# AlibabaResearch/efficientteacher

Hardware: AMD Instinct MI355X
Metric: SSOD images/sec (teacher+student step) YOLOv5l 640px (higher is better)
Workload: dtype bf16

## Files before the change

### efficientteacher_amd/_lib.py

```python
import ctypes
import os
from ctypes import c_char_p, c_double, c_float, c_int, c_int64, c_size_t, c_void_p

import torch

_HERE = os.path.dirname(os.path.abspath(__file__))
LIB_PATH = os.environ.get("ET_HIP_LIB") or os.path.join(_HERE, "libet_hip.so")

ET_F32, ET_BF16, ET_F16 = 0, 1, 2

P = c_void_p
SIGNATURES = {
    "et_build_arch": (c_char_p, []),
    "et_abi_version": (c_int, []),
    "et_nms_ssod_workspace_bytes": (c_int, [c_int, c_int, ctypes.POINTER(c_size_t)]),
    "et_nms_workspace_bytes": (c_int, [c_int, c_int, c_int, c_int, c_int, ctypes.POINTER(c_size_t)]),
    "et_nms": (c_int, [P, c_int, c_int, c_int, c_float, c_float, c_int, c_int, ctypes.c_uint64, ctypes.c_uint64, c_int,
                       c_float, c_int, P, P, P, P, P, c_size_t, P]),
    "et_nms_ssod": (c_int, [P, c_int, c_int, c_int, c_float, c_float, c_int, c_int, P, P, P, P, P, c_size_t, P]),
    "et_val_match": (c_int, [P, c_int, P, c_int, c_int, P, c_int, P, c_int, c_int, P, c_int, c_int, c_int, c_int64, c_int64,
                             P, P, P, P, P, P]),
    "et_val_ap_workspace_bytes": (c_int, [c_int, ctypes.POINTER(c_size_t)]),
    "et_val_ap": (c_int, [P, P, P, c_int64, P, c_int, c_int, P, P, P, P, P, c_size_t, P]),
    "et_detect_decode": (c_int, [P, c_int, c_int, c_int, c_int, c_int, c_int, c_int64, c_int64, c_int64, c_int64,
                                 P, c_float, P, c_int64, c_int64, P]),
    "et_ema_update": (c_int, [P, P, c_int64, c_float, c_float, P]),
    "et_adamw": (c_int, [P, P, P, P, P, c_int, c_int64, c_float, c_float, c_float, c_float, c_float, c_int, c_float, P, P]),
    "et_adamw_tick": (c_int, [P, c_float, c_float, P, P]),
    "et_adamw_dev": (c_int, [P, P, P, P, P, c_int, c_int64, c_float, c_float, c_float, c_float, c_float, P, c_float, P, P]),
    "et_sgd_nesterov": (c_int, [P, P, P, P, c_int, c_int64, c_float, c_float, c_float, c_int, c_float, P, P]),
    "et_cast_f32_to_lp": (c_int, [P, P, c_int, c_int64, P]),
    "et_scaler_check": (c_int, [P, c_int64, P, P]),
    "et_scaler_update": (c_int, [P, c_float, c_float, c_int, P]),
    "et_ema_update_dev": (c_int, [P, P, c_int64, P, P]),
    "et_sgd_nesterov_dev": (c_int, [P, P, P, P, c_int, c_int64, P, c_int, P, P]),
    "et_conv2d_stats_rows": (c_int, [c_int, c_int, c_int]),
    "et_conv2d_stats_rows_for": (c_int, [c_int] * 12),
    "et_conv2d_stats_adds_for": (c_int, [c_int] * 12),
    "et_conv2d_fwd": (c_int, [P, P, P, c_int] + [c_int] * 11 + [P, P, c_int, P, c_int, P, c_int, P, P]),
    "et_conv2d_dgrad": (c_int, [P, P, P, c_int] + [c_int] * 11 + [c_int, P, c_int, P, P]),
    "et_conv2d_dgrad_bn": (c_int, [P, P, P, c_int] + [c_int] * 10 + [P, c_int, P, c_int, P, P, c_int, P, c_int, P, P]),
    "et_conv2d_wgrad": (c_int, [P, P, P, c_int] + [c_int] * 11 + [P, P]),
    "et_conv2d_wgrad_grouped": (c_int, [P, c_int, c_int] + [c_int] * 9 + [P, P]),
    "et_weight_transpose_all": (c_int, [P, P, c_int, P, c_int, ctypes.c_longlong, P]),
    "et_weight_transpose": (c_int, [P, P, c_int, c_int, c_int, c_int, P]),
    "et_conv2d_kernel_name": (c_int, [c_int] * 13 + [c_char_p, c_int]),
    "et_env_knobs": (c_int, [c_char_p, c_int]),
    "et_conv2d_stem_u8_fwd": (c_int, [P, P, c_int, c_float, P, P, c_int, c_int, c_int, c_int, c_int, P, P, c_int, P, c_int, P, P]),
    "et_conv2d_stem_u8_wgrad": (c_int, [P, P, c_int, c_float, P, P, c_int, c_int, c_int, c_int, c_int, P, P]),
    "et_conv2d_stem_kernel_name": (c_int, [c_int] * 12 + [c_char_p, c_int]),
    "et_colsum": (c_int, [P, c_int, c_int, c_int, c_int, P, P]),
    "et_bn_reduce_rows": (c_int, [c_int, c_int, c_int]),
    "et_bn_finalize": (c_int, [P, c_int, c_int, c_double, P, P, c_float, c_float, P, P, P, P, P, P, P, P]),
    "et_bn_eval_affine": (c_int, [c_int, P, P, P, P, c_float, P, P, P]),
    "et_bn_act_fwd": (c_int, [P, c_int, P, c_int, P, c_int, c_int, c_int, c_int, P, P, c_int, P]),
    "et_bn_act_fwd_sharded": (c_int, [P, c_int, P, c_int, P, c_int, c_int, c_int, c_int, P, c_int, c_double, P, P, c_float, c_float,
                                      P, P, P, P, P, P, c_int, P]),
    "et_bn_act_bwd_sharded": (c_int, [P, c_int, P, c_int, P, c_int, c_int, c_int, c_int, P, P, P, P, P, c_int, P, P, P, c_int, c_int, P]),
    "et_bn_act_bwd": (c_int, [P, c_int, P, c_int, P, c_int, c_int, c_int, c_int, P, P, P, P, P, c_int, P, P, P, P,
                              c_size_t, P]),
    "et_bn_act_bwd_from_partials": (c_int, [P, c_int, P, c_int, P, c_int, c_int, c_int, c_int, P, P, P, P, P, c_int, P, P, P,
                                            P, c_int, P, P]),
    "et_act_bwd": (c_int, [P, c_int, P, c_int, P, c_int, c_int, c_int, c_int, c_int, P]),
    "et_pack_input": (c_int, [P, P, c_int, c_int, c_int, c_int, c_int, P]),
    "et_pack_input_u8": (c_int, [P, P, c_int, c_int, c_int, c_int, c_int, c_float, P]),
    "et_maxpool5_fwd": (c_int, [P, c_int, P, c_int, P, c_int, c_int, c_int, c_int, c_int, P]),
    "et_maxpool5_bwd": (c_int, [P, c_int, P, P, c_int, P, c_int, c_int, c_int, c_int, c_int, c_int, P]),
    "et_upsample2x_fwd": (c_int, [P, c_int, P, c_int, c_int, c_int, c_int, c_int, c_int, P]),
    "et_upsample2x_bwd": (c_int, [P, c_int, P, c_int, c_int, c_int, c_int, c_int, c_int, c_int, P]),
    "et_strong_view_u8": (c_int, [P, P, c_int, c_int, c_int, P, P, P, P, c_int, P]),
    "et_mosaic4_u8": (c_int, [P, P, c_int, c_int, c_int, P]),
    "et_pseudo_label_transform": (c_int, [P, P, P, c_int, c_int, c_int, c_int, c_int, P, P, P]),
    "et_score_log_append": (c_int, [P, P, c_int, c_int, P, P, P, c_int64, P]),
    "et_yolo_loss": (c_int, [P, P]),
    "et_ota_workspace_bytes": (c_int, [c_int, c_int, c_int, c_int, ctypes.POINTER(c_size_t)]),
    "et_ota_assign": (c_int, [P, P, c_float, c_int, P, P, P]),
    "et_select_targets": (c_int, [P, P, c_int, P, P, c_int, c_int, P, P]),
    "et_scale_cast": (c_int, [P, P, c_int, c_int64, c_float, P, P]),
    "et_domain_focal": (c_int, [P, c_int, c_int, c_int64, c_int, c_float, P, c_int, P, P]),
    "et_scale_inplace": (c_int, [P, c_int, c_int64, c_float, P, P]),
    "et_v8_decode": (c_int, [P, c_int, P, c_int, c_int, c_int, c_int, c_int, c_int, c_int, c_float, c_float, P, c_int64, c_int64, P]),
    "et_tal_loss": (c_int, [P, P, P, P, P, P, P, c_int, c_int, c_int, c_int, c_int, c_float, c_float, c_float, P, P, P, P, P]),
    "et_tal_assign_workspace_bytes": (c_int, [c_int, c_int, c_int, ctypes.POINTER(c_size_t)]),
    "et_tal_assign": (c_int, [P, P, P, P, P, P, c_int, c_int, c_int, c_int, c_int, c_float, c_float, c_float, P, P, P, P, P, c_size_t, P]),
    "et_tal_targets_pad": (c_int, [P, c_int, c_int, c_int, c_float, c_float, P, P, P]),
    "et_tal_pseudo_split": (c_int, [P, P, P, P, c_int, c_int, c_int, c_int, c_int, c_int, c_float, c_float, P, P, P, P, P, P, P, P, P]),
    "et_tal_assigned_gt": (c_int, [P, c_int, c_int, c_int, P, P]),
    "et_tal_merge_pseudo": (c_int, [P, P, P, P, P, P, P, P, P, c_int, c_int, c_int, c_int, P, P, P, P]),
}



class WgradItem(ctypes.Structure):
    _fields_ = [("x", ctypes.c_void_p), ("dy", ctypes.c_void_p), ("dw", ctypes.c_void_p), ("ldx", ctypes.c_int),
                ("ldy", ctypes.c_int)]


class LossLevel(ctypes.Structure):
    _fields_ = [("p", P), ("dp", P), ("tobj_ws", P), ("sb", c_int64), ("sa", c_int64), ("sy", c_int64),
                ("sx", c_int64), ("ny", c_int), ("nx", c_int), ("anchors", c_float * 6), ("balance", c_float)]


class LossDesc(ctypes.Structure):
    _fields_ = [("dtype", c_int), ("B", c_int), ("na", c_int), ("nc", c_int), ("NT", c_int), ("nl", c_int),
                ("anchor_t", c_float), ("gr", c_float), ("cp", c_float), ("cn", c_float), ("cls_pw", c_float),
                ("obj_pw", c_float), ("box_w", c_float), ("obj_w", c_float), ("cls_w", c_float),
                ("pass_mask", c_int), ("ignore_obj", c_int), ("targets", P), ("acc_ws", P), ("out", P),
                ("ota_match", P), ("obj_channel", c_int), ("balance_dev", P), ("autobalance_ssi", c_int), ("fl_gamma", c_float), ("level", LossLevel * 4)]


_dll = None
_emulated = False
CALL_TIMER = None
_NO_LAUNCH = frozenset(n for n in (
    "et_build_arch", "et_abi_version", "et_nms_ssod_workspace_bytes", "et_nms_workspace_bytes", "et_conv2d_stats_rows", "et_conv2d_stats_rows_for",
    "et_conv2d_kernel_name", "et_conv2d_stem_kernel_name", "et_env_knobs", "et_bn_reduce_rows", "et_ota_workspace_bytes", "et_tal_assign_workspace_bytes", "et_val_ap_workspace_bytes"))


class _TimedDll:

    def __init__(self, dll, timer):
        self._dll, self._timer, self._cache = dll, timer, {}

    def __getattr__(self, name):
        fn = self._cache.get(name)
        if fn is None:
            raw = getattr(self._dll, name)
            if name in _NO_LAUNCH or not name.startswith("et_"):
                fn = raw
            else:
                timer = self._timer

                def fn(*a, _raw=raw, _name=name):
                    tok = timer.begin(_name)
                    rc = _raw(*a)
                    timer.end(tok)
                    return rc
            self._cache[name] = fn
        return fn


class EtHipError(RuntimeError):
    pass


def _header_abi_version():
    import re
    with open(os.path.join(os.path.dirname(_HERE), "include", "et_hip.h")) as f:
        m = re.search(r"^#define\s+ET_ABI_VERSION\s+(\d+)", f.read(), re.M)
    if m is None:
        raise EtHipError("include/et_hip.h does not define ET_ABI_VERSION")
    return int(m.group(1))


ABI_VERSION = _header_abi_version()


def _declare(dll):
    for name, (res, args) in SIGNATURES.items():
        fn = getattr(dll, name)
        fn.restype = res
        fn.argtypes = args
    got = dll.et_abi_version()
    if got != ABI_VERSION:
        raise EtHipError(f"{getattr(dll, '_name', 'libet_hip.so')} has ABI version {got}, this binding needs {ABI_VERSION}: "
                         f"rebuild it (python -m efficientteacher_amd.csrc.build)")
    return dll


def load(path=None):
    global _dll
    if _dll is None:
        path = path or LIB_PATH
        if not os.path.exists(path):
            raise EtHipError(
                f"{path} not found: build the gfx950 kernels first "
                f"(python -m efficientteacher_amd.csrc.build).  There is no CPU fallback.")
        _dll = _declare(ctypes.CDLL(path))
    if CALL_TIMER is not None:
        w = getattr(CALL_TIMER, "_wrapped", None)
        if w is None or w._dll is not _dll:
            w = CALL_TIMER._wrapped = _TimedDll(_dll, CALL_TIMER)
        return w
    return _dll


def _use_library_for_tests(path, emulated):
    global _dll, _emulated
    _dll = _declare(ctypes.CDLL(path)) if path else None
    _emulated = bool(emulated) if path else False


def is_emulated():
    return _emulated
# ... 27 lines not shown
```

### efficientteacher_amd/autograd.py

```python
import torch
from torch.autograd import Function

from . import ops

ACT_CODE = {"silu": ops.ACT_SILU, "relu": ops.ACT_RELU, "none": ops.ACT_NONE}

FUSE_BN_BWD = True
FUSE_BN_BWD_K = 1
_RS_DGRAD = {}


def _dgrad_on_rs_tile(cs, x):
    key = (tuple(x.shape), x.dtype, cs.cinp, cs.coutp, cs.k, cs.stride, cs.pad)
    r = _RS_DGRAD.get(key)
    if r is None:
        N, H, W, _ = x.shape
        r = _RS_DGRAD[key] = cs.stride == 1 and ops.kernel_name("dgrad_full", x.dtype, N, H, W, cs.cinp, cs.coutp, cs.k, cs.stride,
                                                               cs.pad).startswith("conv_gemm_rs_kernel")
    return r


def _fuse_into(cs, bn, x=None):
    if bn is None:
        return None
    if FUSE_BN_BWD_K & (1 if cs.k == 1 else 2):
        return bn
    if cs.k > 1 and (FUSE_BN_BWD_K & 4) and x is not None and _dgrad_on_rs_tile(cs, x):
        return bn
    return None
SHARDED_BN = True


def _bn_train_fwd(x, w_lp, cs_stride, cs_pad, bs, act, residual=None, out=None):
    N, IH, IW, Cin = x.shape
    sh = None
    if SHARDED_BN and bs.sh_ld and ops.few_rows("fwd", x.dtype, N, IH, IW, Cin, w_lp.shape[0], w_lp.shape[1], cs_stride, cs_pad):
        sh = bs.acquire_fwd()
    if sh is not None:
        y = ops.conv2d_fwd(x, w_lp, cs_stride, cs_pad, shards=sh)
        N, OH, OW, _ = y.shape
        z, scale, shift, mean, invstd = ops.bn_act_fwd_sharded(y, sh, N * OH * OW, bs.gamma, bs.beta, bs.eps, bs.momentum, bs.rmean,
                                                               bs.rvar, act, residual=residual, out=out)
        return y, z, scale, shift, mean, invstd
    y, stats = ops.conv2d_fwd(x, w_lp, cs_stride, cs_pad, want_stats=True)
    N, OH, OW, _ = y.shape
    scale, shift, mean, invstd = ops.bn_finalize(stats, N * OH * OW, bs.gamma, bs.beta, bs.eps, bs.momentum, bs.rmean, bs.rvar)
    z = ops.bn_act_fwd(y, scale, shift, act, residual=residual, out=out)
    return y, z, scale, shift, mean, invstd


def _bn_sums(y, scale, shift, act, bs):
    return ops.BnBwdSums(y, scale, shift, act, slot=bs if (SHARDED_BN and bs.sh_ld) else None)


def _bn_train_bwd(dz, y, bs, scale, shift, mean, invstd, act, sums=None, out=None):
    part = sums.take(dz) if sums is not None else None
    if SHARDED_BN and bs.sh_ld and (isinstance(part, tuple) or (part is None and ops.few_reduce_rows(y))):
        sh = part if part is not None else bs.acquire_bwd()
        return ops.bn_act_bwd(dz, y, bs.gamma, scale, shift, mean, invstd, act, bs.ggamma, bs.gbeta, out=out, partial=part, shards=sh)
    return ops.bn_act_bwd(dz, y, bs.gamma, scale, shift, mean, invstd, act, bs.ggamma, bs.gbeta, out=out, partial=part)


GRAD_FORK = True

GRAD_READY_HOOK = None


class GradFork:

    def __init__(self):
        self.gb = None
        self.merged = False

    @staticmethod
    def split(x):
        if not (GRAD_FORK and torch.is_grad_enabled() and x.requires_grad):
            return x, x, None
        h = GradFork()
        a, b = _ForkFn.apply(x, h)
        return a, b, h

    @staticmethod
    def tap(b, fork):
        return b if fork is None else _TapFn.apply(b, fork)

    def take(self, shape, dtype):
        g = self.gb
        if g is None or tuple(g.shape) != tuple(shape) or g.dtype != dtype or g.dim() != 4 or g.stride(3) != 1:
            return None
        ld = g.stride(2)
        if not (ld >= g.shape[3] and g.stride(1) == ld * g.shape[2] and g.stride(0) == ld * g.shape[2] * g.shape[1]):
            return None
        return g


class _ForkFn(Function):
    @staticmethod
    def forward(ctx, x, holder):
        ctx.holder = holder
        return (x.as_strided(x.size(), x.stride(), x.storage_offset()), x.as_strided(x.size(), x.stride(), x.storage_offset()))

    @staticmethod
    def backward(ctx, ga, gb):
        h = ctx.holder
        merged = h.merged
        h.gb, h.merged = None, False
        if ga is None or gb is None:
            return (gb if ga is None else ga), None
        if merged:
            return ga, None
        return ga + gb, None


class _TapFn(Function):
    @staticmethod
    def forward(ctx, x, holder):
        ctx.holder = holder
        return x.as_strided(x.size(), x.stride(), x.storage_offset())

    @staticmethod
    def backward(ctx, g):
        ctx.holder.gb = g
        ctx.holder.merged = False
        return g, None


def _wgrad(x, dy, cs, *more_slots):
    hook = GRAD_READY_HOOK
    slots = (cs,) + more_slots

    def done():
        if hook is not None:
            for s in slots:
                hook(s)
    ops.WGRAD_QUEUE.submit(x, dy, cs.gw if not more_slots else _fused_gw(cs), cs.k, cs.stride, cs.pad,
                           on_done=done if hook is not None else None)


def _fused_gw(cs1):
    return cs1.gw.as_strided((2 * cs1.cout, 1, 1, cs1.cinp), (cs1.cinp, cs1.cinp, cs1.cinp, 1), cs1.gw.storage_offset())


class ConvBnActFn(Function):

    @staticmethod
    def forward(ctx, x, residual, wparam, cs, bs, act, nbt, dst=None, bn_in=None, bn_out=None, acc=None, u8=None):
        ctx.u8 = u8
        ctx.x_u8 = x if isinstance(x, ops.U8Images) else None
        ctx.w_needs_grad = wparam.requires_grad
        ctx.bn_in = bn_in if (bn_in is not None and cs.stride == 1 and residual is None) else None
        ctx.acc = acc
        if nbt is not None:
            nbt.add_(1)
        out = None if dst is None else dst[0][..., dst[1]:dst[1] + cs.coutp]
        y, z, scale, shift, mean, invstd = _bn_train_fwd(x, cs.w_lp, cs.stride, cs.pad, bs, act, residual=residual, out=out)
        ctx.cs, ctx.bs, ctx.act = cs, bs, act
        ctx.has_res = residual is not None
        ctx.x_needs_grad = x.requires_grad
        ctx.bn_mine = None
        if bn_out is not None and residual is None:
            ctx.bn_mine = _bn_sums(y, scale, shift, act, bs)
            bn_out.append(ctx.bn_mine)
        ctx.save_for_backward(None if ctx.x_u8 is not None else x, y, scale, shift, mean, invstd)
        return z

    @staticmethod
    def backward(ctx, dz):
        x, y, scale, shift, mean, invstd = ctx.saved_tensors
        cs, bs = ctx.cs, ctx.bs
        dz = _dense_or_slice(dz)
        dy = _bn_train_bwd(dz, y, bs, scale, shift, mean, invstd, ctx.act, sums=ctx.bn_mine)
        if ctx.w_needs_grad and ctx.u8 is not None:
            hook = GRAD_READY_HOOK
            ops.WGRAD_QUEUE.submit_stem_u8(ctx.u8, dy, cs.gw, on_done=(lambda: hook(cs)) if hook is not None else None)
        elif ctx.w_needs_grad:
            _wgrad(x if ctx.x_u8 is None else ctx.x_u8.packed(), dy, cs)
        dx = None
        if ctx.x_needs_grad:
            wT = cs.transposed()
            into = ctx.acc.take(x.shape, dy.dtype) if (ctx.acc is not None and ctx.bn_in is None) else None
            if into is not None:
                dx = ops.conv2d_dgrad(dy, wT, (x.shape[1], x.shape[2]), cs.stride, cs.pad, out=into, accumulate=True)
                ctx.acc.merged = True
            else:
                dx = ops.conv2d_dgrad(dy, wT, (x.shape[1], x.shape[2]), cs.stride, cs.pad, bn=_fuse_into(cs, ctx.bn_in, x))
        return dx, (dz if ctx.has_res else None), None, None, None, None, None, None, None, None, None, None


class BottleneckFn(Function):

    @staticmethod
    def forward(ctx, x, w1, w2, cs1, bs1, cs2, bs2, act1, act2, nbt1, nbt2, dst=None, bn_in=None, bn_out=None):
        ctx.w_needs_grad = w1.requires_grad or w2.requires_grad
        ctx.bn_in = bn_in
        y1, h, *a1 = _bn_train_fwd(x, cs1.w_lp, cs1.stride, cs1.pad, bs1, act1)
        for nbt in (nbt1, nbt2):
            if nbt is not None:
                nbt.add_(1)
        out = None if dst is None else dst[0][..., dst[1]:dst[1] + cs2.coutp]
        y2, z, *a2 = _bn_train_fwd(h, cs2.w_lp, cs2.stride, cs2.pad, bs2, act2, residual=x, out=out)
        ctx.meta = (cs1, bs1, cs2, bs2, act1, act2)
        ctx.x_needs_grad = x.requires_grad
        ctx.bn_mine = None
        if bn_out is not None:
            ctx.bn_mine = _bn_sums(y2, a2[0], a2[1], act2, bs2)
            bn_out.append(ctx.bn_mine)
        ctx.save_for_backward(x, y1, h, y2, *a1, *a2)
        return z

    @staticmethod
    def backward(ctx, dz):
        x, y1, h, y2, s1, b1, m1, i1, s2, b2, m2, i2 = ctx.saved_tensors
        cs1, bs1, cs2, bs2, act1, act2 = ctx.meta
        dz = _dense_or_slice(dz)
        dy2 = _bn_train_bwd(dz, y2, bs2, s2, b2, m2, i2, act2, sums=ctx.bn_mine)
        if ctx.w_needs_grad:
            _wgrad(h, dy2, cs2)
        inner = _fuse_into(cs2, _bn_sums(y1, s1, b1, act1, bs1), h) if FUSE_BN_BWD else None
        dh = ops.conv2d_dgrad(dy2, cs2.transposed(), (h.shape[1], h.shape[2]), cs2.stride, cs2.pad, bn=inner)
        dy1 = _bn_train_bwd(dh, y1, bs1, s1, b1, m1, i1, act1, sums=inner)
        if ctx.w_needs_grad:
            _wgrad(x, dy1, cs1)
        dx = None
        if ctx.x_needs_grad:
            dx = ops.conv2d_dgrad(dy1, cs1.transposed(), (x.shape[1], x.shape[2]), cs1.stride, cs1.pad,
                                  residual=dz, bn=_fuse_into(cs1, ctx.bn_in, x))
        return (dx,) + (None,) * 13


def c3_stem_fusable(cs1, bs1, cs2, bs2):
    es = cs1.w_lp.element_size()
    return (cs1.k == 1 and cs2.k == 1 and cs1.stride == 1 and cs2.stride == 1 and cs1.cinp == cs2.cinp
            and cs1.coutp == cs1.cout and cs2.coutp == cs2.cout and cs1.cout == cs2.cout
            and cs2.w_lp.data_ptr() == cs1.w_lp.data_ptr() + cs1.w_lp.numel() * es
            and cs2.gw.data_ptr() == cs1.gw.data_ptr() + cs1.gw.numel() * 4
            and bs2.aff_off == bs1.aff_off + bs1.c and bs1.c == cs1.cout and bs2.c == cs2.cout
            and bs1.eps == bs2.eps and bs1.momentum == bs2.momentum)


def _fused_vec(a, b):
    return a.as_strided((a.numel() + b.numel(),), (1,), a.storage_offset())


class C3StemFn(Function):

    @staticmethod
    def forward(ctx, x, w1, w2, cs1, bs1, cs2, bs2, act, nbt1, nbt2, buf, bn_out=None):
        ctx.w_needs_grad = w1.requires_grad or w2.requires_grad
        c = cs1.cout
        wf = cs1.w_lp.as_strided((2 * c, 1, 1, cs1.cinp), (cs1.cinp, cs1.cinp, cs1.cinp, 1), cs1.w_lp.storage_offset())
        sh1 = sh2 = None
        if SHARDED_BN and bs1.sh_ld and bs2.sh_ld and ops.few_rows("fwd", x.dtype, x.shape[0], x.shape[1], x.shape[2], cs1.cinp, 2 * c, 1, 1, 0):
            sh1, sh2 = bs1.acquire_fwd(), bs2.acquire_fwd()
        for nbt in (nbt1, nbt2):
            if nbt is not None:
                nbt.add_(1)
        if sh1 is not None and sh2 is not None:
            y = ops.conv2d_fwd(x, wf, 1, 0, shards=sh1)
            N, H, W, _ = y.shape
            af = torch.empty((4, 2 * c), dtype=torch.float32, device=y.device)
            t = ops.bn_act_fwd_sharded(y[..., :c], sh1, N * H * W, bs1.gamma, bs1.beta, bs1.eps, bs1.momentum, bs1.rmean, bs1.rvar,
                                       act, out=buf[..., :c], aff=af[:, :c])[0]
            y2 = ops.bn_act_fwd_sharded(y[..., c:], sh2, N * H * W, bs2.gamma, bs2.beta, bs2.eps, bs2.momentum, bs2.rmean, bs2.rvar,
                                        act, out=buf[..., 2 * c:], aff=af[:, c:])[0]
            aff = (af[0], af[1], af[2], af[3])
        else:
            y, st = ops.conv2d_fwd(x, wf, 1, 0, want_stats=True)
            N, H, W, _ = y.shape
            aff = ops.bn_finalize(st, N * H * W, _fused_vec(bs1.gamma, bs2.gamma), _fused_vec(bs1.beta, bs2.beta), bs1.eps,
                                  bs1.momentum, _fused_vec(bs1.rmean, bs2.rmean), _fused_vec(bs1.rvar, bs2.rvar))
            t = ops.bn_act_fwd(y[..., :c], aff[0][:c], aff[1][:c], act, out=buf[..., :c])
            y2 = ops.bn_act_fwd(y[..., c:], aff[0][c:], aff[1][c:], act, out=buf[..., 2 * c:])
        ctx.meta = (cs1, bs1, cs2, bs2, act)
        ctx.x_needs_grad = x.requires_grad
        ctx.bn_mine = None
        if bn_out is not None:
            ctx.bn_mine = _bn_sums(y[..., :c], aff[0][:c], aff[1][:c], act, bs1)
            bn_out.append(ctx.bn_mine)
        ctx.save_for_backward(x, y, *aff)
        return t, y2

    @staticmethod
    def backward(ctx, dt, dy2):
        x, y, scale, shift, mean, invstd = ctx.saved_tensors
        cs1, bs1, cs2, bs2, act = ctx.meta
        c = cs1.cout
        N, H, W, _ = y.shape
        dy = torch.empty_like(y)
        halves = ((dt, slice(0, c), bs1), (dy2, slice(c, 2 * c), bs2))
        for g, sl, bs in halves:
            if g is None:
                dy[..., sl].zero_()
                continue
            g = _dense_or_slice(g)
            _bn_train_bwd(g, y[..., sl], bs, scale[sl], shift[sl], mean[sl], invstd[sl], act,
                          sums=ctx.bn_mine if sl.start == 0 else None, out=dy[..., sl])
        if ctx.w_needs_grad:
            _wgrad(x, dy, cs1, cs2)
        dx = None
        if ctx.x_needs_grad:
            wf = cs1.w_lp.as_strided((2 * c, 1, 1, cs1.cinp), (cs1.cinp, cs1.cinp, cs1.cinp, 1), cs1.w_lp.storage_offset())
            dx = ops.conv2d_dgrad(dy, ops.weight_transpose(wf), (x.shape[1], x.shape[2]), 1, 0)
        return (dx,) + (None,) * 11


class _GradDst:

    def __init__(self, p):
        self.shape, self.stride, self.dtype, self.device = tuple(p.shape), tuple(p.stride()), p.dtype, p.device
        self.span = ops._flat_span(p)
        self.buf = None
        self.written = [False, False]

    def flat(self, half, n):
        if self.buf is None:
            self.buf = torch.empty(self.span, dtype=self.dtype, device=self.device)
        cut = n * self.stride[0]
        self.written[half] = True
        return self.buf[:cut] if half == 0 else self.buf[cut:]


class BatchSplitFn(Function):
    @staticmethod
    def forward(ctx, p, n, holder):
        ctx.n, ctx.holder = n, holder
        return p[:n], p[n:]

    @staticmethod
    def backward(ctx, ga, gb):
        h, n = ctx.holder, ctx.n
        cut = n * h.stride[0]

        def is_slot(g, half):
            return (g is not None and h.buf is not None and h.written[half] and tuple(g.stride()) == h.stride
                    and g.data_ptr() == h.buf.data_ptr() + (cut * h.buf.element_size() if half else 0))
        if h.buf is None:
            h.buf = torch.empty(h.span, dtype=h.dtype, device=h.device)
        full = h.buf.as_strided(h.shape, h.stride)
        for half, g in ((0, ga), (1, gb)):
            if is_slot(g, half):
                continue
            dst = full[:n] if half == 0 else full[n:]
            if g is None:
                (h.buf[:cut] if half == 0 else h.buf[cut:]).zero_()
            else:
                (h.buf[:cut] if half == 0 else h.buf[cut:]).zero_()
                dst.copy_(g)
        return full, None, None


def split_batch(p, n):
    if not (torch.is_grad_enabled() and p.requires_grad) or n <= 0 or n >= p.shape[0]:
        return p[:n], p[n:]
    h = _GradDst(p)
    a, b = BatchSplitFn.apply(p, n, h)
    a._et_grad_dst = (h, 0, n)
    b._et_grad_dst = (h, 1, n)
    return a, b


class ConvBiasFn(Function):

    @staticmethod
    def forward(ctx, x, wparam, cs, act, head):
        ctx.w_needs_grad = wparam.requires_grad
        y = ops.conv2d_fwd(x, cs.w_lp, cs.stride, cs.pad, bias=cs.bias, act=act)
        ctx.cs, ctx.act, ctx.head = cs, act, head
        ctx.x_needs_grad = x.requires_grad
        ctx.save_for_backward(x, y)
        if head is None:
            return y
        return head_view(y, *head)

    @staticmethod
    def backward(ctx, dy):
        x, y = ctx.saved_tensors
        cs = ctx.cs
        if ctx.head is not None:
            dy = head_grad_to_nhwc(dy, y.shape, *ctx.head)
        dy = _dense_or_slice(dy)
        if ctx.act != ops.ACT_NONE:
            dy = ops.act_bwd(dy, y, ctx.act)
        if ctx.w_needs_grad:
            ops.conv2d_wgrad(x, dy, cs.gw, cs.k, cs.stride, cs.pad)
            if cs.gbias is not None:
                ops.colsum(dy, cs.gbias)
            if GRAD_READY_HOOK is not None:
                GRAD_READY_HOOK(cs)
        dx = None
        if ctx.x_needs_grad:
            wT = cs.transposed()
            dx = ops.conv2d_dgrad(dy, wT, (x.shape[1], x.shape[2]), cs.stride, cs.pad)
        return dx, None, None, None, None


def head_view(y, na, no):
    B, ny, nx, CP = y.shape
    return y.as_strided((B, na, ny, nx, no), (ny * nx * CP, no, nx * CP, CP, 1), y.storage_offset())


def head_grad_to_nhwc(g, yshape, na, no):
    B, ny, nx, CP = yshape
    want = (ny * nx * CP, no, nx * CP, CP, 1)
    need = (g.storage_offset() + B * ny * nx * CP) * g.element_size()
    if tuple(g.stride()) == want and g.untyped_storage().nbytes() >= need:
        return g.as_strided((B, ny, nx, CP), (ny * nx * CP, nx * CP, CP, 1), g.storage_offset())
    buf = torch.zeros((B, ny, nx, CP), dtype=g.dtype, device=g.device)
    buf.as_strided((B, na, ny, nx, no), want).copy_(g)
    return buf


class JoinSlicesFn(Function):

    @staticmethod
    def forward(ctx, holder, *parts):
        buf = holder[0]
        off = 0
        for p in parts:
            assert p.data_ptr() == buf.data_ptr() + off * buf.element_size() and p.stride() == buf[..., :1].stride()
            off += p.shape[3]
        assert off == buf.shape[3]
        ctx.splits = [p.shape[3] for p in parts]
        return buf

    @staticmethod
    def backward(ctx, dcat):
        dcat = _dense_or_slice(dcat)
        return (None, *torch.split(dcat, ctx.splits, dim=3))


class SppfPoolFn(Function):

    @staticmethod
    def forward(ctx, x, holder=None):
        N, H, W, C = x.shape
        if holder is not None:
            cat = holder[0]
            assert cat.shape == (N, H, W, 4 * C) and x.data_ptr() == cat.data_ptr() and x.stride() == cat[..., :C].stride()
        else:
            cat = torch.empty((N, H, W, 4 * C), dtype=x.dtype, device=x.device)
            cat[..., :C].copy_(x)
        idx = []
        for i in range(3):
            _, ix = ops.maxpool5_fwd(cat[..., i * C:(i + 1) * C], out=cat[..., (i + 1) * C:(i + 2) * C])
            idx.append(ix)
        ctx.save_for_backward(*idx)
        ctx.C = C
        return cat

    @staticmethod
    def backward(ctx, dcat):
        i1, i2, i3 = ctx.saved_tensors
        C = ctx.C
        dcat = _dense_or_slice(dcat)
        d2 = ops.maxpool5_bwd(dcat[..., 3 * C:], i3, base=dcat[..., 2 * C:3 * C])
        d1 = ops.maxpool5_bwd(d2, i2, base=dcat[..., C:2 * C])
        return ops.maxpool5_bwd(d1, i1, base=dcat[..., :C]), None


class UpsampleCatFn(Function):

    @staticmethod
    def forward(ctx, a, b, acc=None, buf=None):
        N, H, W, Ca = a.shape
        Cb = b.shape[3]
        cat = in_place_concat_buffer(b, Ca, buf)
        if cat is None or cat.shape != (N, 2 * H, 2 * W, Ca + Cb):
            cat = torch.empty((N, 2 * H, 2 * W, Ca + Cb), dtype=a.dtype, device=a.device)
            cat[..., Ca:].copy_(b)
        ops.upsample2x_fwd(a, out=cat[..., :Ca])
        ctx.Ca = Ca
        ctx.acc = acc
        ctx.a_shape = tuple(a.shape)
        return cat

    @staticmethod
    def backward(ctx, dcat):
        dcat = _dense_or_slice(dcat)
        da_src = dcat[..., :ctx.Ca]
        into = ctx.acc.take(ctx.a_shape, dcat.dtype) if ctx.acc is not None else None
        if into is not None:
            da = ops.upsample2x_bwd(da_src, out=into, accumulate=True)
            ctx.acc.merged = True
        else:
            da = ops.upsample2x_bwd(da_src)
        return da, dcat[..., ctx.Ca:], None, None


def in_place_concat_buffer(b, Ca, buf):
    if buf is None:
        return None
    es = buf.element_size()
    if (b.data_ptr() == buf.data_ptr() + Ca * es and b.stride() == buf[..., Ca:].stride() and b.shape[:3] == buf.shape[:3]
            and Ca + b.shape[3] == buf.shape[3]):
        return buf
    return None


class GradReverseFn(Function):
    @staticmethod
    def forward(ctx, x):
        return x.view_as(x)

    @staticmethod
    def backward(ctx, g):
        return ops.scale_inplace(g.contiguous().clone(), -1.0)


class DomainFocalFn(Function):

    @staticmethod
    def forward(ctx, label, *feats):
        total = sum(f.shape[0] * f.shape[1] * f.shape[2] for f in feats)
        acc = torch.zeros(1, dtype=torch.float32, device=feats[0].device)
        grads = [ops.domain_focal(f, label, 0.5 / total, acc, want_grad=True) for f in feats]
        ctx.save_for_backward(*grads)
        return ops.scale_cast(acc, torch.float32, scale=0.5 / total)

    @staticmethod
    def backward(ctx, gout):
        g = gout.reshape(1).float().contiguous()
        return (None, *[ops.scale_inplace(gr.clone(), 1.0, dev_scale=g) for gr in ctx.saved_tensors])


def _dense_or_slice(g):
    if g.dim() == 4 and g.stride(3) == 1:
        ld = g.stride(2)
        if ld >= g.shape[3] and g.stride(1) == ld * g.shape[2] and g.stride(0) == ld * g.shape[2] * g.shape[1]:
            return g
    return g.contiguous()
```

### efficientteacher_amd/csrc/conv.hip

```cpp
#include "et_device.h"
#include "../../include/et_hip.h"
#include <stdlib.h>
#include <stdio.h>
#include <string.h>
#include <type_traits>

typedef __attribute__((ext_vector_type(16))) float f32x16;
typedef __attribute__((ext_vector_type(8))) __bf16 bf16x8;
typedef __attribute__((ext_vector_type(8))) _Float16 f16x8;
typedef __attribute__((ext_vector_type(4))) unsigned int u32x4;
__device__ __forceinline__ u32x4 mk4(unsigned a, unsigned b, unsigned c, unsigned d) { u32x4 v = {a, b, c, d}; return v; }
__device__ __forceinline__ void et_pin_loaded(u32x4& v) {
#if defined(__HIP_DEVICE_COMPILE__)
    asm volatile("" : "+v"(v));
#endif
}

template <typename T, typename V> __device__ __forceinline__ f32x16 et_mfma32(const V a, const V b, const f32x16 c) {
    static_assert(sizeof(V) == 16, "8 x 16-bit operands");
    if constexpr (std::is_same<T, et_f16>::value)
        return __builtin_amdgcn_mfma_f32_32x32x16_f16(__builtin_bit_cast(f16x8, a), __builtin_bit_cast(f16x8, b), c, 0, 0, 0);
    else
        return __builtin_amdgcn_mfma_f32_32x32x16_bf16(__builtin_bit_cast(bf16x8, a), __builtin_bit_cast(bf16x8, b), c, 0, 0, 0);
}

#define CONV_MAX_TAPS 36
#ifndef ET_S1_NT
#define ET_S1_NT 1
#endif
#ifndef ET_GLDS_SHORTK_WGS
#define ET_GLDS_SHORTK_WGS 4
#endif
#define RS_A_ROWS(BM) ((BM) + 16)

struct FastDiv {
    uint32_t magic, shift, d;
};
static FastDiv make_fastdiv(uint32_t d) {
    FastDiv f;
    if (d == 0) d = 1;
    f.d = d;
    uint32_t s = 0;
    while ((1ull << s) < d) ++s;
    f.shift = s;
    f.magic = (uint32_t)((((1ull << 32) * ((1ull << s) - d)) / d) + 1);
    return f;
}
__device__ __forceinline__ uint32_t fdiv(uint32_t n, const FastDiv& f) {
    return (__umulhi(n, f.magic) + n) >> f.shift;
}

struct GatherGeom {
    int N, IH, IW, Cin, ldx;
    int QH, QW, M;
    int OH, OW, Cout, ldy;
    int isy, isx;
    int osy, osx, ooy, oox;
    int T, TT;
    int CV, KV;
    int tap_inner;
    int xcd_swz;
    int ntm, ntn, nfast;
    FastDiv dQW, dQH, dCV, dW1;
    signed char dy[CONV_MAX_TAPS], dx[CONV_MAX_TAPS];
    unsigned char wt[CONV_MAX_TAPS];
    int tapinfo[CONV_MAX_TAPS];
};

__device__ __forceinline__ void tap_lookup_uniform(const GatherGeom& g, int tap, int& dy, int& dx, int& wt) {
    const int ti = g.tapinfo[__builtin_amdgcn_readfirstlane(tap)];
    dy = (int)(signed char)(ti & 0xff);
    dx = (int)(signed char)((ti >> 8) & 0xff);
    wt = (ti >> 16) & 0xff;
}

enum { ACT_NONE = 0, ACT_SILU = 1, ACT_RELU = 2 };

struct Epilogue {
    const float* scale;
    const float* bias;
    int act;
    const void* res;
    int ldr;
    float* stats;
    int accumulate;
    const void* bn_y;
    int ld_bn;
    const float* bn_scale;
    const float* bn_shift;
    int bn_act;
    int stats_ld;
};

__device__ __forceinline__ void tile_of_block(const GatherGeom& g, int& bx, int& by) {
    int id = blockIdx.x;
    if (g.nfast) {
        if (g.xcd_swz) {
            const int nb = gridDim.x, q = nb >> 3, r = nb & 7, xcd = id & 7, k = id >> 3;
            id = (xcd < r ? xcd * (q + 1) : r * (q + 1) + (xcd - r) * q) + k;
        }
        bx = id / g.ntn;
        by = id - bx * g.ntn;
    } else {
        by = id / g.ntm;
        bx = id - by * g.ntm;
        if (g.xcd_swz) {
            const int nb = g.ntm, q = nb >> 3, r = nb & 7, xcd = bx & 7, k = bx >> 3;
            bx = (xcd < r ? xcd * (q + 1) : r * (q + 1) + (xcd - r) * q) + k;
        }
    }
}

template <int BKV> __device__ __forceinline__ int lds_swz(int r) {
    if constexpr (BKV == 8) return ((r >> 1) & 7) ^ ((r >> 4) & 3);
    else return (r >> 2) & 3;
}


struct NoBetween { __device__ __forceinline__ void operator()(int) const {} };
template <typename T, int BM, int BN, int WM, int WN, int BKV, typename BETWEEN = NoBetween>
__device__ __forceinline__ void mma_chunk(const u32x4* __restrict__ sm, f32x16 (&acc)[BM / WM / 32][BN / WN / 32],
                                          int wm, int wn, int lane, BETWEEN between = BETWEEN()) {
    constexpr int TM = BM / WM / 32, TN = BN / WN / 32;
    const int l31 = lane & 31, g = lane >> 5;
    u32x4 af[2][TM], bf[2][TN];
    auto fetch = [&](int kk, int set) {
#pragma unroll
        for (int tm = 0; tm < TM; ++tm) {
            const int r = wm * (BM / WM) + tm * 32 + l31;
            af[set][tm] = sm[r * BKV + ((kk * 2 + g) ^ lds_swz<BKV>(r))];
        }
#pragma unroll
        for (int tn = 0; tn < TN; ++tn) {
            const int r = wn * (BN / WN) + tn * 32 + l31;
            bf[set][tn] = sm[(BM + r) * BKV + ((kk * 2 + g) ^ lds_swz<BKV>(r))];
        }
    };
    fetch(0, 0);
#pragma unroll
    for (int kk = 0; kk < BKV / 2; ++kk) {
        const int cur = kk & 1;
        if (kk + 1 < BKV / 2) {
            fetch(kk + 1, cur ^ 1);
            __builtin_amdgcn_sched_barrier(0);
        }
#pragma unroll
        for (int tm = 0; tm < TM; ++tm)
#pragma unroll
            for (int tn = 0; tn < TN; ++tn) {
                if constexpr (sizeof(T) == 2) {
                    acc[tm][tn] = et_mfma32<T>(af[cur][tm], bf[cur][tn], acc[tm][tn]);
                } else {
                    acc[tm][tn] = __builtin_amdgcn_mfma_f32_32x32x2f32(__uint_as_float(af[cur][tm].x), __uint_as_float(bf[cur][tn].x), acc[tm][tn], 0, 0, 0);
                    acc[tm][tn] = __builtin_amdgcn_mfma_f32_32x32x2f32(__uint_as_float(af[cur][tm].y), __uint_as_float(bf[cur][tn].y), acc[tm][tn], 0, 0, 0);
                    acc[tm][tn] = __builtin_amdgcn_mfma_f32_32x32x2f32(__uint_as_float(af[cur][tm].z), __uint_as_float(bf[cur][tn].z), acc[tm][tn], 0, 0, 0);
                    acc[tm][tn] = __builtin_amdgcn_mfma_f32_32x32x2f32(__uint_as_float(af[cur][tm].w), __uint_as_float(bf[cur][tn].w), acc[tm][tn], 0, 0, 0);
                }
            }
        between(kk);
    }
}

template <int BM, int BN, int WM, int WN, int SROWS = 32> struct EpiLds {
    static constexpr int WCOLS = BN / WN, SLD = WCOLS + 4, SLAB = SROWS * SLD;
    static constexpr int FLOATS = WM * WN * SLAB;
    static constexpr int VEC16 = (FLOATS * 4 + 15) / 16;
};

template <int TN> struct EpiSums {
    float ssum[TN], ssq[TN];
    float bs1[8], bs2[8];
    const float* cst = nullptr;
    int cstride = 0;
    __device__ __forceinline__ void clear() {
#pragma unroll
        for (int tn = 0; tn < TN; ++tn) { ssum[tn] = 0.f; ssq[tn] = 0.f; }
#pragma unroll
        for (int e = 0; e < 8; ++e) { bs1[e] = 0.f; bs2[e] = 0.f; }
    }
};

template <int BN, int WN, int MODE>
__device__ __forceinline__ void conv_epilogue_write_stats(EpiSums<BN / WN / 32>& st, const GatherGeom& g, const Epilogue& ep, int n0, int lane,
                                                          int wn, int row, int zero_rows, int nrows) {
    constexpr int TN = BN / WN / 32, WCOLS = BN / WN, CVN = WCOLS / 8;
    const int l31 = lane & 31, hi = lane >> 5;
    const int scv = lane % CVN;
    const int co = n0 + wn * WCOLS + scv * 8;
    const bool bnb = MODE == 1 ? false : ep.bn_y != nullptr;
    if (bnb) {
#pragma unroll
        for (int e = 0; e < 8; ++e)
            for (int m = CVN; m < 64; m <<= 1) { st.bs1[e] += __shfl_xor(st.bs1[e], m); st.bs2[e] += __shfl_xor(st.bs2[e], m); }
        if (ep.stats_ld) {
            if (lane < CVN && co + 8 <= g.Cout) {
                float* d0 = ep.stats + ((size_t)(blockIdx.x % ET_BN_SHARDS) * 2) * ep.stats_ld + co;
#pragma unroll
                for (int e = 0; e < 8; ++e) { unsafeAtomicAdd(d0 + e, st.bs1[e]); unsafeAtomicAdd(d0 + ep.stats_ld + e, st.bs2[e]); }
            }
        } else if (lane < CVN && co + 8 <= g.Cout) {
            for (int r = 0; r <= zero_rows; ++r) {
                if (row + r >= nrows) break;
                float* d0 = ep.stats + ((size_t)(row + r) * 2 + 0) * g.Cout + co;
                float* d1 = ep.stats + ((size_t)(row + r) * 2 + 1) * g.Cout + co;
                if (r == 0) {
                    *(float4*)d0 = make_float4(st.bs1[0], st.bs1[1], st.bs1[2], st.bs1[3]); *(float4*)(d0 + 4) = make_float4(st.bs1[4], st.bs1[5], st.bs1[6], st.bs1[7]);
                    *(float4*)d1 = make_float4(st.bs2[0], st.bs2[1], st.bs2[2], st.bs2[3]); *(float4*)(d1 + 4) = make_float4(st.bs2[4], st.bs2[5], st.bs2[6], st.bs2[7]);
                } else {
                    const float4 z = make_float4(0.f, 0.f, 0.f, 0.f);
                    *(float4*)d0 = z; *(float4*)(d0 + 4) = z; *(float4*)d1 = z; *(float4*)(d1 + 4) = z;
                }
            }
        }
    } else {
#pragma unroll
        for (int tn = 0; tn < TN; ++tn) {
            const float sv = st.ssum[tn] + __shfl_xor(st.ssum[tn], 32);
            const float qv = st.ssq[tn] + __shfl_xor(st.ssq[tn], 32);
            const int cc = n0 + wn * WCOLS + tn * 32 + l31;
            if (ep.stats_ld) {
                if (hi == 0 && cc < g.Cout) {
                    float* d0 = ep.stats + ((size_t)(blockIdx.x % ET_BN_SHARDS) * 2) * ep.stats_ld + cc;
                    unsafeAtomicAdd(d0, sv); unsafeAtomicAdd(d0 + ep.stats_ld, qv);
                }
            } else if (hi == 0 && cc < g.Cout) {
                for (int r = 0; r <= zero_rows; ++r) {
                    if (row + r >= nrows) break;
                    ep.stats[((size_t)(row + r) * 2 + 0) * g.Cout + cc] = r == 0 ? sv : 0.f;
                    ep.stats[((size_t)(row + r) * 2 + 1) * g.Cout + cc] = r == 0 ? qv : 0.f;
                }
            }
        }
    }
}

template <int BN, int WN, int WM, int MODE>
__device__ __forceinline__ void conv_stats_add_sharded_wg(EpiSums<BN / WN / 32>& st, const GatherGeom& g, const Epilogue& ep, int tid, int lane,
                                                          int wm, int wn, float* red, int n0 = 0) {
    constexpr int TN = BN / WN / 32, WCOLS = BN / WN, CVN = WCOLS / 8;
    const int l31 = lane & 31, hi = lane >> 5;
    const bool bnb = MODE == 1 ? false : ep.bn_y != nullptr;
    __syncthreads();
    float* const r0 = red + (wm * 2) * BN + wn * WCOLS;
    if (bnb) {
        const int scv = lane % CVN;
#pragma unroll
        for (int e = 0; e < 8; ++e)
            for (int m = CVN; m < 64; m <<= 1) { st.bs1[e] += __shfl_xor(st.bs1[e], m); st.bs2[e] += __shfl_xor(st.bs2[e], m); }
        if (lane < CVN) {
#pragma unroll
            for (int e = 0; e < 8; ++e) { r0[scv * 8 + e] = st.bs1[e]; r0[BN + scv * 8 + e] = st.bs2[e]; }
        }
    } else {
#pragma unroll
        for (int tn = 0; tn < TN; ++tn) {
            const float sv = st.ssum[tn] + __shfl_xor(st.ssum[tn], 32);
            const float qv = st.ssq[tn] + __shfl_xor(st.ssq[tn], 32);
            if (hi == 0) { r0[tn * 32 + l31] = sv; r0[BN + tn * 32 + l31] = qv; }
        }
    }
    __syncthreads();
    float* const dst = ep.stats + ((size_t)(blockIdx.x % ET_BN_SHARDS) * 2) * ep.stats_ld + n0;
    for (int i = tid; i < 2 * BN; i += 64 * WM * WN) {
        const int t = i / BN, c = i % BN;
        float v = 0.f;
#pragma unroll
        for (int w = 0; w < WM; ++w) v += red[(w * 2 + t) * BN + c];
        if (n0 + c < g.Cout) unsafeAtomicAdd(dst + (size_t)t * ep.stats_ld + c, v);
    }
}

template <typename T, int BM, int BN, int WM, int WN, int ACT, int SROWS = 32, int MODE = 0, bool DEFER = false, bool EPF = true>
__device__ __forceinline__ void conv_epilogue_act(f32x16 (&acc)[BM / WM / 32][BN / WN / 32], u32x4* lds_raw, T* __restrict__ Y,
                                                  const GatherGeom& g, const Epilogue& ep, int bx, int m0, int n0, int tid,
                                                  int lane, int wm, int wn, EpiSums<BN / WN / 32>& st) {
    constexpr int TM = BM / WM / 32, TN = BN / WN / 32;
    static_assert(SROWS == 32 || SROWS == 16, "slab rows");
    constexpr int NH = 32 / SROWS;
    using L = EpiLds<BM, BN, WM, WN, SROWS>;
    constexpr int WCOLS = L::WCOLS, SLD = L::SLD;
    constexpr int CVN = WCOLS / 8;
    constexpr int RPI = 64 / CVN;
    static_assert(RPI <= SROWS, "a store iteration covers at most one slab");
    const int l31 = lane & 31, hi = lane >> 5;
    const int wave = wm * WN + wn;
    float* const stg = (float*)lds_raw + wave * L::SLAB;
    float (&ssum)[TN] = st.ssum;
    float (&ssq)[TN] = st.ssq;
    float (&bs1)[8] = st.bs1;
    float (&bs2)[8] = st.bs2;
    const bool ident = (g.osy == 1 && g.osx == 1 && g.ooy == 0 && g.oox == 0 && g.QH == g.OH && g.QW == g.OW);
    float csc[TN], cbi[TN];
#pragma unroll
    for (int tn = 0; tn < TN; ++tn) {
        const int co = n0 + wn * WCOLS + tn * 32 + l31;
        const bool cok = co < g.Cout;
        if constexpr (DEFER) {
            csc[tn] = st.cst[co - n0];
            cbi[tn] = st.cst[st.cstride + co - n0];
        } else {
            csc[tn] = (ep.scale && cok) ? ep.scale[co] : 1.0f;
            cbi[tn] = (ep.bias && cok) ? ep.bias[co] : 0.0f;
        }
    }
    const int srow = lane / CVN, scv = lane % CVN;
    const int co = n0 + wn * WCOLS + scv * 8;
    const bool bnb = MODE == 1 ? false : ep.bn_y != nullptr;
    const void* const ep_res = MODE == 1 ? nullptr : ep.res;
    const bool ep_accumulate = MODE == 1 ? false : (bool)ep.accumulate;
    const bool lean = ident && !bnb && ep_res == nullptr && !ep_accumulate && m0 + (wm + 1) * (BM / WM) <= g.M && n0 + BN <= g.Cout;
    float bsc[8], bsh[8];
#pragma unroll
    for (int e = 0; e < 8; ++e) { bsc[e] = 1.f; bsh[e] = 0.f; }
    if (bnb && co + 8 <= g.Cout) {
#pragma unroll
        for (int e = 0; e < 8; ++e) {
            if constexpr (DEFER) { bsc[e] = st.cst[2 * st.cstride + co - n0 + e]; bsh[e] = st.cst[3 * st.cstride + co - n0 + e]; }
            else { bsc[e] = ep.bn_scale[co + e]; bsh[e] = ep.bn_shift[co + e]; }
        }
    }
    auto bn_bwd_sums = [&](const float (&dz8)[8], const float (&y8)[8]) {
        auto body = [&](auto act_tag) {
            constexpr int BACT = decltype(act_tag)::value;
#pragma unroll
            for (int e = 0; e < 8; ++e) {
                const float u = y8[e] * bsc[e] + bsh[e];
                float gact = 1.f;
                if constexpr (BACT == ACT_SILU) { const float sg = __builtin_amdgcn_rcpf(1.0f + __expf(-u)); gact = sg * (1.0f + u * (1.0f - sg)); }
                else if constexpr (BACT == ACT_RELU) gact = u > 0.f ? 1.f : 0.f;
                const float du = dz8[e] * gact;
                bs1[e] += du;
                bs2[e] += du * y8[e];
            }
        };
        if (ep.bn_act == ACT_SILU) body(std::integral_constant<int, ACT_SILU>{});
        else if (ep.bn_act == ACT_RELU) body(std::integral_constant<int, ACT_RELU>{});
        else body(std::integral_constant<int, ACT_NONE>{});
    };
    constexpr int NIT = SROWS / RPI;
    constexpr bool PF = EPF && sizeof(T) == 2 && MODE == 0;
    const bool pf_on = PF && !lean && (ep_res != nullptr || ep_accumulate || bnb);
    const bool pf_a_is_res = ep_res != nullptr;
    u32x4 pf_a[NIT], pf_b[NIT];
    auto pix_of = [&](int p) -> long long {
        if (ident) return p;
        const uint32_t t1 = fdiv((uint32_t)p, g.dQW), qx = p - t1 * g.QW;
        const uint32_t n = fdiv(t1, g.dQH), qy = t1 - n * g.QH;
        return ((long long)n * g.OH + (qy * g.osy + g.ooy)) * g.OW + (qx * g.osx + g.oox);
    };
#pragma unroll
    for (int tmh = 0; tmh < TM * NH; ++tmh) {
        const int tm = tmh / NH, hoff = (tmh % NH) * SROWS;
        if constexpr (PF) {
            if (pf_on) {
#pragma unroll
                for (int it = 0; it < NIT; ++it) {
                    const int p = m0 + wm * (BM / WM) + tm * 32 + hoff + it * RPI + srow;
                    if (p < g.M && co + 8 <= g.Cout) {
                        const long long pix = pix_of(p);
                        if (pf_a_is_res) pf_a[it] = *(const u32x4*)((const T*)ep_res + pix * ep.ldr + co);
                        else if (ep_accumulate) pf_a[it] = *(const u32x4*)(Y + pix * g.ldy + co);
                        if (bnb) pf_b[it] = *(const u32x4*)((const T*)ep.bn_y + pix * ep.ld_bn + co);
                    }
                }
            }
        }
#pragma unroll
        for (int rr = 0; rr < 16 / NH; ++rr) {
            const int r = (tmh % NH) * (16 / NH) + rr;
            const int row = (rr & 3) + 8 * (rr >> 2) + 4 * hi;
#pragma unroll
            for (int tn = 0; tn < TN; ++tn) {
                float v = acc[tm][tn][r];
                ssum[tn] += v;
                ssq[tn] += v * v;
                v = v * csc[tn] + cbi[tn];
                if constexpr (ACT == ACT_SILU) v = v * __builtin_amdgcn_rcpf(1.0f + __expf(-v));
                else if constexpr (ACT == ACT_RELU) v = fmaxf(v, 0.f);
                stg[row * SLD + tn * 32 + l31] = v;
            }
        }
        __builtin_amdgcn_s_waitcnt(0xC07F);
        __builtin_amdgcn_wave_barrier();
        if constexpr (sizeof(T) == 2) {
            if (lean) {
#pragma unroll
                for (int it = 0; it < SROWS / RPI; ++it) {
                    const int row = it * RPI + srow;
                    const long long p = m0 + wm * (BM / WM) + tm * 32 + hoff + row;
                    const float4 a = *(const float4*)(stg + row * SLD + scv * 8);
                    const float4 b = *(const float4*)(stg + row * SLD + scv * 8 + 4);
                    *(u32x4*)(Y + p * g.ldy + co) = mk4(et_lp<T>::pack(a.x, a.y), et_lp<T>::pack(a.z, a.w), et_lp<T>::pack(b.x, b.y), et_lp<T>::pack(b.z, b.w));
                }
                __builtin_amdgcn_s_waitcnt(0xC07F);
                __builtin_amdgcn_wave_barrier();
                continue;
            }
        }
#pragma unroll
        for (int it = 0; it < SROWS / RPI; ++it) {
            const int row = it * RPI + srow;
            const int p = m0 + wm * (BM / WM) + tm * 32 + hoff + row;
            if (p < g.M && co < g.Cout) {
                const long long pix = pix_of(p);
                float v[8];
                const float4 a = *(const float4*)(stg + row * SLD + scv * 8);
                const float4 b = *(const float4*)(stg + row * SLD + scv * 8 + 4);
                v[0] = a.x; v[1] = a.y; v[2] = a.z; v[3] = a.w; v[4] = b.x; v[5] = b.y; v[6] = b.z; v[7] = b.w;
                T* yp = Y + pix * g.ldy + co;
                if (co + 8 <= g.Cout) {
                    if constexpr (sizeof(T) == 2) {
                        if (ep_res) {
                            u32x4 rr;
                            if constexpr (PF) rr = pf_a[it];
                            else rr = *(const u32x4*)((const T*)ep_res + pix * ep.ldr + co);
                            v[0] += et_lp<T>::lo(rr.x); v[1] += et_lp<T>::hi(rr.x);
                            v[2] += et_lp<T>::lo(rr.y); v[3] += et_lp<T>::hi(rr.y);
                            v[4] += et_lp<T>::lo(rr.z); v[5] += et_lp<T>::hi(rr.z);
                            v[6] += et_lp<T>::lo(rr.w); v[7] += et_lp<T>::hi(rr.w);
                        }
                        if (ep_accumulate) {
                            u32x4 rr;
                            if (PF && !pf_a_is_res) rr = pf_a[it];
                            else rr = *(const u32x4*)yp;
                            v[0] += et_lp<T>::lo(rr.x); v[1] += et_lp<T>::hi(rr.x);
                            v[2] += et_lp<T>::lo(rr.y); v[3] += et_lp<T>::hi(rr.y);
                            v[4] += et_lp<T>::lo(rr.z); v[5] += et_lp<T>::hi(rr.z);
                            v[6] += et_lp<T>::lo(rr.w); v[7] += et_lp<T>::hi(rr.w);
                        }
                        const u32x4 packed = mk4(et_lp<T>::pack(v[0], v[1]), et_lp<T>::pack(v[2], v[3]), et_lp<T>::pack(v[4], v[5]),
                                                 et_lp<T>::pack(v[6], v[7]));
                        *(u32x4*)yp = packed;
                        if (bnb) {
                            u32x4 yy;
                            if constexpr (PF) yy = pf_b[it];
                            else yy = *(const u32x4*)((const T*)ep.bn_y + pix * ep.ld_bn + co);
                            const unsigned pw[4] = {packed.x, packed.y, packed.z, packed.w}, yw[4] = {yy.x, yy.y, yy.z, yy.w};
                            float dz8[8], y8[8];
#pragma unroll
                            for (int e = 0; e < 8; ++e) {
                                dz8[e] = (e & 1) ? et_lp<T>::hi(pw[e >> 1]) : et_lp<T>::lo(pw[e >> 1]);
                                y8[e] = (e & 1) ? et_lp<T>::hi(yw[e >> 1]) : et_lp<T>::lo(yw[e >> 1]);
                            }
                            bn_bwd_sums(dz8, y8);
                        }
                    } else {
                        if (ep_res) {
                            const float* rp = (const float*)ep_res + pix * ep.ldr + co;
                            const float4 r0 = *(const float4*)rp, r1 = *(const float4*)(rp + 4);
                            v[0] += r0.x; v[1] += r0.y; v[2] += r0.z; v[3] += r0.w; v[4] += r1.x; v[5] += r1.y; v[6] += r1.z; v[7] += r1.w;
                        }
                        if (ep_accumulate) {
                            const float4 r0 = *(const float4*)yp, r1 = *(const float4*)((const float*)yp + 4);
                            v[0] += r0.x; v[1] += r0.y; v[2] += r0.z; v[3] += r0.w; v[4] += r1.x; v[5] += r1.y; v[6] += r1.z; v[7] += r1.w;
                        }
                        *(float4*)yp = make_float4(v[0], v[1], v[2], v[3]);
                        *(float4*)((float*)yp + 4) = make_float4(v[4], v[5], v[6], v[7]);
                        if (bnb) {
                            const float* bp = (const float*)ep.bn_y + pix * ep.ld_bn + co;
                            const float4 y0 = *(const float4*)bp, y1 = *(const float4*)(bp + 4);
                            const float yv8[8] = {y0.x, y0.y, y0.z, y0.w, y1.x, y1.y, y1.z, y1.w};
                            bn_bwd_sums(v, yv8);
                        }
                    }
                } else {
                    for (int e = 0; e < 8 && co + e < g.Cout; ++e) {
                        float x = v[e];
                        if (ep_res) x += et_elem<T>::ld(((const T*)ep_res)[pix * ep.ldr + co + e]);
                        if (ep_accumulate) x += et_elem<T>::ld(yp[e]);
                        yp[e] = et_elem<T>::st(x);
                    }
                }
            }
        }
        __builtin_amdgcn_s_waitcnt(0xC07F);
        __builtin_amdgcn_wave_barrier();
    }
    if constexpr (!DEFER) {
        if (ep.stats) {
            constexpr int RPW = (BM / WM) / 64;
            static_assert((BM / WM) % 64 == 0, "wave tiles are whole 64-row blocks");
            if (ep.stats_ld) conv_stats_add_sharded_wg<BN, WN, WM, MODE>(st, g, ep, tid, lane, wm, wn, (float*)lds_raw, n0);
            else conv_epilogue_write_stats<BN, WN, MODE>(st, g, ep, n0, lane, wn, (m0 + wm * (BM / WM)) / 64, RPW - 1, (g.M + 63) / 64);
        }
    }
}

template <typename T, int BM, int BN, int WM, int WN, int SROWS = 32, int MODE = 0, bool DEFER = false, bool EPF = true>
__device__ __forceinline__ void conv_epilogue(f32x16 (&acc)[BM / WM / 32][BN / WN / 32], u32x4* lds_raw, T* __restrict__ Y,
                                              const GatherGeom& g, const Epilogue& ep, int bx, int m0, int n0, int tid,
                                              int lane, int wm, int wn, EpiSums<BN / WN / 32>& st) {
    if (ep.act == ACT_SILU) conv_epilogue_act<T, BM, BN, WM, WN, ACT_SILU, SROWS, MODE, DEFER, EPF>(acc, lds_raw, Y, g, ep, bx, m0, n0, tid, lane, wm, wn, st);
    else if (ep.act == ACT_RELU) conv_epilogue_act<T, BM, BN, WM, WN, ACT_RELU, SROWS, MODE, DEFER, EPF>(acc, lds_raw, Y, g, ep, bx, m0, n0, tid, lane, wm, wn, st);
    else conv_epilogue_act<T, BM, BN, WM, WN, ACT_NONE, SROWS, MODE, DEFER, EPF>(acc, lds_raw, Y, g, ep, bx, m0, n0, tid, lane, wm, wn, st);
}
template <typename T, int BM, int BN, int WM, int WN, bool EPF = true>
__device__ __forceinline__ void conv_epilogue(f32x16 (&acc)[BM / WM / 32][BN / WN / 32], u32x4* lds_raw, T* __restrict__ Y,
                                              const GatherGeom& g, const Epilogue& ep, int bx, int m0, int n0, int tid,
                                              int lane, int wm, int wn) {
    EpiSums<BN / WN / 32> st;
    st.clear();
    conv_epilogue<T, BM, BN, WM, WN, 32, 0, false, EPF>(acc, lds_raw, Y, g, ep, bx, m0, n0, tid, lane, wm, wn, st);
}

template <typename T, int BM, int BN, int WM, int WN, int BKV, bool UTAP>
__global__ __launch_bounds__(256) void conv_gemm_kernel(const T* __restrict__ X, const T* __restrict__ W,
                                                        T* __restrict__ Y, GatherGeom g, Epilogue ep) {
    constexpr int VEC = et_elem<T>::VEC;
    constexpr int TM = BM / WM / 32, TN = BN / WN / 32;
    constexpr int RPT = 256 / BKV;
    constexpr int RA = BM / RPT, RB = BN / RPT;
    constexpr int STAGE_VEC = (BM + BN) * BKV;
    constexpr int EPI_VEC = EpiLds<BM, BN, WM, WN>::VEC16;
    constexpr int LDS_VEC = 2 * STAGE_VEC > EPI_VEC ? 2 * STAGE_VEC : EPI_VEC;
    __shared__ __attribute__((aligned(16))) u32x4 lds_raw[LDS_VEC];
    u32x4* const lds0 = lds_raw;
    u32x4* const lds1 = lds_raw + STAGE_VEC;

    const int tid = threadIdx.x, lane = tid & 63, wave = tid >> 6;
    const int wm = wave / WN, wn = wave % WN;
    int bx, by;
    tile_of_block(g, bx, by);
    const int m0 = bx * BM, n0 = by * BN;
    const int lvec = tid % BKV, lrow = tid / BKV;

    int a_off[RA], a_iy[RA], a_ix[RA];
    bool a_ok[RA];
#pragma unroll
    for (int j = 0; j < RA; ++j) {
        const int p = m0 + lrow + j * RPT;
        a_ok[j] = p < g.M;
        const uint32_t pp = a_ok[j] ? p : 0;
        const uint32_t t1 = fdiv(pp, g.dQW), qx = pp - t1 * g.QW;
        const uint32_t n = fdiv(t1, g.dQH), qy = t1 - n * g.QH;
        a_iy[j] = qy * g.isy;
        a_ix[j] = qx * g.isx;
        a_off[j] = ((n * g.IH + a_iy[j]) * g.IW + a_ix[j]) * g.ldx;
    }
    int b_off[RB];
    bool b_ok[RB];
#pragma unroll
    for (int j = 0; j < RB; ++j) {
        const int co = n0 + lrow + j * RPT;
        b_ok[j] = co < g.Cout;
        b_off[j] = (b_ok[j] ? co : 0) * g.TT * g.Cin;
    }

    f32x16 acc[TM][TN];
#pragma unroll
    for (int tm = 0; tm < TM; ++tm)
#pragma unroll
        for (int tn = 0; tn < TN; ++tn)
#pragma unroll
            for (int r = 0; r < 16; ++r) acc[tm][tn][r] = 0.f;

    const int nchunks = (g.KV + BKV - 1) / BKV;
    u32x4 raA[RA], rbA[RB], raB[RA], rbB[RB];
    unsigned okA = 0u, okB = 0u;
    int tap_u = 0, cv_u = 0;

    auto gload = [&](int chunk, int tap_c, int cv_c, u32x4 (&ra)[RA], u32x4 (&rb)[RB]) -> unsigned {
        int tap, cv;
        bool kok = true;
        if constexpr (UTAP) {
            tap = tap_c; cv = cv_c + lvec;
        } else {
            const uint32_t kv = chunk * BKV + lvec;
            kok = kv < (uint32_t)g.KV;
            const uint32_t kk = kok ? kv : 0;
            tap = fdiv(kk, g.dCV); cv = kk - tap * g.CV;
        }
        int dy, dx, wt;
        if constexpr (UTAP) tap_lookup_uniform(g, tap, dy, dx, wt);
        else { dy = g.dy[tap]; dx = g.dx[tap]; wt = g.wt[tap]; }
        const int doff = (dy * g.IW + dx) * g.ldx + cv * VEC;
        const int woff = wt * g.Cin + cv * VEC;
        unsigned okmask = 0u;
#pragma unroll
        for (int j = 0; j < RA; ++j) {
            const bool ok = kok && a_ok[j] && (unsigned)(a_iy[j] + dy) < (unsigned)g.IH &&
                            (unsigned)(a_ix[j] + dx) < (unsigned)g.IW;
            ra[j] = *(const u32x4*)(X + (ok ? a_off[j] + doff : 0));
            okmask |= ok ? (1u << j) : 0u;
        }
#pragma unroll
        for (int j = 0; j < RB; ++j) {
            const bool ok = kok && b_ok[j];
            rb[j] = *(const u32x4*)(W + (ok ? b_off[j] + woff : 0));
            okmask |= ok ? (1u << (16 + j)) : 0u;
        }
        return okmask;
    };
#define ET_ADVANCE_CURSOR()                                              \
    if constexpr (UTAP) {                                                \
        if (g.tap_inner) {                                               \
            if (++tap_u >= g.T) { tap_u = 0; cv_u += BKV; }              \
        } else {                                                         \
            cv_u += BKV;                                                 \
            if (cv_u >= g.CV) { cv_u = 0; ++tap_u; }                     \
        }                                                                \
    }
    auto lstore = [&](u32x4* __restrict__ dst, const u32x4 (&ra)[RA], const u32x4 (&rb)[RB], unsigned okmask) {
        const u32x4 zero = mk4(0, 0, 0, 0);
#pragma unroll
        for (int j = 0; j < RA; ++j) {
            const int r = lrow + j * RPT;
            dst[r * BKV + (lvec ^ lds_swz<BKV>(r))] = ((okmask >> j) & 1u) ? ra[j] : zero;
        }
#pragma unroll
        for (int j = 0; j < RB; ++j) {
            const int r = lrow + j * RPT;
            dst[(BM + r) * BKV + (lvec ^ lds_swz<BKV>(r))] = ((okmask >> (16 + j)) & 1u) ? rb[j] : zero;
// ... 623 lines not shown
    auto stage_a_piece = [&](int q, int ub, int j, int cv) {
        u32x4* const wbase = slotA + ub * A_VEC + q * 512 + wave * 64;
        const int dy = sgn * (j - 1);
        if constexpr (BUF) {
            const unsigned bad = (a_nokm >> (3 * q + 1 + dy)) & 1u;
            et_bufdma16(rsX, (bad << 31) | (unsigned)a_off[q], (unsigned)(((dy + 1) * rowstep + cv * VEC) * (int)sizeof(T)), wbase);
        } else {
            const bool ok = (a_okm >> (3 * q + 1 + dy)) & 1u;
            et_glds16(ok ? X + (a_off[q] + dy * g.IW * g.ldx + (cv + lv) * VEC) : ZERO, wbase);
        }
    };
    auto stage_b_piece = [&](int j, int b, int jj, int tap, int cv) {
        u32x4* const wbase = slotB + (2 * j + b) * HALF_VEC + wave * 64;
        if constexpr (BUF) {
            et_bufdma16(rsW, voffB, (unsigned)(((jj * 128 + j * 32) * wrow + tap * g.Cin + cv * VEC) * (int)sizeof(T)), wbase + jj * 512);
        } else {
            const bool ok = (b_okm >> (j * 2 + jj)) & 1u;
            et_glds16(ok ? W + (b_off0 + (jj * 128 + j * 32) * wrow + tap * g.Cin + (cv + lv) * VEC) : ZERO, wbase + jj * 512);
        }
    };

    u32x4 af[2][4], bf[4];
    auto load_a = [&](int i, int ub, auto shift_tag) {
        constexpr int SFT = decltype(shift_tag)::value;
        const char* sm = (const char*)(slotA + ub * A_VEC);
#pragma unroll
        for (int t = 0; t < 2; ++t)
#pragma unroll
            for (int kk = 0; kk < 4; ++kk) af[t][kk] = *(const u32x4*)(sm + (abase[i][t][SFT] ^ (kk * 32)));
    };
    auto load_b = [&](int j, int b) {
        const u32x4* sm = slotB + (2 * j + b) * HALF_VEC;
        const int r = wn * 32 + l31;
#pragma unroll
        for (int kk = 0; kk < 4; ++kk) bf[kk] = sm[r * BKV + ((kk * 2 + gk) ^ lds_swz<BKV>(r))];
    };
    auto mfma8 = [&](int i, int j, auto&& piece0, auto&& piece1) {
        __builtin_amdgcn_s_setprio(1);
        __builtin_amdgcn_sched_barrier(0);
#pragma unroll
        for (int kk = 0; kk < 4; ++kk)
#pragma unroll
            for (int t = 0; t < 2; ++t) {
                acc[2 * i + t][j] = et_mfma32<T>(af[t][kk], bf[kk], acc[2 * i + t][j]);
                const int n = kk * 2 + t;
                if (n == 1) { __builtin_amdgcn_sched_barrier(0); piece0(); __builtin_amdgcn_sched_barrier(0); }
                if (n == 4) { __builtin_amdgcn_sched_barrier(0); piece1(); __builtin_amdgcn_sched_barrier(0); }
            }
        __builtin_amdgcn_sched_barrier(0);
        __builtin_amdgcn_s_setprio(0);
    };
    auto nothing = [] {};

    const int nunits = 3 * (g.CV / BKV);
#pragma unroll
    for (int q = 0; q < NPIECE; ++q) stage_a_piece(q, 0, 0, 0);
#pragma unroll
    for (int j = 0; j < 2; ++j) { stage_b_piece(j, 0, 0, sgn > 0 ? 0 : 2, 0); stage_b_piece(j, 0, 1, sgn > 0 ? 0 : 2, 0); }
    et_wait_vmem();
    __builtin_amdgcn_s_barrier();
#define ET_PP_BAR() __builtin_amdgcn_s_barrier()
#define ET_PP_WAIT(n) et_wait_vmem_le_pp<n>()
    if (wm == 1) __builtin_amdgcn_s_barrier();

    int jrow = 0, cv_u = 0, bbuf = 0;
#pragma unroll 1
    for (int u = 0; u < nunits; ++u) {
        const bool more = u + 1 < nunits;
        int nj = jrow + 1, ncv = cv_u;
        if (nj == 3) { nj = 0; ncv += BKV; }
        const int ub = u & 1, nub = ub ^ 1;
        auto chunk = [&](auto ktag) {
            constexpr int k = decltype(ktag)::value;
            const bool stage_b = k < 2 || more;
            const int kn = k < 2 ? k + 1 : 0;
            const int ntap = (k < 2 ? jrow : nj) * 3 + (sgn > 0 ? kn : 2 - kn), nbcv = k < 2 ? cv_u : ncv;
            const int nb = bbuf ^ 1;
            const std::integral_constant<int, k> shift{};
            load_a(0, ub, shift); load_b(0, bbuf);
            if (k > 0 && more) ET_PP_WAIT(1); else ET_PP_WAIT(0);
            ET_PP_BAR();
            mfma8(0, 0, [&] { if (more) stage_a_piece(2 * k, nub, nj, ncv); }, nothing);
            ET_PP_BAR();
            load_b(1, bbuf);
            ET_PP_BAR();
            mfma8(0, 1, [&] { if (stage_b) stage_b_piece(0, nb, 0, ntap, nbcv); }, [&] { if (stage_b) stage_b_piece(0, nb, 1, ntap, nbcv); });
            ET_PP_BAR();
            load_a(1, ub, shift);
            ET_PP_BAR();
            mfma8(1, 1, [&] { if (stage_b) stage_b_piece(1, nb, 0, ntap, nbcv); }, [&] { if (stage_b) stage_b_piece(1, nb, 1, ntap, nbcv); });
            ET_PP_BAR();
            load_b(0, bbuf);
            if (stage_b) ET_PP_WAIT(2); else ET_PP_WAIT(0);
            ET_PP_BAR();
            mfma8(1, 0, [&] { if (k < 2 && more) stage_a_piece(2 * k + 1, nub, nj, ncv); }, nothing);
            ET_PP_BAR();
            bbuf = nb;
        };
        chunk(std::integral_constant<int, 0>{});
        chunk(std::integral_constant<int, 1>{});
        chunk(std::integral_constant<int, 2>{});
        jrow = nj; cv_u = ncv;
    }
    if (wm == 0) __builtin_amdgcn_s_barrier();
    __syncthreads();
    conv_epilogue<T, BM, BN, WM, WN, false>(acc, lds_raw, Y, g, ep, bx, m0, n0, tid, lane, wm, wn);
#undef ET_PP_BAR
#undef ET_PP_WAIT
}
template <typename T>
__global__ __launch_bounds__(512, 2) void conv_gemm_pprs_kernel(const T* __restrict__ X, const T* __restrict__ W,
                                                                T* __restrict__ Y, const T* __restrict__ ZERO,
                                                                GatherGeom g, Epilogue ep) {
    conv_gemm_pprs_body<T, true>(X, W, Y, ZERO, g, ep);
}
template <typename T>
__global__ __launch_bounds__(512, 2) void conv_gemm_pprs_flat_kernel(const T* __restrict__ X, const T* __restrict__ W,
                                                                     T* __restrict__ Y, const T* __restrict__ ZERO,
                                                                     GatherGeom g, Epilogue ep) {
    conv_gemm_pprs_body<T, false>(X, W, Y, ZERO, g, ep);
}

template <typename T, int KC, int WN, int TN, int WM, int TMW, int NS, int WGS, bool FULL, bool BUF>
__device__ __forceinline__ void conv1x1_stream_body(const T* __restrict__ X, const T* __restrict__ W,
                                                    T* __restrict__ Y, const T* __restrict__ ZERO,
                                                    const GatherGeom& g, const Epilogue& ep) {
    constexpr int BN = 32 * TN * WN, BM = 32 * TMW * WM, BKV = 8, VEC = 8;
    constexpr int TM = TMW;
    constexpr int NT = 64 * WM * WN;
    constexpr int CH_VEC = BM * BKV;
    constexpr int DT = CH_VEC < NT ? CH_VEC : NT;
    constexpr int PER = CH_VEC / DT;
    constexpr int MODE = FULL ? 0 : 1;
    using L = EpiLds<BM, BN, WM, WN, 16>;
    static_assert(KC == 1 || KC == 2 || KC == 4, "K = 64 * KC");
    static_assert(CH_VEC % DT == 0 && DT % 64 == 0 && PER >= 1 && (NS - 1) * PER < 64 && NS >= 2 && NS <= 16, "ring");
    __shared__ __attribute__((aligned(16))) u32x4 lds_raw[NS * CH_VEC + L::VEC16 + BN];
    u32x4* const ring = lds_raw;
    u32x4* const slabs = lds_raw + NS * CH_VEC;
    float* const cst = (float*)(lds_raw + NS * CH_VEC + L::VEC16);

    const int tid = threadIdx.x, lane = tid & 63;
    const int wave = __builtin_amdgcn_readfirstlane(tid >> 6);
    const int wm = wave / WN, wn = wave % WN;
    const int l31 = lane & 31, gk = lane >> 5;
    const int lvec = tid % BKV, lrow = tid / BKV;
    constexpr int RPT = DT / BKV;
    const bool stager = wave * 64 < DT;

    for (int c = tid; c < BN; c += NT) {
        const bool cok = c < g.Cout;
        cst[c] = (ep.scale && cok) ? ep.scale[c] : 1.0f;
        cst[BN + c] = (ep.bias && cok) ? ep.bias[c] : 0.0f;
        cst[2 * BN + c] = (FULL && ep.bn_y && cok) ? ep.bn_scale[c] : 1.0f;
        cst[3 * BN + c] = (FULL && ep.bn_y && cok) ? ep.bn_shift[c] : 0.0f;
    }

    int a_row[PER], a_lv[PER];
#pragma unroll
    for (int j = 0; j < PER; ++j) {
        a_row[j] = lrow + j * RPT;
        a_lv[j] = (lvec ^ lds_swz<BKV>(a_row[j])) * VEC;
    }
    et_rsrc rsX;
    if constexpr (BUF) {
        rsX = et_make_rsrc(X, (unsigned)(((size_t)(g.M - 1) * g.ldx + KC * 64) * sizeof(T)));
#pragma unroll
        for (int j = 0; j < PER; ++j) a_row[j] = (a_row[j] * g.ldx + a_lv[j]) * (int)sizeof(T);
    }
    const int ntiles = g.ntm;
    const int my_tiles = ((int)blockIdx.x < ntiles) ? (ntiles - 1 - (int)blockIdx.x) / (int)gridDim.x + 1 : 0;
    const int total = my_tiles * KC;
    int is_tile = blockIdx.x, is_kc = 0, is_slot = 0, issued = 0;
    auto issue = [&]() {
        if (stager) {
            u32x4* const wbase = ring + is_slot * CH_VEC + wave * 64;
            const int m0i = is_tile * BM;
            const unsigned soff = (unsigned)(((size_t)m0i * g.ldx + is_kc * 64) * sizeof(T));
#pragma unroll
            for (int j = 0; j < PER; ++j) {
                if constexpr (BUF) {
#if ET_S1_NT
                    et_bufdma16_nt(rsX, (unsigned)a_row[j], soff, wbase + j * DT);
#else
                    et_bufdma16(rsX, (unsigned)a_row[j], soff, wbase + j * DT);
#endif
                } else {
                    const int p = m0i + a_row[j];
                    const T* src = p < g.M ? X + ((size_t)p * g.ldx + is_kc * 64 + a_lv[j]) : ZERO;
#if ET_S1_NT
                    et_glds16_nt(src, wbase + j * DT);
#else
                    et_glds16(src, wbase + j * DT);
#endif
                }
            }
        }
        ++issued;
        if (++is_kc == KC) { is_kc = 0; is_tile += gridDim.x; }
        is_slot = is_slot + 1 == NS ? 0 : is_slot + 1;
    };
#pragma unroll
    for (int s = 0; s < NS - 1; ++s)
        if (issued < total) issue();

    u32x4 bw[TN][KC * 4];
#pragma unroll
    for (int tn = 0; tn < TN; ++tn) {
        const int co = wn * (32 * TN) + tn * 32 + l31;
        const bool cok = co < g.Cout;
        const T* wr = W + (size_t)(cok ? co : 0) * g.Cin + gk * VEC;
#pragma unroll
        for (int ks = 0; ks < KC * 4; ++ks) {
            bw[tn][ks] = *(const u32x4*)(wr + ks * 16);
            if (!cok) bw[tn][ks] = mk4(0, 0, 0, 0);
        }
    }
#pragma unroll
    for (int tn = 0; tn < TN; ++tn)
#pragma unroll
        for (int ks = 0; ks < KC * 4; ++ks) et_pin_loaded(bw[tn][ks]);
    __syncthreads();

    int abase[TM];
#pragma unroll
    for (int tm = 0; tm < TM; ++tm) {
        const int r = wm * (32 * TMW) + tm * 32 + l31;
        abase[tm] = (r * BKV + (gk ^ lds_swz<BKV>(r))) * 16;
    }

    EpiSums<TN> st;
    st.clear();
    st.cst = cst;
    st.cstride = BN;
    int rd = 0, q = 0;
    for (int i = 0; i < my_tiles; ++i) {
        const int m0 = ((int)blockIdx.x + i * (int)gridDim.x) * BM;
        f32x16 acc[TM][TN];
#pragma unroll
        for (int tm = 0; tm < TM; ++tm)
#pragma unroll
            for (int tn = 0; tn < TN; ++tn)
#pragma unroll
                for (int r = 0; r < 16; ++r) acc[tm][tn][r] = 0.f;
#pragma unroll
        for (int kc = 0; kc < KC; ++kc, ++q) {
            const int ahead = min(NS - 2, total - 1 - q);
            switch (ahead) {
#define ET_S1_WAIT(A) case A: et_wait_vmem_le_lds_read_done<((A) <= NS - 2 ? (A) : 0) * PER>(); break;
                ET_S1_WAIT(1) ET_S1_WAIT(2) ET_S1_WAIT(3) ET_S1_WAIT(4) ET_S1_WAIT(5) ET_S1_WAIT(6) ET_S1_WAIT(7)
                ET_S1_WAIT(8) ET_S1_WAIT(9) ET_S1_WAIT(10) ET_S1_WAIT(11) ET_S1_WAIT(12) ET_S1_WAIT(13) ET_S1_WAIT(14)
#undef ET_S1_WAIT
                default: et_wait_vmem_lds_read_done(); break;
            }
            __builtin_amdgcn_s_barrier();
            if (issued < total) issue();
            const char* const sa = (const char*)(ring + rd * CH_VEC);
            u32x4 af[2][TM];
#pragma unroll
            for (int tm = 0; tm < TM; ++tm) af[0][tm] = *(const u32x4*)(sa + abase[tm]);
#pragma unroll
            for (int kk = 0; kk < 4; ++kk) {
                const int cur = kk & 1;
                if (kk + 1 < 4) {
#pragma unroll
                    for (int tm = 0; tm < TM; ++tm) af[cur ^ 1][tm] = *(const u32x4*)(sa + (abase[tm] ^ ((kk + 1) * 32)));
                    __builtin_amdgcn_sched_barrier(0);
                }
#pragma unroll
                for (int tm = 0; tm < TM; ++tm)
#pragma unroll
                    for (int tn = 0; tn < TN; ++tn)
                        acc[tm][tn] = et_mfma32<T>(af[cur][tm], bw[tn][kc * 4 + kk], acc[tm][tn]);
            }
            rd = rd + 1 == NS ? 0 : rd + 1;
        }
        conv_epilogue<T, BM, BN, WM, WN, 16, MODE, true>(acc, slabs, Y, g, ep, 0, m0, 0, tid, lane, wm, wn, st);
    }
    if (ep.stats) {
        if (ep.stats_ld) conv_stats_add_sharded_wg<BN, WN, WM, MODE>(st, g, ep, tid, lane, wm, wn, (float*)ring);
        else conv_epilogue_write_stats<BN, WN, MODE>(st, g, ep, 0, lane, wn, (int)blockIdx.x * WM + wm, 0, (int)gridDim.x * WM);
    }
}
template <typename T, int KC, int WN, int TN, int WM, int TMW, int NS, int WGS, bool FULL>
__global__ __launch_bounds__(64 * WM * WN, WGS) void conv1x1_stream_kernel(const T* __restrict__ X, const T* __restrict__ W,
                                                                          T* __restrict__ Y, const T* __restrict__ ZERO,
                                                                          GatherGeom g, Epilogue ep) {
    conv1x1_stream_body<T, KC, WN, TN, WM, TMW, NS, WGS, FULL, true>(X, W, Y, ZERO, g, ep);
}
template <typename T, int KC, int WN, int TN, int WM, int TMW, int NS, int WGS, bool FULL>
__global__ __launch_bounds__(64 * WM * WN, WGS) void conv1x1_stream_flat_kernel(const T* __restrict__ X, const T* __restrict__ W,
                                                                               T* __restrict__ Y, const T* __restrict__ ZERO,
                                                                               GatherGeom g, Epilogue ep) {
    conv1x1_stream_body<T, KC, WN, TN, WM, TMW, NS, WGS, FULL, false>(X, W, Y, ZERO, g, ep);
}

#define STEM_TR 4
#define STEM_TC 64
#define STEM_PH 12
#define STEM_PITCH 132
#define STEM_PSLOTS (7 * 256)
#define STEM_WPITCH 37
#define STEM_WSLOTS (10 * 256)
#define STEM_MAX_SEGS 4

struct StemArgs {
    const uint16_t* x; const uint16_t* w; uint16_t* y; const uint16_t* zero;
    int N, IH, IW, ldx, OH, OW, ldy, Cout;
// ... 1266 lines not shown
    else if (p.kind == GEMM_PP) snprintf(buf, n, "conv_gemm_pp_kernel<%s>", t);
    else if (p.kind == GEMM_PPRS) snprintf(buf, n, "conv_gemm_pprs_kernel<%s>", t);
    else if (p.kind == GEMM_RS) snprintf(buf, n, "conv_gemm_rs_kernel<%s, %d, %d, %d, %d>", t, p.BM, p.BN, p.WM, p.WN);
    else if (p.kind == GEMM_GLDS) snprintf(buf, n, "conv_gemm_glds_kernel<%s, %d, %d, %d, %d, %d, %d, %s>", t, p.BM, p.BN, p.WM, p.WN, p.BKV, p.NS, p.utap ? "true" : "false");
    else snprintf(buf, n, "conv_gemm_kernel<%s, %d, %d, %d, %d, %d, %s>", t, p.BM, p.BN, p.WM, p.WN, p.BKV, p.utap ? "true" : "false");
}

static int s1_grid(int ntm, const GemmPlan& p) {
    int n = env_int("ET_CONV_S1_WGS", p.wgs * device_cus());
    if (n < 1) n = 1;
    return n < ntm ? n : ntm;
}

template <typename T>
static int launch_gemm(const void* X, const void* W, void* Y, const void* zero16, GatherGeom g, const Epilogue& ep,
                       hipStream_t s) {
    if (g.M <= 0) return 0;
    g.nfast = 1;
    const GemmPlan* const pp = plan_gemm(g, (int)sizeof(T), zero16 != nullptr, ep.res != nullptr || ep.accumulate || ep.bn_y != nullptr);
    if (!pp) return -2;
    const GemmPlan& p = *pp;
    g.ntm = (g.M + p.BM - 1) / p.BM;
    g.ntn = (g.Cout + p.BN - 1) / p.BN;
    const T* x = (const T*)X; const T* w = (const T*)W; T* y = (T*)Y; const T* z = (const T*)zero16;
    const dim3 grid(g.ntm * g.ntn), block(64 * p.WM * p.WN);
    int i = 0;
#define ET_TWINS(BUF_, GRID_, KERN_, FLAT_) \
    { if (BUF_) hipLaunchKernelGGL(KERN_, GRID_, block, 0, s, x, w, y, z, g, ep); else hipLaunchKernelGGL(FLAT_, GRID_, block, 0, s, x, w, y, z, g, ep); return 0; }
    if (p.kind == GEMM_REG) {
#define ET_REG(BM_, BN_, WM_, WN_, BKV_, UT_) \
    if (pp == &reg_rows[i++]) { hipLaunchKernelGGL((conv_gemm_kernel<T, BM_, BN_, WM_, WN_, BKV_, UT_>), grid, block, 0, s, x, w, y, g, ep); return 0; }
        ET_REG_ROWS
#undef ET_REG
    }
    if (p.kind == GEMM_GLDS) {
#define ET_GLDS(BM_, BN_, WM_, WN_, BKV_, NS_, UT_) \
    if constexpr (NS_ == 2 || sizeof(T) == 2) if (pp == &glds_rows[i]) { hipLaunchKernelGGL((conv_gemm_glds_kernel<T, BM_, BN_, WM_, WN_, BKV_, NS_, UT_>), grid, block, 0, s, x, w, y, z, g, ep); return 0; } \
    ++i;
        ET_GLDS_ROWS
#undef ET_GLDS
    }
    if constexpr (sizeof(T) == 2) {
        if (p.kind == GEMM_S1) {
            const dim3 sgrid(s1_grid(g.ntm, p));
            const bool s1buf = env_int("ET_CONV_BUF_DMA", 1) && (size_t)g.M * g.ldx * sizeof(T) < (1ull << 31);
#define ET_S1(KC_, WN_, TN_, WM_, TMW_, NS_, WGS_, FULL_) \
    if (pp == &s1_rows[i++]) ET_TWINS(s1buf, sgrid, (conv1x1_stream_kernel<T, KC_, WN_, TN_, WM_, TMW_, NS_, WGS_, FULL_>), (conv1x1_stream_flat_kernel<T, KC_, WN_, TN_, WM_, TMW_, NS_, WGS_, FULL_>))
            ET_S1_ROWS
#undef ET_S1
        }
        if (p.kind == GEMM_PP) {
            hipLaunchKernelGGL((conv_gemm_pp_kernel<T>), grid, block, 0, s, x, w, y, z, g, ep);
            return 0;
        }
        if (p.kind == GEMM_PPRS || p.kind == GEMM_RS) {
            const size_t xb = ((size_t)g.N * g.IH * g.IW * g.ldx + (size_t)g.IW * g.ldx) * sizeof(T), wb = (size_t)g.Cout * g.TT * g.Cin * sizeof(T);
            const bool buf = env_int("ET_CONV_BUF_DMA", 1) && xb < (1ull << 31) && wb < (1ull << 31);
            if (p.kind == GEMM_PPRS) ET_TWINS(buf, grid, (conv_gemm_pprs_kernel<T>), (conv_gemm_pprs_flat_kernel<T>))
#define ET_RS(BM_, BN_, WM_, WN_) \
    if (pp == &rs_rows[i++]) ET_TWINS(buf, grid, (conv_gemm_rs_kernel<T, BM_, BN_, WM_, WN_>), (conv_gemm_rs_flat_kernel<T, BM_, BN_, WM_, WN_>))
            ET_RS_ROWS
#undef ET_RS
        }
    }
#undef ET_TWINS
    return -2;
}

extern "C" int et_conv2d_stats_rows(int N, int OH, int OW) { return (N * OH * OW + 63) / 64; }

static bool stem_eligible(int dtype, int Cin, int Cout, int KH, int KW, int stride, int pad, bool has_residual, bool has_zero_page) {
    return (dtype == ET_BF16 || dtype == ET_F16) && KH == 6 && KW == 6 && stride == 2 && pad == 2 && Cin == 8 && Cout <= 64 && Cout % 8 == 0 &&
           !has_residual && has_zero_page;
}
static int stem_grid(int ntiles) {
    int grid = env_int("ET_CONV_STEM_WGS", 2 * device_cus());
    if (grid < 1) grid = 1;
    return grid < ntiles ? grid : ntiles;
}
template <typename A>
static void stem_tiles(A& a, int N, int IH, int IW) {
    a.N = N; a.IH = IH; a.IW = IW;
    a.OH = (IH + 4 - 6) / 2 + 1; a.OW = (IW + 4 - 6) / 2 + 1;
    a.trn = (a.OH + STEM_TR - 1) / STEM_TR; a.tcn = (a.OW + STEM_TC - 1) / STEM_TC;
    a.ntiles = N * a.trn * a.tcn;
}
template <bool U8>
static void launch_stem(StemArgs& a, int dtype, const float* scale, const float* bias, int act, float* stats, int stats_ld, hipStream_t s) {
    a.scale = scale; a.bias = bias; a.act = act; a.stats = stats; a.stats_ld = stats ? stats_ld : 0;
    a.stat_rows = (a.N * a.OH * a.OW + 63) / 64;
    int grid = stem_grid(a.ntiles);
    if (stats && !stats_ld && grid > a.stat_rows) grid = a.stat_rows;
#define ET_STEM(T_, ACT_) \
    do { \
        if constexpr (U8) hipLaunchKernelGGL((conv_stem_u8_kernel<T_, ACT_>), dim3(grid), dim3(256), 0, s, a); \
        else hipLaunchKernelGGL((conv_stem_kernel<T_, ACT_>), dim3(grid), dim3(256), 0, s, a); \
    } while (0)
    if (dtype == ET_F16) { if (act == ACT_SILU) ET_STEM(et_f16, ACT_SILU); else if (act == ACT_RELU) ET_STEM(et_f16, ACT_RELU); else ET_STEM(et_f16, ACT_NONE); }
    else { if (act == ACT_SILU) ET_STEM(uint16_t, ACT_SILU); else if (act == ACT_RELU) ET_STEM(uint16_t, ACT_RELU); else ET_STEM(uint16_t, ACT_NONE); }
#undef ET_STEM
}

extern "C" int et_conv2d_fwd(const void* x, const void* w, void* y, int dtype, int N, int IH, int IW, int Cin,
                             int ldx, int Cout, int KH, int KW, int stride, int pad, int ldy, const float* scale,
                             const float* bias, int act, const void* residual, int ldr, float* stats_partial,
                             int stats_ld, const void* zero16, et_stream_t stream) {
    if (!x || !w || !y) return -1;
    if (KH * KW > CONV_MAX_TAPS || stride < 1 || N <= 0 || Cout <= 0 || stats_ld < 0 || (stats_ld && stats_ld < Cout)) return -2;
    if (stem_eligible(dtype, Cin, Cout, KH, KW, stride, pad, residual != nullptr, zero16 != nullptr)) {
        StemArgs a;
        a.x = (const uint16_t*)x; a.w = (const uint16_t*)w; a.y = (uint16_t*)y; a.zero = (const uint16_t*)zero16;
        a.ldx = ldx; a.Cout = Cout; a.ldy = ldy;
        stem_tiles(a, N, IH, IW);
        launch_stem<false>(a, dtype, scale, bias, act, stats_partial, stats_ld, (hipStream_t)stream);
        ET_CHECK_LAUNCH();
        return 0;
    }
    GatherGeom g;
    const int vec = dtype == ET_F32 ? 4 : 8;
    int rc = fwd_geom(g, N, IH, IW, Cin, ldx, Cout, KH, KW, stride, pad, ldy, vec);
    if (rc) return rc;
    if (residual && !(residual == (const void*)y && ldr == ldy)) {
        const size_t eb = dtype == ET_F32 ? 4 : 2, npix = (size_t)g.N * g.OH * g.OW;
        const uintptr_t r0 = (uintptr_t)residual, r1 = r0 + ((npix - 1) * (size_t)ldr + (size_t)Cout) * eb;
        const uintptr_t y0 = (uintptr_t)y, y1 = y0 + ((npix - 1) * (size_t)ldy + (size_t)Cout) * eb;
        if (npix > 0 && r0 < y1 && y0 < r1) {
            const bool same_rows = ldr == ldy && ((r0 > y0 ? r0 - y0 : y0 - r0) % ((size_t)ldy * eb)) >= (size_t)Cout * eb &&
                                   ((r0 > y0 ? r0 - y0 : y0 - r0) % ((size_t)ldy * eb)) + (size_t)Cout * eb <= (size_t)ldy * eb;
            if (!same_rows) return -2;
        }
    }
    Epilogue ep{scale, bias, act, residual, ldr, stats_partial, 0};
    ep.stats_ld = stats_partial ? stats_ld : 0;
    if (!with_dtype(dtype, [&](auto t) { rc = launch_gemm<typename decltype(t)::type>(x, w, y, zero16, g, ep, (hipStream_t)stream); })) return -2;
    if (rc) return rc;
    ET_CHECK_LAUNCH();
    return 0;
}

template <typename T>
__global__ __launch_bounds__(256) void zero_lattice_kernel(T* __restrict__ dx, int N, int IH, int IW, int ldx, int Cin, int QH, int QW,
                                                           int stride, int py, int px) {
    const long long i = (long long)blockIdx.x * 256 + threadIdx.x;
    const long long total = (long long)N * QH * QW * Cin;
    if (i >= total) return;
    const int c = (int)(i % Cin);
    long long q = i / Cin;
    const int qx = (int)(q % QW); q /= QW;
    const int qy = (int)(q % QH);
    const int n = (int)(q / QH);
    dx[(((long long)n * IH + qy * stride + py) * IW + qx * stride + px) * ldx + c] = T(0);
}

static int conv2d_dgrad_impl(const void* dy, const void* wT, void* dx, int dtype, int N, int IH, int IW, int Cin,
                             int ldx, int Cout, int KH, int KW, int stride, int pad, int ldy, int accumulate,
                             const void* residual, int ldr, const void* bn_y, int ld_bn, const float* bn_scale,
                             const float* bn_shift, int bn_act, float* bn_stats, int bn_stats_ld, const void* zero16, et_stream_t stream) {
    if (!dy || !wT || !dx) return -1;
    if (KH * KW > CONV_MAX_TAPS || stride < 1 || stride > 2 || N <= 0) return -2;
    if (residual && stride != 1) return -2;
    if (bn_y && (stride != 1 || !bn_scale || !bn_shift || !bn_stats || Cin % 8 || bn_stats_ld < 0 || (bn_stats_ld && bn_stats_ld < Cin))) return -2;
    const int vec = dtype == ET_F32 ? 4 : 8;
    for (int py = 0; py < stride; ++py)
        for (int px = 0; px < stride; ++px) {
            GatherGeom g;
            int rc = dgrad_geom(g, py, px, N, IH, IW, Cin, ldx, Cout, KH, KW, stride, pad, ldy, vec);
            if (rc == 1) continue;
            if (rc) return rc;
            const int t = g.T, QH = g.QH, QW = g.QW;
            Epilogue ep{nullptr, nullptr, ACT_NONE, residual, ldr, bn_y ? bn_stats : nullptr, accumulate,
                        bn_y, ld_bn, bn_scale, bn_shift, bn_act, bn_y ? bn_stats_ld : 0};
            if (t == 0) {
                const long long total = (long long)N * QH * QW * Cin;
                if (!accumulate && total > 0) {
                    if (dtype == ET_F32) hipLaunchKernelGGL((zero_lattice_kernel<float>), dim3(et_cdiv(total, 256)), dim3(256), 0, (hipStream_t)stream, (float*)dx, N, IH, IW, ldx, Cin, QH, QW, stride, py, px);
                    else hipLaunchKernelGGL((zero_lattice_kernel<uint16_t>), dim3(et_cdiv(total, 256)), dim3(256), 0, (hipStream_t)stream, (uint16_t*)dx, N, IH, IW, ldx, Cin, QH, QW, stride, py, px);
                }
                continue;
            }
            if (!with_dtype(dtype, [&](auto t) { rc = launch_gemm<typename decltype(t)::type>(dy, wT, dx, zero16, g, ep, (hipStream_t)stream); })) return -2;
            if (rc) return rc;
        }
    ET_CHECK_LAUNCH();
    return 0;
}

extern "C" int et_conv2d_dgrad(const void* dy, const void* wT, void* dx, int dtype, int N, int IH, int IW, int Cin,
                               int ldx, int Cout, int KH, int KW, int stride, int pad, int ldy, int accumulate,
                               const void* residual, int ldr,
                               const void* zero16, et_stream_t stream) {
    return conv2d_dgrad_impl(dy, wT, dx, dtype, N, IH, IW, Cin, ldx, Cout, KH, KW, stride, pad, ldy, accumulate, residual, ldr,
                             nullptr, 0, nullptr, nullptr, 0, nullptr, 0, zero16, stream);
}

extern "C" int et_conv2d_dgrad_bn(const void* dy, const void* wT, void* dx, int dtype, int N, int IH, int IW, int Cin,
                                  int ldx, int Cout, int KH, int KW, int pad, int ldy, const void* residual, int ldr,
                                  const void* bn_y, int ld_bn, const float* bn_scale, const float* bn_shift, int bn_act,
                                  float* bn_stats_partial, int bn_stats_ld, const void* zero16, et_stream_t stream) {
    if (!bn_y) return -1;
    return conv2d_dgrad_impl(dy, wT, dx, dtype, N, IH, IW, Cin, ldx, Cout, KH, KW, 1, pad, ldy, 0, residual, ldr, bn_y, ld_bn,
                             bn_scale, bn_shift, bn_act, bn_stats_partial, bn_stats_ld, zero16, stream);
}

static void wgrad_geom(WgradGeom& g, int N, int IH, int IW, int Cin, int ldx, int Cout, int KH, int KW, int stride, int pad, int ldy) {
    const int OH = (IH + 2 * pad - KH) / stride + 1, OW = (IW + 2 * pad - KW) / stride + 1;
    g.N = N; g.IH = IH; g.IW = IW; g.Cin = Cin; g.ldx = ldx;
    g.QH = OH; g.QW = OW; g.P = N * OH * OW; g.Cout = Cout; g.ldy = ldy;
    g.isy = g.isx = stride; g.T = KH * KW; g.NC = g.T * Cin;
    g.dQW = make_fastdiv(OW); g.dQH = make_fastdiv(OH); g.dCin = make_fastdiv(Cin); g.dW1 = make_fastdiv(OW + 1);
    g.PP = N * OH * (OW + 1);
    g.ident = (KH == 1 && KW == 1 && stride == 1 && pad == 0 && OH == IH && OW == IW) ? 1 : 0;
    g.buf = 0;
    for (int ky = 0; ky < KH; ++ky)
        for (int kx = 0; kx < KW; ++kx) {
            g.dy[ky * KW + kx] = (signed char)(ky - pad);
            g.dx[ky * KW + kx] = (signed char)(kx - pad);
        }
}

#define ET_WG_ROWS \
    ET_WG(256, 256, 2, 4) ET_WG(256, 128, 4, 2) ET_WG(256, 64, 4, 1) \
    ET_WG(128, 256, 2, 4) ET_WG(128, 128, 2, 2) ET_WG(128, 64, 2, 2) \
    ET_WG(64, 256, 1, 4)  ET_WG(64, 128, 2, 2)  ET_WG(64, 64, 2, 2)
#define ET_WGRS_ROWS ET_WGRS(128, 128, 2, 4, 1) ET_WGRS(64, 64, 2, 2, 1) ET_WGRS(128, 64, 2, 2, 2)
#define ET_WGREG_ROWS ET_WGREG(128, 128) ET_WGREG(128, 64) ET_WGREG(64, 128) ET_WGREG(64, 64)
enum { WGRAD_REG = 0, WGRAD_TR = 1, WGRAD_RS = 2 };
struct WgradRow { int kind, bm, bn, wm, wn, stride; };
#define ET_WG(BM_, BN_, WM_, WN_) {WGRAD_TR, BM_, BN_, WM_, WN_, 0},
#define ET_WGRS(BM_, BN_, WM_, WN_, ST_) {WGRAD_RS, BM_, BN_, WM_, WN_, ST_},
#define ET_WGREG(BM_, BN_) {WGRAD_REG, BM_, BN_, 2, 2, 0},
static const WgradRow wg_rows[] = {ET_WG_ROWS};
static const WgradRow wgrs_rows[] = {ET_WGRS_ROWS};
static const WgradRow wgreg_rows[] = {ET_WGREG_ROWS};
#undef ET_WG
#undef ET_WGRS
#undef ET_WGREG

static const WgradRow* plan_wgrad(const WgradGeom& g, int elem_bytes, bool have_zero_page) {
    const bool wideN = g.NC > 64;
    const bool tallM = g.Cout > 64;
    struct { bool tr; int bm, bn; bool rs; int rs_stride; } p{false, tallM ? 128 : 64, wideN ? 128 : 64, false, 1};
    p.tr = elem_bytes == 2 && have_zero_page;
    if (p.tr) {
        if (g.T > 1 && g.Cout >= 256 && g.NC >= 256) { p.bm = 256; p.bn = 256; }
        else if (g.T > 1 && g.isy == 1 && g.NC >= 256 && g.Cout == 128) p.bn = 256;
        else if (g.T == 1 && g.Cout >= 512 && g.NC >= 512) { p.bm = 256; p.bn = 256; }
    }
    if (p.tr && g.T == 9 && g.isy == 1 && g.isx == 1 && g.dy[0] == -1 && g.dx[0] == -1 && g.dy[8] == 1 && g.dx[8] == 1 &&
        g.QH == g.IH && g.QW == g.IW && g.QW >= 2 && 64 / (g.QW + 1) + 2 <= g.QH &&
        (long long)g.N * g.IH * g.IW * (g.ldx > g.ldy ? g.ldx : g.ldy) < (1ll << 31)) {
        if (g.Cout >= 128 && g.Cin >= 128) { p.rs = true; p.bm = 128; p.bn = 128; }
        else if (g.Cout <= 64 && g.Cin <= 64) { p.rs = true; p.bm = 64; p.bn = 64; }
    }
    if (p.tr && g.T == 9 && g.isy == 2 && g.isx == 2 && g.dy[0] == -1 && g.dx[0] == -1 && g.dy[8] == 1 && g.dx[8] == 1 &&
        g.IH == 2 * g.QH && g.IW == 2 * g.QW && g.QW >= 2 && 64 / (g.QW + 1) + 2 <= g.QH && g.Cout >= 128 && g.Cin >= 64 && g.Cin < 128 &&
        (long long)g.N * g.IH * g.IW * (g.ldx > g.ldy ? g.ldx : g.ldy) < (1ll << 31)) {
        p.rs = true; p.rs_stride = 2; p.bm = 128; p.bn = 64;
    }
    if (p.rs) return find_row(wgrs_rows, [&](const WgradRow& r) { return r.bm == p.bm && r.bn == p.bn && r.stride == p.rs_stride; });
    const auto tile = [&](const WgradRow& r) { return r.bm == p.bm && r.bn == p.bn; };
    return p.tr ? find_row(wg_rows, tile) : find_row(wgreg_rows, tile);
}
static void wgrad_plan_name(const WgradRow& p, int dtype, char* buf, int n) {
    const char* t = dtype_tname(dtype);
    if (p.kind == WGRAD_RS && p.stride == 2) snprintf(buf, n, "conv_wgrad_rs_kernel<%s, %d, %d, %d, %d, 2>", t, p.bm, p.bn, p.wm, p.wn);
    else if (p.kind == WGRAD_RS) snprintf(buf, n, "conv_wgrad_rs_kernel<%s, %d, %d, %d, %d>", t, p.bm, p.bn, p.wm, p.wn);
    else if (p.kind == WGRAD_TR) snprintf(buf, n, "conv_wgrad_tr_kernel<%s, %d, %d, %d, %d>", t, p.bm, p.bn, p.wm, p.wn);
    else snprintf(buf, n, "conv_wgrad_kernel<%s, %d, %d>", t, p.bm, p.bn);
}

struct SplitK { int per, nsk; };
static SplitK wgrad_split_k(int len, int chunk, int tiles, int cap) {
    const int max_sk = max(1, len / (chunk * 25));
    auto eff = [&](int k) { const int b = tiles * k; return (double)b / ((double)((b + cap - 1) / cap) * cap); };
    int sk = max(1, min(cap / tiles, max_sk));
    if (eff(sk) < 0.8)
        for (int k = sk + 1; k <= min(max_sk, max(4, 2 * cap / tiles)); ++k)
            if (eff(k) > eff(sk) + 0.1) sk = k;
    sk = max(1, min(sk, max_sk));
    int per = (len + sk - 1) / sk;
    per = ((per + chunk - 1) / chunk) * chunk;
    return SplitK{per, (len + per - 1) / per};
}

template <typename T>
static int launch_wgrad(const WgradGroup& grp, const void* zero16, WgradGeom& g, hipStream_t s) {
    constexpr int VEC = et_elem<T>::VEC;
    constexpr int BKP = 8 * VEC;
    const WgradRow* const wp = plan_wgrad(g, (int)sizeof(T), zero16 != nullptr);
    if (!wp) return -2;
    const bool tr = wp->kind == WGRAD_TR;
    const int bm = wp->bm, bn = wp->bn, n_cu = device_cus();
    const uint16_t* z = (const uint16_t*)zero16;
    g.xcd = 1;
    g.ntm = (g.Cout + bm - 1) / bm;
    int i = 0;
    if constexpr (sizeof(T) == 2) {
        if (wp->kind == WGRAD_RS) {
            g.ntn = 3 * ((g.Cin + bn - 1) / bn);
            const int slots = wp->stride == 2 ? 2 : (bm == 128 ? 2 : 4);
            const SplitK sk = wgrad_split_k(g.PP, 64, grp.n * g.ntn * g.ntm, slots * n_cu);
            g.Pper = sk.per; g.nsk = sk.nsk;
            const dim3 grid(grp.n * g.ntn * g.ntm * sk.nsk);
#define ET_WGRS(BM_, BN_, WM_, WN_, ST_) \
    if (wp == &wgrs_rows[i++]) { hipLaunchKernelGGL((conv_wgrad_rs_kernel<T, BM_, BN_, WM_, WN_, ST_>), grid, dim3(64 * WM_ * WN_), 0, s, grp, z, g); return 0; }
            ET_WGRS_ROWS
#undef ET_WGRS
            return -2;
        }
    }
    g.ntn = (g.NC + bn - 1) / bn;
    const int lds_kb = tr ? (bm + bn) / 4 : 64;
    const int slots = tr ? max(1, min(160 / lds_kb, bm * bn <= 64 * 64 ? 5 : (bm * bn <= 128 * 64 ? 3 : 2))) : 2;
    const SplitK sk = wgrad_split_k(g.P, BKP, grp.n * g.ntn * g.ntm, slots * n_cu);
    g.Pper = sk.per; g.nsk = sk.nsk;
    if constexpr (sizeof(T) == 2) {
        if (tr) {
            const dim3 grid(grp.n * g.ntn * g.ntm * sk.nsk);
            g.buf = g.ident && env_int("ET_CONV_BUF_DMA", 1);
            for (int k = 0; k < grp.n && g.buf; ++k)
                if ((size_t)g.P * grp.it[k].ldx * 2 >= (1ull << 31) || (size_t)g.P * grp.it[k].ldy * 2 >= (1ull << 31)) g.buf = 0;
#define ET_WG(BM_, BN_, WM_, WN_) \
    if (wp == &wg_rows[i++]) { hipLaunchKernelGGL((conv_wgrad_tr_kernel<T, BM_, BN_, WM_, WN_>), grid, dim3(64 * WM_ * WN_), 0, s, grp, z, g); return 0; }
            ET_WG_ROWS
#undef ET_WG
            return -2;
        }
    }
    const dim3 grid(g.ntn * g.ntm * sk.nsk), block(256);
    for (int k = 0; k < grp.n; ++k) {
        const T* xx = (const T*)grp.it[k].x; const T* yy = (const T*)grp.it[k].dy;
        float* dw = grp.it[k].dw;
        g.ldx = grp.it[k].ldx; g.ldy = grp.it[k].ldy;
        i = 0;
#define ET_WGREG(BM_, BN_) \
    if (wp == &wgreg_rows[i++]) hipLaunchKernelGGL((conv_wgrad_kernel<T, BM_, BN_>), grid, block, 0, s, xx, yy, dw, g);
        ET_WGREG_ROWS
#undef ET_WGREG
    }
    return wp->kind == WGRAD_REG ? 0 : -2;
}

extern "C" int et_conv2d_wgrad_grouped(const et_wgrad_item* items, int n_items, int dtype, int N, int IH, int IW, int Cin,
                                       int Cout, int KH, int KW, int stride, int pad, const void* zero16,
                                       et_stream_t stream) {
    if (!items || n_items <= 0 || n_items > WGRAD_MAX_GROUP) return -1;
    if (KH * KW > CONV_MAX_TAPS || stride < 1 || N <= 0) return -2;
    const int vec = dtype == ET_F32 ? 4 : 8;
    if (Cin % vec || Cout % vec) return -2;
    WgradGroup grp;
    grp.n = n_items;
    for (int i = 0; i < n_items; ++i) {
        if (!items[i].x || !items[i].dy || !items[i].dw) return -1;
        grp.it[i].x = (const uint16_t*)items[i].x; grp.it[i].dy = (const uint16_t*)items[i].dy; grp.it[i].dw = items[i].dw;
// ... 234 lines not shown
```

### efficientteacher_amd/models/backbone/common.py

```python
import torch
import torch.nn as nn

from ... import ops
from ... import autograd as _ag
from ...autograd import BottleneckFn, C3StemFn, ConvBnActFn, JoinSlicesFn, SppfPoolFn, c3_stem_fusable


_ACTIVATIONS = {"silu": (nn.SiLU, None), "relu": (lambda: nn.ReLU(inplace=True), "relu")}


def get_activation(act=True):
    if isinstance(act, str):
        if act not in _ACTIVATIONS:
            raise AttributeError(f"activation '{act}' has no fused kernel (supported: {sorted(_ACTIVATIONS)})")
        make, name = _ACTIVATIONS[act]
        return make(), name
    if isinstance(act, nn.Module):
        return act, None
    return (nn.SiLU() if act is True else nn.Identity()), None


def autopad(k, p=None):
    if p is not None:
        return p
    return [x // 2 for x in k] if isinstance(k, (list, tuple)) else k // 2


def _act_code(m):
    if isinstance(m, nn.SiLU):
        return ops.ACT_SILU
    if isinstance(m, nn.ReLU):
        return ops.ACT_RELU
    if isinstance(m, nn.Identity):
        return ops.ACT_NONE
    raise NotImplementedError(f"activation {type(m).__name__} has no gfx950 kernel yet (SiLU / ReLU / Identity only)")


class Conv(nn.Module):
    def __init__(self, c1, c2, k=1, s=1, p=None, g=1, act=True):
        super().__init__()
        self.conv = nn.Conv2d(c1, c2, k, s, autopad(k, p), groups=g, bias=False)
        self.bn = nn.BatchNorm2d(c2)
        self.act, self.act_name = get_activation(act=act)

    def forward(self, x, residual=None, dst=None, bn_in=None, bn_out=None, acc=None):
        cs = getattr(self.conv, "_et_slot", None)
        if cs is None:
            raise RuntimeError("model state is not on the device arenas yet: move the Model to a GPU "
                               "(model.to('cuda')) before calling it -- there is no CPU path")
        bs = self.bn._et_slot
        act = _act_code(self.act)
        u8 = None
        if isinstance(x, ops.U8Images):
            mode = ops.stem_u8_mode(x, cs.w_lp, cs.stride, cs.pad)
            u8 = x if mode & 2 else None
            if not mode & 1:
                x = x.packed()
        if self.bn.training:
            nbt = None if self._et_flat().bulk_nbt else self.bn.num_batches_tracked
            return ConvBnActFn.apply(x, residual, self.conv.weight, cs, bs, act, nbt, dst, bn_in, bn_out, acc, u8)
        flat = self._et_flat()
        o = bs.aff_off
        out = None if dst is None else dst[0][..., dst[1]:dst[1] + cs.coutp]
        return ops.conv2d_fwd(x, cs.w_lp, cs.stride, cs.pad, scale=flat.eval_scale[o:o + bs.c],
                              bias=flat.eval_shift[o:o + bs.c], act=act, residual=residual, out=out)

    def forward_fuse(self, x):
        return self.forward(x)

    def _et_flat(self):
        return self.conv._et_flat_ref()


class Bottleneck(nn.Module):
    def __init__(self, c1, c2, shortcut=True, g=1, k=(1, 3), e=0.5, act=True):
        super().__init__()
        c_ = int(c2 * e)
        self.cv1 = Conv(c1, c_, k[0], 1, act=act)
        self.cv2 = Conv(c_, c2, k[1], 1, g=g, act=act)
        self.add = shortcut and c1 == c2

    def forward(self, x, dst=None, bn_in=None, bn_out=None):
        c1, c2 = self.cv1, self.cv2
        if (self.add and c1.bn.training and c2.bn.training and torch.is_grad_enabled() and c1.conv.stride[0] == 1
                and getattr(c1.conv, "_et_slot", None) is not None):
            bulk = c1._et_flat().bulk_nbt
            return BottleneckFn.apply(x, c1.conv.weight, c2.conv.weight, c1.conv._et_slot, c1.bn._et_slot,
                                      c2.conv._et_slot, c2.bn._et_slot, _act_code(c1.act), _act_code(c2.act),
                                      None if bulk else c1.bn.num_batches_tracked,
                                      None if bulk else c2.bn.num_batches_tracked, dst, bn_in, bn_out)
        if self.add or not (c1.bn.training and torch.is_grad_enabled() and _ag.FUSE_BN_BWD):
            return self.cv2(self.cv1(x), residual=x if self.add else None, dst=dst)
        mid = []
        h = self.cv1(x, bn_in=bn_in, bn_out=mid)
        return self.cv2(h, dst=dst, bn_in=mid[0] if mid else None, bn_out=bn_out)


class C3(nn.Module):
    def __init__(self, c1, c2, n=1, shortcut=True, g=1, e=0.5, act=True):
        super().__init__()
        c_ = int(c2 * e)
        if act == 'relu_silu':
            act, last_act = 'relu', 'silu'
        elif act == 'silu':
            act, last_act = 'silu', 'silu'
        elif act == 'relu_lrelu':
            act, last_act = 'relu', 'lrelu'
        elif act == 'relu_hswish':
            act, last_act = 'relu', 'hard_swish'
        else:
            last_act = act
        self.cv1 = Conv(c1, c_, 1, 1, act=act)
        self.cv2 = Conv(c1, c_, 1, 1, act=act)
        self.cv3 = Conv(2 * c_, c2, 1, act=last_act)
        self.m = nn.Sequential(*[Bottleneck(c_, c_, shortcut, g, e=1.0, act=act) for _ in range(n)])

    def forward(self, x, dst=None):
        N, H, W, _ = x.shape
        c_ = self.cv2.conv.out_channels
        c1s, c2s = getattr(self.cv1.conv, "_et_slot", None), getattr(self.cv2.conv, "_et_slot", None)
        last = len(self.m) - 1
        if (c1s is not None and self.cv1.bn.training and self.cv2.bn.training and torch.is_grad_enabled()
                and len(self.m) > 0 and c3_stem_fusable(c1s, self.cv1.bn._et_slot, c2s, self.cv2.bn._et_slot)):
            buf = torch.empty((N, H, W, 3 * c_), dtype=x.dtype, device=x.device)
            bulk = self.cv1._et_flat().bulk_nbt
            fuse = _ag.FUSE_BN_BWD
            hand = [] if fuse else None
            t, y2 = C3StemFn.apply(x, self.cv1.conv.weight, self.cv2.conv.weight, c1s, self.cv1.bn._et_slot, c2s,
                                   self.cv2.bn._et_slot, _act_code(self.cv1.act),
                                   None if bulk else self.cv1.bn.num_batches_tracked,
                                   None if bulk else self.cv2.bn.num_batches_tracked, buf, hand)
            for i, b in enumerate(self.m):
                nxt = [] if (fuse and i != last) else None
                t = b(t, dst=(buf, c_) if i == last else None, bn_in=hand[0] if hand else None, bn_out=nxt)
                hand = nxt
            return self.cv3(JoinSlicesFn.apply((buf[..., c_:],), t, y2), dst=dst)
        if (c1s is not None and not self.cv1.bn.training and not self.cv2.bn.training and not torch.is_grad_enabled() and len(self.m) > 0
                and c3_stem_fusable(c1s, self.cv1.bn._et_slot, c2s, self.cv2.bn._et_slot)
                and _act_code(self.cv1.act) == _act_code(self.cv2.act)):
            flat = self.cv1._et_flat()
            o = self.cv1.bn._et_slot.aff_off
            buf = torch.empty((N, H, W, 2 * c_), dtype=x.dtype, device=x.device)
            wf = c1s.w_lp.as_strided((2 * c_, 1, 1, c1s.cinp), (c1s.cinp, c1s.cinp, c1s.cinp, 1), c1s.w_lp.storage_offset())
            ops.conv2d_fwd(x, wf, 1, 0, scale=flat.eval_scale[o:o + 2 * c_], bias=flat.eval_shift[o:o + 2 * c_],
                           act=_act_code(self.cv1.act), out=buf)
            t = buf[..., :c_]
            for i, b in enumerate(self.m):
                t = b(t, dst=(buf, 0) if i == last else None)
            return self.cv3(buf, dst=dst)
        buf = torch.empty((N, H, W, 2 * c_), dtype=x.dtype, device=x.device)
        y2 = self.cv2(x, dst=(buf, c_))
        train = self.cv1.bn.training and torch.is_grad_enabled() and _ag.FUSE_BN_BWD and len(self.m) > 0
        hand = [] if train else None
        t = self.cv1(x, bn_out=hand)
        for i, b in enumerate(self.m):
            nxt = [] if (train and i != last) else None
            t = b(t, dst=(buf, 0) if i == last else None, bn_in=hand[0] if hand else None, bn_out=nxt)
            hand = nxt
        if torch.is_grad_enabled() and (t.requires_grad or y2.requires_grad):
            cat = JoinSlicesFn.apply((buf,), t, y2)
        else:
            cat = buf
        return self.cv3(cat, dst=dst)


class C2f(nn.Module):
    def __init__(self, c1, c2, n=1, shortcut=False, g=1, e=0.5, act=True):
        super().__init__()
        self.c = int(c2 * e)
        if self.c % 8:
            raise NotImplementedError("C2f hidden width must be a multiple of 8 channels (16-byte NHWC vectors)")
        self.cv1 = Conv(c1, 2 * self.c, 1, 1, act=act)
        self.cv2 = Conv((2 + n) * self.c, c2, 1, act=act)
        self.m = nn.ModuleList(Bottleneck(self.c, self.c, shortcut, g, k=(3, 3), e=1.0, act=act) for _ in range(n))

    def forward(self, x):
        N, H, W, _ = x.shape
        c, n = self.c, len(self.m)
        buf = torch.empty((N, H, W, (2 + n) * c), dtype=x.dtype, device=x.device)
        y = self.cv1(x, dst=(buf, 0))
        parts = [y]
        t = y[..., c:]
        for i, m in enumerate(self.m):
            t = m(t, dst=(buf, (2 + i) * c))
            parts.append(t)
        if torch.is_grad_enabled() and any(p.requires_grad for p in parts):
            return self.cv2(JoinSlicesFn.apply((buf,), *parts))
        return self.cv2(buf)


class SPPF(nn.Module):
    def __init__(self, c1, c2, k=5, act=True):
        super().__init__()
        if k != 5:
            raise NotImplementedError("the SPPF pooling kernel is specialised for k=5 (every shipped config)")
        c_ = c1 // 2
        if act == 'relu_silu':
            act, last_act = 'relu', 'silu'
        elif act == 'relu_lrelu':
            act, last_act = 'relu', 'lrelu'
        elif act == 'relu_hswish':
            act, last_act = 'relu', 'hard_swish'
        else:
            last_act = act
        self.cv1 = Conv(c1, c_, 1, 1, act=act)
        self.cv2 = Conv(c_ * 4, c2, 1, 1, act=last_act)
        self.m = nn.MaxPool2d(kernel_size=k, stride=1, padding=k // 2)

    def forward(self, x):
        cs = getattr(self.cv1.conv, "_et_slot", None)
        if cs is None or cs.coutp != self.cv1.conv.out_channels:
            return self.cv2(SppfPoolFn.apply(self.cv1(x)))
        N, H, W, _ = x.shape
        cat = torch.empty((N, H, W, 4 * cs.coutp), dtype=x.dtype, device=x.device)
        return self.cv2(SppfPoolFn.apply(self.cv1(x, dst=(cat, 0)), (cat,)))


class Concat(nn.Module):
    def __init__(self, dimension=1):
        super().__init__()
        self.d = dimension

    def forward(self, x):
        return torch.cat(x, 3 if self.d == 1 else self.d)
```

### efficientteacher_amd/models/backbone/yolov5_backbone.py

```python
import torch.nn as nn

from ...autograd import GradFork

from ...utils.general import make_divisible
from .common import C3, SPPF, Conv


STAGE_EVENTS = None


def _mark_stage(name, t):
    if STAGE_EVENTS is not None and t.is_cuda and t.requires_grad:
        import torch
        e = torch.cuda.Event()
        e.record()
        STAGE_EVENTS[name] = e


class YoloV5BackBone(nn.Module):
    reads_u8_images = True
    supports_concat_dst = True

    def __init__(self, cfg):
        super(YoloV5BackBone, self).__init__()
        self.gd = cfg.Model.depth_multiple
        self.gw = cfg.Model.width_multiple
        self.channels_out = {'stage1': 64, 'stage2_1': 128, 'stage2_2': 128, 'stage3_1': 256, 'stage3_2': 256,
                             'stage4_1': 512, 'stage4_2': 512, 'stage5': 1024, 'spp': 1024, 'csp1': 1024,
                             'conv1': 1024}
        self.re_channels_out()
        if cfg.Model.Backbone.activation == 'SiLU':
            CONV_ACT, C_ACT = 'silu', 'silu'
        elif cfg.Model.Backbone.activation == 'ReLU':
            CONV_ACT, C_ACT = 'relu', 'relu'
        else:
            CONV_ACT, C_ACT = 'hard_swish', 'relu_hswish'
        c = self.channels_out
        self.stage1 = Conv(3, c['stage1'], 6, 2, 2, 1, CONV_ACT)
        self.stage2_1 = Conv(c['stage1'], c['stage2_1'], 3, 2, None, 1, CONV_ACT)
        self.stage2_2 = C3(c['stage2_1'], c['stage2_2'], self.get_depth(3), True, 1, 0.5, C_ACT)
        self.stage3_1 = Conv(c['stage2_2'], c['stage3_1'], 3, 2, None, 1, CONV_ACT)
        self.stage3_2 = C3(c['stage3_1'], c['stage3_2'], self.get_depth(6), True, 1, 0.5, C_ACT)
        self.stage4_1 = Conv(c['stage3_2'], c['stage4_1'], 3, 2, None, 1, CONV_ACT)
        self.stage4_2 = C3(c['stage4_1'], c['stage4_2'], self.get_depth(9), True, 1, 0.5, C_ACT)
        self.stage5_1 = Conv(c['stage4_2'], c['stage5'], 3, 2, None, 1, CONV_ACT)
        self.stage5_2 = C3(c['stage5'], c['csp1'], self.get_depth(3), True, 1, 0.5, C_ACT)
        self.sppf = SPPF(c['csp1'], c['spp'], 5, CONV_ACT)
        self.out_shape = {'C3_size': c['stage3_2'], 'C4_size': c['stage4_2'], 'C5_size': c['conv1']}

    def forward(self, x, dst_c3=None, dst_c4=None):
        x1 = self.stage1(x)
        _mark_stage("p1", x1)
        x21 = self.stage2_1(x1)
        x22 = self.stage2_2(x21)
        _mark_stage("p2", x22)
        x31 = self.stage3_1(x22)
        c3, c3n, f3 = GradFork.split(self.stage3_2(x31, dst=dst_c3))
        _mark_stage("p3", c3)
        x41 = self.stage4_1(c3, acc=f3)
        c4, c4n, f4 = GradFork.split(self.stage4_2(x41, dst=dst_c4))
        _mark_stage("p4", c4)
        x51 = self.stage5_1(c4, acc=f4)
        x5 = self.stage5_2(x51)
        return GradFork.tap(c3n, f3), GradFork.tap(c4n, f4), self.sppf(x5)

    def get_depth(self, n):
        return max(round(n * self.gd), 1) if n > 1 else n

    def get_width(self, n):
        return make_divisible(n * self.gw, 8)

    def re_channels_out(self):
        for k, v in self.channels_out.items():
            self.channels_out[k] = self.get_width(v)
```

### efficientteacher_amd/models/head/yolov5_head.py

```python
import math

import torch
import torch.nn as nn

from ... import ops
from ...autograd import ConvBiasFn, head_view


class Detect(nn.Module):
    stride = None

    def __init__(self, cfg):
        super().__init__()
        ds, mdl = cfg.Dataset, cfg.Model
        if ds.np:
            raise NotImplementedError("keypoint heads are outside the hot path")
        self.nc, self.num_keypoints = ds.nc, ds.np
        self.cur_imgsize = [ds.img_size] * 2
        anchor_table = torch.tensor(mdl.anchors, dtype=torch.float32)
        self.nl, self.na = anchor_table.shape[0], anchor_table.shape[1] // 2
        self.no = 5 + self.nc + self.num_keypoints
        self.register_buffer('anchors', anchor_table.view(self.nl, self.na, 2))
        self.grid = [torch.zeros(1) for _ in range(self.nl)]
        self.anchor_grid = [torch.zeros(1) for _ in range(self.nl)]
        widths = [int(c * mdl.width_multiple) for c in mdl.Neck.out_channels]
        self.m = nn.ModuleList([nn.Conv2d(c, self.na * self.no, kernel_size=1) for c in widths])
        self.stride = mdl.Head.strides
        self.export = False

    def initialize_biases(self, cf=None):
        cls_prior = math.log(0.6 / (self.nc - 0.99)) if cf is None else torch.log(cf / cf.sum())
        for conv, s in zip(self.m, self.stride):
            cells = (640 / s) ** 2
            bias = conv.bias.detach().view(self.na, self.no).clone()
            bias[:, 4] += math.log(8 / cells)
            bias[:, 5:] += cls_prior
            conv.bias = torch.nn.Parameter(bias.reshape(-1), requires_grad=True)

    def _raw(self, xi, i):
        cs = getattr(self.m[i], "_et_slot", None)
        if cs is None:
            raise RuntimeError("model state is not on the device arenas yet (model.to('cuda')); no CPU path")
        if self.training and torch.is_grad_enabled():
            return ConvBiasFn.apply(xi, self.m[i].weight, cs, ops.ACT_NONE, (self.na, self.no))
        return head_view(ops.conv2d_fwd(xi, cs.w_lp, 1, 0, bias=cs.bias), self.na, self.no)

    def forward(self, x):
        x = list(x)
        if self.export:
            raise NotImplementedError("export path is out of scope")
        for i in range(self.nl):
            x[i] = self._raw(x[i], i)
        if self.training:
            return x
        B = x[0].shape[0]
        sizes = [xi.shape[1] * xi.shape[2] * xi.shape[3] for xi in x]
        z = torch.empty((B, sum(sizes), self.no), dtype=torch.float32, device=x[0].device)
        off = 0
        for i in range(self.nl):
            apx = (self.anchors[i] * self.stride[i]).float().contiguous()
            ops.detect_decode(x[i], apx, float(self.stride[i]), z, off)
            off += sizes[i]
        return (z, x)
```

### efficientteacher_amd/models/neck/yolov5_neck.py

```python
import torch
import torch.nn as nn

from ...autograd import GradFork, JoinSlicesFn, UpsampleCatFn
from ...utils.general import make_divisible
from ..backbone.common import C3, Concat, Conv


class YoloV5Neck(nn.Module):
    def __init__(self, cfg):
        super(YoloV5Neck, self).__init__()
        self.gd = cfg.Model.depth_multiple
        self.gw = cfg.Model.width_multiple
        input_p3, input_p4, input_p5 = cfg.Model.Neck.in_channels
        output_p3, output_p4, output_p5 = cfg.Model.Neck.out_channels
        self.channels = {'input_p3': input_p3, 'input_p4': input_p4, 'input_p5': input_p5,
                         'output_p3': output_p3, 'output_p4': output_p4, 'output_p5': output_p5}
        self.re_channels_out()
        for k, v in self.channels.items():
            setattr(self, k, v)
        if cfg.Model.Neck.activation == 'SiLU':
            CONV_ACT, C_ACT = 'silu', 'silu'
        elif cfg.Model.Neck.activation == 'ReLU':
            CONV_ACT, C_ACT = 'relu', 'relu'
        else:
            CONV_ACT, C_ACT = 'hard_swish', 'relu_hswish'
        self.conv1 = Conv(self.input_p5, int(self.input_p5 / 2), 1, 1, None, 1, CONV_ACT)
        self.upsample1 = nn.Upsample(scale_factor=2, mode="nearest")
        self.C1 = C3(int(self.input_p5 / 2) + self.input_p4, self.input_p4, self.get_depth(3), False, 1, 0.5, C_ACT)
        self.conv2 = Conv(self.input_p4, self.input_p3, 1, 1, None, 1, CONV_ACT)
        self.upsample2 = nn.Upsample(scale_factor=2, mode="nearest")
        self.C2 = C3(self.input_p3 + self.input_p3, self.output_p3, self.get_depth(3), False, 1, 0.5, C_ACT)
        self.conv3 = Conv(self.output_p3, self.output_p3, 3, 2, None, 1, CONV_ACT)
        self.C3 = C3(self.output_p3 + self.input_p3, self.output_p4, self.get_depth(3), False, 1, 0.5, C_ACT)
        self.conv4 = Conv(self.output_p4, self.output_p4, 3, 2, None, 1, CONV_ACT)
        self.C4 = C3(self.output_p4 + int(self.input_p5 / 2), self.output_p5, self.get_depth(3), False, 1, 0.5, C_ACT)
        self.concat = Concat()

    def get_depth(self, n):
        return max(round(n * self.gd), 1) if n > 1 else n

    def get_width(self, n):
        return make_divisible(n * self.gw, 8)

    def re_channels_out(self):
        for k, v in self.channels.items():
            self.channels[k] = self.get_width(v)

    def concat_slots(self, N, H3, W3, dtype, device):
        c1o, c2o = self.conv1.conv.out_channels, self.conv2.conv.out_channels
        if c1o % 8 or c2o % 8 or self.input_p3 % 8 or self.input_p4 % 8:
            return None
        cat2 = torch.empty((N, H3, W3, c2o + self.input_p3), dtype=dtype, device=device)
        cat1 = torch.empty((N, H3 // 2, W3 // 2, c1o + self.input_p4), dtype=dtype, device=device)
        return (cat2, c2o), (cat1, c1o)

    def forward(self, inputs, cat_bufs=None):
        P3, P4, P5 = inputs
        b3, b4 = cat_bufs if cat_bufs is not None else (None, None)
        N, H5, W5, _ = P5.shape
        c1o = self.conv1.conv.out_channels
        if c1o % 8 or self.conv4.conv.out_channels % 8 or self.conv2.conv.out_channels % 8 or self.conv3.conv.out_channels % 8:
            xp_1 = self.conv1(P5)
            x1 = self.C1(UpsampleCatFn.apply(xp_1, P4, None, b4))
            xp_2 = self.conv2(x1)
            x2 = self.C2(UpsampleCatFn.apply(xp_2, P3, None, b3))
            x3 = self.C3(self.concat([self.conv3(x2), xp_2]))
            x4 = self.C4(self.concat([self.conv4(x3), xp_1]))
            return x2, x3, x4
        c4o = self.conv4.conv.out_channels
        buf4 = torch.empty((N, H5, W5, c4o + c1o), dtype=P5.dtype, device=P5.device)
        xp_1u, xp_1, f1 = GradFork.split(self.conv1(P5, dst=(buf4, c4o)))
        x1 = self.C1(UpsampleCatFn.apply(xp_1u, P4, f1, b4))
        xp_1 = GradFork.tap(xp_1, f1)
        c2o, c3o = self.conv2.conv.out_channels, self.conv3.conv.out_channels
        buf3 = torch.empty((N, x1.shape[1], x1.shape[2], c3o + c2o), dtype=x1.dtype, device=x1.device)
        xp_2u, xp_2, f2 = GradFork.split(self.conv2(x1, dst=(buf3, c3o)))
        x2c, x2, g2 = GradFork.split(self.C2(UpsampleCatFn.apply(xp_2u, P3, f2, b3)))
        xp_2 = GradFork.tap(xp_2, f2)
        t3 = self.conv3(x2c, dst=(buf3, 0), acc=g2)
        x2 = GradFork.tap(x2, g2)
        x3c, x3, g3 = GradFork.split(self.C3(self._join(buf3, t3, xp_2)))
        t4 = self.conv4(x3c, dst=(buf4, 0), acc=g3)
        x3 = GradFork.tap(x3, g3)
        x4 = self.C4(self._join(buf4, t4, xp_1))
        return x2, x3, x4

    @staticmethod
    def _join(buf, a, b):
        if torch.is_grad_enabled() and (a.requires_grad or b.requires_grad):
            return JoinSlicesFn.apply((buf,), a, b)
        return buf
```

### efficientteacher_amd/ops.py

```python
import torch

from . import _lib
from ._lib import ET_BF16, ET_F16, ET_F32

ACT_NONE, ACT_SILU, ACT_RELU = 0, 1, 2


class KernelTimer:

    def __init__(self):
        self.rows = []
        self.shapes = []

    def span(self, tag, flops, launches=1, nbytes=0, shape=None):
        a, b = torch.cuda.Event(enable_timing=True), torch.cuda.Event(enable_timing=True)
        self.rows.append((tag, flops, launches, nbytes, a, b))
        self.shapes.append(shape)
        return a, b

    def summary(self):
        agg = {}
        for tag, fl, n, nb, a, b in self.rows:
            ms = a.elapsed_time(b)
            t = agg.setdefault(tag, dict(ms=0.0, flops=0.0, launches=0, bytes=0.0))
            t["ms"] += ms; t["flops"] += fl; t["launches"] += n; t["bytes"] += nb
        return agg


TIMER = None
SCOPE = None


class FamilyTimer:

    FAMILY = {
        "et_conv2d_fwd": "gather_gemm", "et_conv2d_dgrad": "gather_gemm", "et_conv2d_dgrad_bn": "gather_gemm",
        "et_conv2d_wgrad": "wgrad", "et_conv2d_wgrad_grouped": "wgrad", "et_conv2d_stem_u8_fwd": "gather_gemm", "et_conv2d_stem_u8_wgrad": "wgrad",
        "et_bn_finalize": "bn", "et_bn_act_fwd": "bn", "et_bn_act_fwd_sharded": "bn", "et_bn_act_bwd_sharded": "bn", "et_bn_act_bwd": "bn", "et_bn_act_bwd_from_partials": "bn", "et_act_bwd": "bn",
        "et_nms": "nms_loss_pl", "et_nms_ssod": "nms_loss_pl", "et_detect_decode": "nms_loss_pl", "et_pseudo_label_transform": "nms_loss_pl",
        "et_select_targets": "nms_loss_pl", "et_yolo_loss": "nms_loss_pl", "et_ota_assign": "nms_loss_pl", "et_score_log_append": "nms_loss_pl",
        "et_scale_cast": "nms_loss_pl", "et_domain_focal": "nms_loss_pl", "et_scale_inplace": "nms_loss_pl", "et_v8_decode": "nms_loss_pl",
        "et_tal_loss": "nms_loss_pl", "et_tal_assign": "nms_loss_pl", "et_colsum": "nms_loss_pl", "et_tal_pseudo_split": "nms_loss_pl", "et_tal_targets_pad": "nms_loss_pl",
        "et_tal_assigned_gt": "nms_loss_pl", "et_tal_merge_pseudo": "nms_loss_pl",
        "et_sgd_nesterov": "optimizer_ema", "et_sgd_nesterov_dev": "optimizer_ema", "et_adamw": "optimizer_ema", "et_ema_update": "optimizer_ema",
        "et_ema_update_dev": "optimizer_ema", "et_cast_f32_to_lp": "optimizer_ema", "et_scaler_check": "optimizer_ema", "et_scaler_update": "optimizer_ema", "et_weight_transpose": "optimizer_ema",
        "et_weight_transpose_all": "optimizer_ema", "et_bn_eval_affine": "optimizer_ema",
    }

    def __init__(self):
        self.rows = []

    def begin(self, name):
        fam = self.FAMILY.get(name, "pool_upsample_pack")
        if fam == "gather_gemm":
            fam = "gather_gemm_teacher" if SCOPE == "teacher" else "gather_gemm_student"
        a, b = torch.cuda.Event(enable_timing=True), torch.cuda.Event(enable_timing=True)
        a.record()
        return (fam, torch.cuda.current_stream().cuda_stream, a, b)

    def end(self, tok):
        tok[3].record()
        self.rows.append(tok)

    def summary(self):
        out = {}
        for fam, sid, a, b in self.rows:
            d = out.setdefault(sid, {})
            d[fam] = d.get(fam, 0.0) + a.elapsed_time(b)
        return out


def kernel_name(op, dtype, N, IH, IW, Cin, Cout, k, stride, pad, parity_class=0, zero_page=True):
    import ctypes
    buf = ctypes.create_string_buffer(256)
    code = {"fwd": 0, "dgrad": 1, "wgrad": 2, "dgrad_full": 3, "fwd_res": 4}[op]
    dt = _ET_OF[dtype]
    _lib.check(_lib.load().et_conv2d_kernel_name(code, dt, N, IH, IW, Cin, Cout, k, k, stride, pad, int(bool(zero_page)),
                                                 parity_class, buf, 256), "et_conv2d_kernel_name")
    return buf.value.decode()


def stats_rows(op, dtype, N, IH, IW, Cin, Cout, k, stride, pad, zero_page=True):
    dt = _ET_OF[dtype]
    rows = _lib.load().et_conv2d_stats_rows_for({"fwd": 0, "dgrad_bn": 1, "fwd_res": 2}[op], dt, N, IH, IW, Cin, Cout, k, k, stride, pad, int(bool(zero_page)))
    if rows <= 0:
        raise _lib.EtHipError(f"et_conv2d_stats_rows_for failed with code {rows}")
    return rows


def stats_adds(op, dtype, N, IH, IW, Cin, Cout, k, stride, pad, zero_page=True):
    dt = _ET_OF[dtype]
    n = _lib.load().et_conv2d_stats_adds_for({"fwd": 0, "dgrad_bn": 1, "fwd_res": 2}[op], dt, N, IH, IW, Cin, Cout, k, k, stride, pad, int(bool(zero_page)))
    if n <= 0:
        raise _lib.EtHipError(f"et_conv2d_stats_adds_for failed with code {n}")
    return n


SHARD_MAX_ADDS = 12800
_FEW_ROWS = {}


def few_rows(op, dtype, N, IH, IW, Cin, Cout, k, stride, pad):
    key = (op, dtype, N, IH, IW, Cin, Cout, k, stride, pad)
    r = _FEW_ROWS.get(key)
    if r is None:
        r = _FEW_ROWS[key] = stats_adds(op, dtype, N, IH, IW, Cin, Cout, k, stride, pad)
    return r <= SHARD_MAX_ADDS


def few_reduce_rows(y):
    N, H, W, C = y.shape
    return _lib.load().et_bn_reduce_rows(N * H * W, C, et_dtype(y)) <= SHARD_MAX_ADDS


def env_knobs():
    import ctypes
    buf = ctypes.create_string_buffer(1024)
    _lib.check(_lib.load().et_env_knobs(buf, 1024), "et_env_knobs")
    return buf.value.decode()


_ZERO_PAGES = {}


def zero_page(device):
    z = _ZERO_PAGES.get(device)
    if z is None:
        z = _ZERO_PAGES[device] = torch.zeros(256, dtype=torch.uint8, device=device)
    return z


_BN_TOTALS = {}


def bn_totals_scratch(device):
    key = (device, torch.cuda.current_stream(device).cuda_stream if device.type == "cuda" else 0)
    z = _BN_TOTALS.get(key)
    if z is None:
        z = _BN_TOTALS[key] = torch.zeros(2 * 2048 + 32, dtype=torch.float64, device=device)
    return z


_ET_OF = {torch.float32: ET_F32, torch.bfloat16: ET_BF16, torch.float16: ET_F16}
LP_DTYPES = (torch.bfloat16, torch.float16)


def et_dtype(t):
    try:
        return _ET_OF[t.dtype]
    except KeyError:
        raise TypeError(f"unsupported dtype {t.dtype} (float32 = parity mode, bfloat16 = performance mode, float16 = the "
                        "reference's AMP recipe)") from None


def _nhwc(x):
    assert x.dim() == 4 and x.stride(3) == 1, "NHWC tensor with contiguous channels expected"
    ld = x.stride(2)
    assert x.stride(1) == ld * x.shape[2] and x.stride(0) == ld * x.shape[2] * x.shape[1], \
        "pixels must be dense over the pixel stride"
    return ld


def conv_out_hw(ih, iw, k, s, p):
    return (ih + 2 * p - k) // s + 1, (iw + 2 * p - k) // s + 1


class U8Images:
    requires_grad = False
    is_cuda = True

    def __init__(self, parts, dtype, norm_scale):
        self.parts = [p.contiguous() for p in parts]
        _, C, H, W = self.parts[0].shape
        assert all(p.dtype == torch.uint8 and p.shape[1:] == (C, H, W) and p.device == self.parts[0].device for p in self.parts)
        self.C = C
        self.shape = torch.Size((sum(p.shape[0] for p in self.parts), H, W, 8))
        self.dtype, self.device, self.norm_scale = dtype, self.parts[0].device, float(norm_scale)
        self._packed = None

    def dim(self):
        return 4

    def packed(self):
        if self._packed is None:
            self._packed = pack_input(self.parts, self.dtype, self.norm_scale)
        return self._packed

    def c_segments(self):
        n = len(self.parts)
# ... 139 lines not shown
        self.last.clear()
        self._cb_armed = False
        self.join()

    def submit(self, x, dy, dw, ksize, stride, pad, on_done=None):
        if self.group <= 1 or x.dtype not in LP_DTYPES:
            conv2d_wgrad(x, dy, dw, ksize, stride, pad)
            if on_done is not None:
                on_done()
            return
        if not self._cb_armed:
            try:
                torch.autograd.Variable._execution_engine.queue_callback(self.flush)
                self._cb_armed = True
            except RuntimeError:
                conv2d_wgrad(x, dy, dw, ksize, stride, pad)
                if on_done is not None:
                    on_done()
                return
        key = (tuple(x.shape), tuple(dy.shape), ksize, stride, pad, x.device)
        self.tick += 1
        for k in [k for k, t in self.last.items() if k != key and self.tick - t > self.stale]:
            self._flush_key(k)
        lst = self.pending.setdefault(key, [])
        lst.append((x, dy, dw, on_done))
        self.last[key] = self.tick
        if len(lst) >= self.group:
            self._flush_key(key)

    def submit_stem_u8(self, u8, dy, dw, on_done=None):
        dev = dy.device
        side_ok = dev.type == "cuda" and self.use_side in (1, 3)
        if side_ok and not self._cb_armed:
            try:
                torch.autograd.Variable._execution_engine.queue_callback(self.flush)
                self._cb_armed = True
            except RuntimeError:
                side_ok = False
        if side_ok:
            main, side = torch.cuda.current_stream(dev), self.side_stream(dev)
            side.wait_stream(main)
            with torch.cuda.stream(side):
                stem_u8_wgrad(u8, dy, dw)
                dy.record_stream(side)
                for p in u8.parts:
                    p.record_stream(side)
                if on_done is not None:
                    on_done()
            self._dirty.add(dev)
            return
        stem_u8_wgrad(u8, dy, dw)
        if on_done is not None:
            on_done()

    def _flush_key(self, key):
        lst = self.pending.pop(key, None)
        self.last.pop(key, None)
        if not lst:
            return
        xs, dys, ksize, stride, pad, dev = key
        items = [(a, b, c) for a, b, c, _ in lst]
        if dev.type == "cuda" and (self.use_side == 1 or (self.use_side == 2 and ksize == 1) or (self.use_side == 3 and ksize > 1)):
            main, side = torch.cuda.current_stream(dev), self.side_stream(dev)
            side.wait_stream(main)
            with torch.cuda.stream(side):
                conv2d_wgrad_grouped(items, ksize, stride, pad)
                for a, b, _ in items:
                    a.record_stream(side)
                    b.record_stream(side)
                for _, _, _, cb in lst:
                    if cb is not None:
                        cb()
            self._dirty.add(dev)
            return
        conv2d_wgrad_grouped(items, ksize, stride, pad)
        for _, _, _, cb in lst:
            if cb is not None:
                cb()

    def join(self):
        for dev in self._dirty:
            torch.cuda.current_stream(dev).wait_stream(self._side[dev])
        self._dirty.clear()

    def flush(self):
        self._cb_armed = False
        for key in list(self.pending.keys()):
            self._flush_key(key)
        self.join()


WGRAD_QUEUE = WgradQueue()


def conv2d_wgrad_grouped(items, ksize, stride, pad):
    x0, dy0, dw0 = items[0]
    N, IH, IW, Cin = x0.shape
    _, OH, OW, Cout = dy0.shape
    arr = (_lib.WgradItem * len(items))()
    for i, (x, dy, dw) in enumerate(items):
        assert x.shape == x0.shape and dy.shape == dy0.shape and x.dtype == dy.dtype == x0.dtype
        assert dw.dtype == torch.float32 and dw.is_contiguous() and dw.shape == (Cout, ksize, ksize, Cin)
        arr[i].x, arr[i].dy, arr[i].dw = _lib.ptr(x), _lib.ptr(dy), _lib.ptr(dw)
        arr[i].ldx, arr[i].ldy = _nhwc(x), _nhwc(dy)
    ev = TIMER.span(kernel_name("wgrad", x0.dtype, N, IH, IW, Cin, Cout, ksize, stride, pad),
                    2.0 * len(items) * N * OH * OW * Cout * Cin * ksize * ksize, 1,
                    nbytes=len(items) * ((N * IH * IW * Cin + N * OH * OW * Cout) * x0.element_size() + 8 * Cout * Cin * ksize * ksize),
                    shape=("wgrad", N, IH, IW, Cin, Cout, ksize, stride)) if TIMER else None
    if ev:
        ev[0].record()
    _lib.check(_lib.load().et_conv2d_wgrad_grouped(arr, len(items), et_dtype(x0), N, IH, IW, Cin, Cout, ksize, ksize,
                                                   stride, pad, _lib.ptr(zero_page(x0.device)), _lib.stream(x0)),
               "et_conv2d_wgrad_grouped")
    if ev:
        ev[1].record()


def weight_transpose(w):
    Cout, KH, KW, Cin = w.shape
    wt = torch.empty((Cin, KH, KW, Cout), dtype=w.dtype, device=w.device)
    _lib.check(_lib.load().et_weight_transpose(_lib.ptr(w), _lib.ptr(wt), et_dtype(w), Cout, KH * KW, Cin,
                                               _lib.stream(w)), "et_weight_transpose")
    return wt


def weight_transpose_all(w_arena, wT_arena, table, total):
    _lib.check(_lib.load().et_weight_transpose_all(_lib.ptr(w_arena), _lib.ptr(wT_arena), et_dtype(w_arena),
                                                   _lib.ptr(table), table.shape[0], int(total), _lib.stream(w_arena)),
               "et_weight_transpose_all")


class BnBwdSums:
    __slots__ = ("y", "scale", "shift", "act", "partial", "dz_ptr", "slot")

    def __init__(self, y, scale, shift, act, slot=None):
        self.y, self.scale, self.shift, self.act, self.slot = y, scale, shift, act, slot
        self.partial, self.dz_ptr = None, None

    def take(self, dz):
        p = self.partial if (self.partial is not None and dz.data_ptr() == self.dz_ptr) else None
        self.partial, self.dz_ptr = None, None
        return p


def conv2d_dgrad(dy, wT, in_hw, stride, pad, *, out=None, accumulate=False, residual=None, bn=None):
    N, OH, OW, Cout = dy.shape
    Cin, KH, KW, Cout2 = wT.shape
    assert Cout == Cout2 and wT.dtype == dy.dtype
    IH, IW = in_hw
    assert conv_out_hw(IH, IW, KH, stride, pad) == (OH, OW)
    if out is None:
        assert not accumulate
        out = torch.empty((N, IH, IW, Cin), dtype=dy.dtype, device=dy.device)
    if bn is not None and stride == 1 and not accumulate and bn.y.shape == out.shape and bn.y.dtype == out.dtype:
        lib = _lib.load()
        if bn.slot is not None and few_rows("dgrad_bn", dy.dtype, N, IH, IW, Cin, Cout, KH, stride, pad):
            keep = bn.slot.acquire_bwd()
            part, part_ld = keep
        else:
            rows = stats_rows("dgrad_bn", dy.dtype, N, IH, IW, Cin, Cout, KH, stride, pad)
            keep = part = torch.empty((rows, 2, Cin), dtype=torch.float32, device=dy.device)
            part_ld = 0
        ev = TIMER.span(kernel_name("dgrad_full", dy.dtype, N, IH, IW, Cin, Cout, KH, stride, pad), 2.0 * N * OH * OW * Cout * Cin * KH * KW,
                        nbytes=(dy.numel() + 2 * N * IH * IW * Cin + wT.numel()) * dy.element_size(),
                        shape=("dgrad", N, IH, IW, Cin, Cout, KH, stride)) if TIMER else None
        if ev:
            ev[0].record()
        _lib.check(lib.et_conv2d_dgrad_bn(_lib.ptr(dy), _lib.ptr(wT), _lib.ptr(out), et_dtype(dy), N, IH, IW, Cin, _nhwc(out), Cout,
                                          KH, KW, pad, _nhwc(dy), _lib.ptr(residual), _nhwc(residual) if residual is not None else 0,
                                          _lib.ptr(bn.y), _nhwc(bn.y), _lib.ptr(bn.scale), _lib.ptr(bn.shift), bn.act,
                                          _lib.ptr(part), part_ld, _lib.ptr(zero_page(dy.device)), _lib.stream(dy)), "et_conv2d_dgrad_bn")
        if ev:
            ev[1].record()
        bn.partial, bn.dz_ptr = keep, out.data_ptr()
        return out
    tag = (kernel_name("dgrad_full" if (accumulate or residual is not None) else "dgrad", dy.dtype, N, IH, IW, Cin, Cout, KH, stride, pad) if stride == 1 else
           "conv_gemm (stride-2 dgrad parity classes)") if TIMER else None
    ev = TIMER.span(tag, 2.0 * N * OH * OW * Cout * Cin * KH * KW,
                    stride * stride, nbytes=(dy.numel() + N * IH * IW * Cin + wT.numel()) * dy.element_size(),
                    shape=("dgrad", N, IH, IW, Cin, Cout, KH, stride)) if TIMER else None
    if ev:
        ev[0].record()
    _lib.check(_lib.load().et_conv2d_dgrad(_lib.ptr(dy), _lib.ptr(wT), _lib.ptr(out), et_dtype(dy), N, IH, IW, Cin,
                                           _nhwc(out), Cout, KH, KW, stride, pad, _nhwc(dy), int(accumulate),
                                           _lib.ptr(residual), _nhwc(residual) if residual is not None else 0,
                                           _lib.ptr(zero_page(dy.device)), _lib.stream(dy)), "et_conv2d_dgrad")
    if ev:
        ev[1].record()
    return out


def conv2d_wgrad(x, dy, dw, ksize, stride, pad):
    N, IH, IW, Cin = x.shape
    _, OH, OW, Cout = dy.shape
    assert dw.dtype == torch.float32 and dw.is_contiguous() and dw.shape == (Cout, ksize, ksize, Cin)
    assert x.dtype == dy.dtype
    ev = TIMER.span(kernel_name("wgrad", x.dtype, N, IH, IW, Cin, Cout, ksize, stride, pad), 2.0 * N * OH * OW * Cout * Cin * ksize * ksize) if TIMER else None
    if ev:
        ev[0].record()
    _lib.check(_lib.load().et_conv2d_wgrad(_lib.ptr(x), _lib.ptr(dy), _lib.ptr(dw), et_dtype(x), N, IH, IW, Cin,
                                           _nhwc(x), Cout, ksize, ksize, stride, pad, _nhwc(dy),
                                           _lib.ptr(zero_page(x.device)), _lib.stream(x)), "et_conv2d_wgrad")
    if ev:
        ev[1].record()
    return dw


def colsum(x2d_like, out):
    N, H, W, C = x2d_like.shape
    _lib.check(_lib.load().et_colsum(_lib.ptr(x2d_like), et_dtype(x2d_like), N * H * W, C, _nhwc(x2d_like),
                                     _lib.ptr(out), _lib.stream(out)), "et_colsum")
    return out


def bn_finalize(stats, count, gamma, beta, eps, momentum, running_mean=None, running_var=None):
    rows, _, C = stats.shape
    dev = stats.device
    aff = torch.empty((4, C), dtype=torch.float32, device=dev)
    scale, shift, mean, invstd = aff[0], aff[1], aff[2], aff[3]
    assert C <= 2048
    ws = bn_totals_scratch(dev)
    _lib.check(_lib.load().et_bn_finalize(_lib.ptr(stats), rows, C, float(count), _lib.ptr(gamma), _lib.ptr(beta),
                                          eps, momentum, _lib.ptr(running_mean), _lib.ptr(running_var),
                                          _lib.ptr(scale), _lib.ptr(shift), _lib.ptr(mean), _lib.ptr(invstd),
                                          _lib.ptr(ws), _lib.stream(stats)), "et_bn_finalize")
    return scale, shift, mean, invstd


def bn_eval_affine(gamma, beta, running_mean, running_var, eps):
    C = gamma.numel()
    scale = torch.empty(C, dtype=torch.float32, device=gamma.device)
    shift = torch.empty_like(scale)
    _lib.check(_lib.load().et_bn_eval_affine(C, _lib.ptr(gamma), _lib.ptr(beta), _lib.ptr(running_mean),
                                             _lib.ptr(running_var), eps, _lib.ptr(scale), _lib.ptr(shift),
                                             _lib.stream(gamma)), "et_bn_eval_affine")
    return scale, shift


def bn_act_fwd(y, scale, shift, act, residual=None, out=None):
    N, H, W, C = y.shape
    if out is None:
        out = torch.empty((N, H, W, C), dtype=y.dtype, device=y.device)
    ldr = _nhwc(residual) if residual is not None else 0
    _lib.check(_lib.load().et_bn_act_fwd(_lib.ptr(y), _nhwc(y), _lib.ptr(out), _nhwc(out), _lib.ptr(residual), ldr,
                                         et_dtype(y), N * H * W, C, _lib.ptr(scale), _lib.ptr(shift), act,
                                         _lib.stream(y)), "et_bn_act_fwd")
    return out


def bn_act_fwd_sharded(y, shards, count, gamma, beta, eps, momentum, running_mean, running_var, act, residual=None, out=None, aff=None):
    N, H, W, C = y.shape
    if out is None:
        out = torch.empty((N, H, W, C), dtype=y.dtype, device=y.device)
    if aff is None:
        aff = torch.empty((4, C), dtype=torch.float32, device=y.device)
    ldr = _nhwc(residual) if residual is not None else 0
    sh, ld = shards
    a0 = _lib.ptr(aff)
    rs = aff.stride(0) * 4
    assert aff.stride(1) == 1 and aff.dtype == torch.float32
    _lib.check(_lib.load().et_bn_act_fwd_sharded(_lib.ptr(y), _nhwc(y), _lib.ptr(out), _nhwc(out), _lib.ptr(residual), ldr, et_dtype(y),
                                                 N * H * W, C, _lib.ptr(sh), ld, float(count), _lib.ptr(gamma), _lib.ptr(beta), eps,
                                                 momentum, _lib.ptr(running_mean), _lib.ptr(running_var), a0, a0 + rs, a0 + 2 * rs,
                                                 a0 + 3 * rs, act, _lib.stream(y)),
               "et_bn_act_fwd_sharded")
    sc, shf, mean, invstd = aff.unbind(0)
    return out, sc, shf, mean, invstd


def bn_act_bwd(dz, y, gamma, scale, shift, mean, invstd, act, dgamma, dbeta, out=None, partial=None, shards=None):
    N, H, W, C = y.shape
    lib = _lib.load()
    if out is None:
        out = torch.empty((N, H, W, C), dtype=y.dtype, device=y.device)
    if shards is not None:
        sh, ld = shards
        _lib.check(lib.et_bn_act_bwd_sharded(_lib.ptr(dz), _nhwc(dz), _lib.ptr(y), _nhwc(y), _lib.ptr(out), _nhwc(out), et_dtype(y),
                                             N * H * W, C, _lib.ptr(gamma), _lib.ptr(scale), _lib.ptr(shift), _lib.ptr(mean),
                                             _lib.ptr(invstd), act, _lib.ptr(dgamma), _lib.ptr(dbeta), _lib.ptr(sh), ld,
                                             0 if partial is not None else 1, _lib.stream(y)), "et_bn_act_bwd_sharded")
        return out
    if partial is not None:
        ws = torch.empty(3 * C, dtype=torch.float32, device=y.device)
        _lib.check(lib.et_bn_act_bwd_from_partials(_lib.ptr(dz), _nhwc(dz), _lib.ptr(y), _nhwc(y), _lib.ptr(out), _nhwc(out),
                                                   et_dtype(y), N * H * W, C, _lib.ptr(gamma), _lib.ptr(scale), _lib.ptr(shift),
                                                   _lib.ptr(mean), _lib.ptr(invstd), act, _lib.ptr(dgamma), _lib.ptr(dbeta),
                                                   _lib.ptr(bn_totals_scratch(y.device)), _lib.ptr(partial), partial.shape[0],
                                                   _lib.ptr(ws), _lib.stream(y)), "et_bn_act_bwd_from_partials")
        return out
    rows = lib.et_bn_reduce_rows(N * H * W, C, et_dtype(y))
    nws = rows * 2 * C + 3 * C
    ws = torch.empty(nws, dtype=torch.float32, device=y.device)
    _lib.check(lib.et_bn_act_bwd(_lib.ptr(dz), _nhwc(dz), _lib.ptr(y), _nhwc(y), _lib.ptr(out), _nhwc(out),
                                 et_dtype(y), N * H * W, C, _lib.ptr(gamma), _lib.ptr(scale), _lib.ptr(shift),
                                 _lib.ptr(mean), _lib.ptr(invstd), act, _lib.ptr(dgamma), _lib.ptr(dbeta),
                                 _lib.ptr(bn_totals_scratch(y.device)), _lib.ptr(ws), nws, _lib.stream(y)),
               "et_bn_act_bwd")
    return out


def act_bwd(dz, y, act, out=None):
    N, H, W, C = y.shape
    if out is None:
        out = torch.empty((N, H, W, C), dtype=y.dtype, device=y.device)
    _lib.check(_lib.load().et_act_bwd(_lib.ptr(dz), _nhwc(dz), _lib.ptr(y), _nhwc(y), _lib.ptr(out), _nhwc(out),
                                      et_dtype(y), N * H * W, C, act, _lib.stream(y)), "et_act_bwd")
    return out


def pack_input(x_nchw, dtype, norm_scale=255.0, out=None):
    if isinstance(x_nchw, (list, tuple)):
        parts = list(x_nchw)
        _, C, H, W = parts[0].shape
        assert all(p.shape[1:] == parts[0].shape[1:] and p.device == parts[0].device for p in parts)
        y = torch.empty((sum(p.shape[0] for p in parts), H, W, 8), dtype=dtype, device=parts[0].device)
        b0 = 0
        for p in parts:
            pack_input(p, dtype, norm_scale, out=y[b0:b0 + p.shape[0]])
            b0 += p.shape[0]
        return y
    x = x_nchw.contiguous()
    B, C, H, W = x.shape
    y = out if out is not None else torch.empty((B, H, W, 8), dtype=dtype, device=x.device)
    assert y.shape == (B, H, W, 8) and y.is_contiguous() and y.dtype == dtype
    if x.dtype == torch.uint8:
        _lib.check(_lib.load().et_pack_input_u8(_lib.ptr(x), _lib.ptr(y), et_dtype(y), B, C, H, W, float(norm_scale), _lib.stream(x)),
                   "et_pack_input_u8")
        return y
    if x.dtype != torch.float32:
        x = x.float()
    _lib.check(_lib.load().et_pack_input(_lib.ptr(x), _lib.ptr(y), et_dtype(y), B, C, H, W, _lib.stream(x)),
               "et_pack_input")
    return y


def maxpool5_fwd(x, out=None):
    N, H, W, C = x.shape
    if out is None:
        out = torch.empty((N, H, W, C), dtype=x.dtype, device=x.device)
    idx = torch.empty((N, H, W, C), dtype=torch.uint8, device=x.device)
    _lib.check(_lib.load().et_maxpool5_fwd(_lib.ptr(x), _nhwc(x), _lib.ptr(out), _nhwc(out), _lib.ptr(idx),
                                           et_dtype(x), N, H, W, C, _lib.stream(x)), "et_maxpool5_fwd")
    return out, idx


def maxpool5_bwd(dy, idx, base=None, out=None):
    N, H, W, C = dy.shape
    if out is None:
        out = torch.empty((N, H, W, C), dtype=dy.dtype, device=dy.device)
    ldb = _nhwc(base) if base is not None else 0
    _lib.check(_lib.load().et_maxpool5_bwd(_lib.ptr(dy), _nhwc(dy), _lib.ptr(idx), _lib.ptr(base), ldb, _lib.ptr(out),
                                           _nhwc(out), et_dtype(dy), N, H, W, C, _lib.stream(dy)), "et_maxpool5_bwd")
    return out


def upsample2x_fwd(x, out=None):
    N, H, W, C = x.shape
    if out is None:
        out = torch.empty((N, 2 * H, 2 * W, C), dtype=x.dtype, device=x.device)
    _lib.check(_lib.load().et_upsample2x_fwd(_lib.ptr(x), _nhwc(x), _lib.ptr(out), _nhwc(out), et_dtype(x), N, H, W, C,
                                             _lib.stream(x)), "et_upsample2x_fwd")
    return out


def upsample2x_bwd(dy, out=None, accumulate=False):
    N, H2, W2, C = dy.shape
    H, W = H2 // 2, W2 // 2
    if out is None:
        assert not accumulate
        out = torch.empty((N, H, W, C), dtype=dy.dtype, device=dy.device)
    assert out.shape == (N, H, W, C) and out.dtype == dy.dtype
    _lib.check(_lib.load().et_upsample2x_bwd(_lib.ptr(dy), _nhwc(dy), _lib.ptr(out), _nhwc(out), et_dtype(dy), N, H, W, C,
                                             int(bool(accumulate)), _lib.stream(dy)), "et_upsample2x_bwd")
    return out


def pseudo_label_transform(dets, counts, M_s, width, height, clip01=False):
    B, max_det, _ = dets.shape
    dev = dets.device
    M_s = M_s.to(device=dev, dtype=torch.float64).contiguous()
    t9 = torch.empty((B * max_det, 9), dtype=torch.float64, device=dev)
    valid = torch.empty((B * max_det,), dtype=torch.uint8, device=dev)
    _lib.check(_lib.load().et_pseudo_label_transform(_lib.ptr(dets), _lib.ptr(counts), _lib.ptr(M_s), B, max_det,
                                                     int(width), int(height), int(bool(clip01)), _lib.ptr(t9),
                                                     _lib.ptr(valid), _lib.stream(dets)), "et_pseudo_label_transform")
    return t9, valid


def strong_view_u8(weak, minv, lut, cutouts, flags, border_value=114):
    B, C, H, W = weak.shape
    assert weak.dtype == torch.uint8 and C == 3 and weak.is_contiguous()
    assert minv.dtype == torch.float64 and minv.shape == (B, 6) and flags.dtype == torch.int32 and flags.shape == (B, 3)
    assert cutouts.dtype == torch.int32 and cutouts.shape == (B, 32, 7) and (lut is None or (lut.dtype == torch.uint8 and lut.shape == (B, 3, 256)))
    out = torch.empty_like(weak)
    _lib.check(_lib.load().et_strong_view_u8(_lib.ptr(weak), _lib.ptr(out), B, H, W, _lib.ptr(minv.contiguous()),
                                             _lib.ptr(lut.contiguous()) if lut is not None else None, _lib.ptr(cutouts.contiguous()),
                                             _lib.ptr(flags.contiguous()), int(border_value), _lib.stream(weak)), "et_strong_view_u8")
    return out


def score_log_append(dets, counts, conf_log, cls_log, log_count):
    B, max_det, _ = dets.shape
    assert conf_log.dtype == torch.float32 and cls_log.dtype == torch.int32 and log_count.dtype == torch.int64
    assert conf_log.numel() == cls_log.numel()
    _lib.check(_lib.load().et_score_log_append(_lib.ptr(dets), _lib.ptr(counts), B, max_det, _lib.ptr(conf_log),
                                               _lib.ptr(cls_log), _lib.ptr(log_count), conf_log.numel(),
                                               _lib.stream(dets)), "et_score_log_append")


def val_match(dets, counts, targets, shapes, net_hw, iouv, nc, correct, conf, cls, valid, nt, row_offset=0, single_cls=False):
    B, max_det = dets.shape[0], dets.shape[1]
    if dets.dtype != torch.float32 or dets.stride(2) != 1 or (B > 1 and dets.stride(0) != max_det * dets.stride(1)):
        dets = dets.float().contiguous()
    assert counts.dtype == torch.int32 and counts.numel() == B and counts.is_contiguous()
    targets = targets.reshape(-1, 6)
    if targets.dtype != torch.float32 or not targets.is_contiguous():
        targets = targets.float().contiguous()
    assert shapes.dtype == torch.float32 and shapes.shape == (B, 5) and shapes.is_contiguous()
    assert iouv.dtype == torch.float32 and iouv.is_contiguous() and nt.dtype == torch.int32 and nt.numel() == nc
    rows = conf.numel()
    assert correct.dtype == cls.dtype == valid.dtype == torch.int32 and conf.dtype == torch.float32
    assert correct.numel() == cls.numel() == valid.numel() == rows
    NT = targets.shape[0]
    _lib.check(_lib.load().et_val_match(_lib.ptr(dets), dets.stride(1), _lib.ptr(counts), B, max_det,
                                        _lib.ptr(targets) if NT else None, NT, _lib.ptr(shapes), int(net_hw[0]), int(net_hw[1]),
                                        _lib.ptr(iouv), iouv.numel(), int(bool(single_cls)), int(nc), int(row_offset), rows,
                                        _lib.ptr(correct), _lib.ptr(conf), _lib.ptr(cls), _lib.ptr(valid), _lib.ptr(nt),
# ... 366 lines not shown
```

### include/et_hip.h

```cpp
#ifndef ET_HIP_H
#define ET_HIP_H
#include <stddef.h>
#include <stdint.h>

#ifdef __cplusplus
extern "C" {
#endif

typedef void* et_stream_t;

enum { ET_F32 = 0, ET_BF16 = 1, ET_F16 = 2 };

#define ET_ABI_VERSION 8
const char* et_build_arch(void);
int et_abi_version(void);

int et_nms_ssod_workspace_bytes(int B, int A, size_t* bytes );
int et_nms_ssod(const float* pred, int B, int A, int no, float conf_thres, float iou_thres,
                int agnostic, int max_det, float* dets, int* counts, int64_t* keep,
                int* n_candidates, void* workspace, size_t ws_bytes, et_stream_t stream);

int et_nms_workspace_bytes(int B, int A, int no, int multi_label, int max_nms, size_t* bytes );
int et_nms(const float* pred, int B, int A, int no, float conf_thres, float iou_thres, int agnostic,
           int multi_label, uint64_t class_mask_lo, uint64_t class_mask_hi, int max_nms, float max_wh,
           int max_det, float* dets, int* counts, int64_t* keep, int* n_candidates, void* workspace,
           size_t ws_bytes, et_stream_t stream);

int et_val_match(const float* dets, int det_row_stride, const int* counts, int B, int max_det, const float* targets, int NT,
                 const float* shapes, int net_h, int net_w, const float* iouv, int niou, int single_cls, int nc,
                 int64_t row_offset, int64_t arena_rows, int* correct, float* conf, int* cls, int* valid, int* nt,
                 et_stream_t stream);

int et_val_ap_workspace_bytes(int nc, size_t* bytes );
int et_val_ap(const int* cls, const int* correct, const float* conf, int64_t N, const int* nt, int nc, int niou, double* ap,
              double* p, double* r, double* f1, void* workspace, size_t ws_bytes, et_stream_t stream);

int et_detect_decode(const void* raw, int dtype, int B, int na, int ny, int nx, int no,
                     int64_t sb, int64_t sa, int64_t sy, int64_t sx, const float* anchor_px,
                     float stride, float* z, int64_t A_total, int64_t a_offset, et_stream_t stream);

int et_ema_update(float* ema, const float* model, int64_t n, float d, float one_minus_d, et_stream_t stream);
int et_adamw(float* p, const float* grad, float* exp_avg, float* exp_avg_sq, void* lp_shadow, int shadow_dtype, int64_t n, float lr,
             float beta1, float beta2, float eps, float weight_decay, int step, float inv_scale, const float* scaler,
             et_stream_t stream);
int et_adamw_tick(double* tick, float beta1, float beta2, const float* scaler, et_stream_t stream);
int et_adamw_dev(float* p, const float* grad, float* exp_avg, float* exp_avg_sq, void* lp_shadow, int shadow_dtype, int64_t n, float lr,
                 float beta1, float beta2, float eps, float weight_decay, const double* tick, float inv_scale, const float* scaler,
                 et_stream_t stream);
int et_sgd_nesterov(float* p, const float* grad, float* momentum_buf, void* lp_shadow, int shadow_dtype, int64_t n,
                    float lr, float momentum, float weight_decay, int first_step, float inv_scale, const float* scaler,
                    et_stream_t stream);
int et_cast_f32_to_lp(const float* src, void* dst, int dtype, int64_t n, et_stream_t stream);
int et_scaler_check(const float* grads, int64_t n, float* scaler, et_stream_t stream);
int et_scaler_update(float* scaler, float growth_factor, float backoff_factor, int growth_interval, et_stream_t stream);
int et_ema_update_dev(float* ema, const float* model, int64_t n, const float* d_and_one_minus_d, et_stream_t stream);
int et_sgd_nesterov_dev(float* p, const float* grad, float* momentum_buf, void* lp_shadow, int shadow_dtype, int64_t n,
                        const float* hp, int first_step, const float* scaler, et_stream_t stream);

int et_conv2d_stats_rows(int N, int OH, int OW);
int et_conv2d_stats_rows_for(int op, int dtype, int N, int IH, int IW, int Cin, int Cout, int KH, int KW, int stride, int pad,
                             int have_zero_page);
int et_conv2d_stats_adds_for(int op, int dtype, int N, int IH, int IW, int Cin, int Cout, int KH, int KW, int stride, int pad,
                             int have_zero_page);
#define ET_BN_SHARDS 16
int et_conv2d_fwd(const void* x, const void* w, void* y, int dtype, int N, int IH, int IW, int Cin,
                  int ldx, int Cout, int KH, int KW, int stride, int pad, int ldy, const float* scale,
                  const float* bias, int act, const void* residual, int ldr, float* stats_partial, int stats_ld,
                  const void* zero16, et_stream_t stream);
int et_conv2d_dgrad(const void* dy, const void* wT, void* dx, int dtype, int N, int IH, int IW, int Cin,
                    int ldx, int Cout, int KH, int KW, int stride, int pad, int ldy, int accumulate,
                    const void* residual , int ldr,
                    const void* zero16, et_stream_t stream);
int et_conv2d_dgrad_bn(const void* dy, const void* wT, void* dx, int dtype, int N, int IH, int IW, int Cin, int ldx, int Cout,
                       int KH, int KW, int pad, int ldy, const void* residual, int ldr, const void* bn_y, int ld_bn,
                       const float* bn_scale, const float* bn_shift, int bn_act, float* bn_stats_partial,
                       int bn_stats_ld ,
                       const void* zero16, et_stream_t stream);
int et_conv2d_wgrad(const void* x, const void* dy, float* dw, int dtype, int N, int IH, int IW, int Cin,
                    int ldx, int Cout, int KH, int KW, int stride, int pad, int ldy, const void* zero16,
                    et_stream_t stream);
typedef struct et_wgrad_item { const void* x; const void* dy; float* dw; int ldx, ldy; } et_wgrad_item;
int et_conv2d_wgrad_grouped(const et_wgrad_item* items , int n_items, int dtype, int N, int IH, int IW,
                            int Cin, int Cout, int KH, int KW, int stride, int pad, const void* zero16,
                            et_stream_t stream);
int et_weight_transpose(const void* w, void* wT, int dtype, int Cout, int taps, int Cin, et_stream_t stream);
int et_conv2d_kernel_name(int op, int dtype, int N, int IH, int IW, int Cin, int Cout, int KH, int KW, int stride,
                          int pad, int have_zero_page, int parity_class, char* buf , int buflen);
int et_env_knobs(char* buf , int buflen);
int et_conv2d_stem_u8_fwd(const void* const* seg_ptrs, const int* seg_counts, int n_segs, float norm_scale, const void* w, void* y,
                          int dtype, int IH, int IW, int Cout, int ldy, const float* scale, const float* bias, int act,
                          float* stats_partial, int stats_ld, const void* zero16, et_stream_t stream);
int et_conv2d_stem_u8_wgrad(const void* const* seg_ptrs, const int* seg_counts, int n_segs, float norm_scale, const void* dy, float* dw,
                            int dtype, int IH, int IW, int Cout, int ldy, const void* zero16, et_stream_t stream);
int et_conv2d_stem_kernel_name(int op, int dtype, int in_is_u8, int C, int N, int IH, int IW, int Cout, int KH, int KW, int stride,
                               int pad, char* buf , int buflen);
int et_weight_transpose_all(const void* w_arena, void* wT_arena, int dtype, const int* table, int n_layers,
                            long long total_elems, et_stream_t stream);
int et_colsum(const void* x, int dtype, int P, int C, int ld, float* out, et_stream_t stream);

int et_bn_reduce_rows(int P, int C, int dtype);
int et_bn_finalize(const float* stats_partial, int rows, int C, double count, const float* gamma,
                   const float* beta, float eps, float momentum, float* running_mean, float* running_var,
                   float* scale, float* shift, float* save_mean, float* save_invstd,
                   double* ws , et_stream_t stream);
int et_bn_eval_affine(int C, const float* gamma, const float* beta, const float* running_mean,
                      const float* running_var, float eps, float* scale, float* shift, et_stream_t stream);
int et_bn_act_fwd(const void* y, int ldy, void* z, int ldz, const void* residual, int ldr, int dtype, int P,
                  int C, const float* scale, const float* shift, int act, et_stream_t stream);
int et_bn_act_bwd(const void* dz, int lddz, const void* y, int ldy, void* dy, int lddy, int dtype, int P, int C,
                  const float* gamma, const float* scale, const float* shift, const float* save_mean,
                  const float* save_invstd, int act, float* dgamma, float* dbeta,
                  double* totals , float* workspace, size_t ws_floats,
                  et_stream_t stream);
int et_bn_act_bwd_from_partials(const void* dz, int lddz, const void* y, int ldy, void* dy, int lddy, int dtype, int P, int C,
                                const float* gamma, const float* scale, const float* shift, const float* save_mean,
                                const float* save_invstd, int act, float* dgamma, float* dbeta, double* totals,
                                const float* partials, int partial_rows, float* workspace, et_stream_t stream);
int et_bn_act_fwd_sharded(const void* y, int ldy, void* z, int ldz, const void* residual, int ldr, int dtype, int P, int C,
                          const float* shards, int shard_ld, double count, const float* gamma, const float* beta, float eps,
                          float momentum, float* running_mean, float* running_var, float* scale, float* shift, float* save_mean,
                          float* save_invstd, int act, et_stream_t stream);
int et_bn_act_bwd_sharded(const void* dz, int lddz, const void* y, int ldy, void* dy, int lddy, int dtype, int P, int C,
                          const float* gamma, const float* scale, const float* shift, const float* save_mean,
                          const float* save_invstd, int act, float* dgamma, float* dbeta, float* shards, int shard_ld, int reduce,
                          et_stream_t stream);
int et_act_bwd(const void* dz, int lddz, const void* y, int ldy, void* dy, int lddy, int dtype, int P, int C,
               int act, et_stream_t stream);

int et_pack_input(const float* x_nchw, void* y_nhwc8, int dtype, int B, int C, int H, int W, et_stream_t stream);
int et_pack_input_u8(const uint8_t* x_nchw, void* y_nhwc8, int dtype, int B, int C, int H, int W, float norm_scale,
                     et_stream_t stream);
int et_maxpool5_fwd(const void* x, int ldx, void* y, int ldy, uint8_t* argmax, int dtype, int B, int H, int W, int C,
                    et_stream_t stream);
int et_maxpool5_bwd(const void* dy, int lddy, const uint8_t* argmax, const void* base, int ldb, void* dx, int lddx,
                    int dtype, int B, int H, int W, int C, et_stream_t stream);
int et_upsample2x_fwd(const void* x, int ldx, void* y, int ldy, int dtype, int B, int H, int W, int C, et_stream_t stream);
int et_upsample2x_bwd(const void* dy, int lddy, void* dx, int lddx, int dtype, int B, int H, int W, int C,
                      int accumulate , et_stream_t stream);

int et_strong_view_u8(const uint8_t* weak, uint8_t* strong, int B, int H, int W, const double* minv, const uint8_t* lut,
                      const int* cutouts, const int* flags, int border_value, et_stream_t stream);
int et_mosaic4_u8(const int64_t* tiles, uint8_t* out, int B, int S, int border_value, et_stream_t stream);

int et_pseudo_label_transform(const float* dets, const int* counts, const double* M_s, int B, int max_det,
                              int width, int height, int clip01 ,
                              double* targets9, uint8_t* valid, et_stream_t stream);
int et_score_log_append(const float* dets, const int* counts, int B, int max_det, float* conf_log, int* cls_log,
                        uint64_t* log_count, int64_t cap, et_stream_t stream);

typedef struct {
    const void* p;
    float* dp;
    void* tobj_ws;
    int64_t sb, sa, sy, sx;
    int ny, nx;
    float anchors[6];
    float balance;
} et_loss_level;
typedef struct {
    int dtype, B, na, nc, NT, nl;
    float anchor_t, gr, cp, cn, cls_pw, obj_pw, box_w, obj_w, cls_w;
    int pass_mask, ignore_obj;
    const float* targets;
    float* acc_ws;
    float* out;
    const int* ota_match;
    int obj_channel;
    float* balance_dev;
    int autobalance_ssi;
    float fl_gamma;
    et_loss_level level[4];
} et_loss_desc;
int et_yolo_loss(const et_loss_desc* desc , et_stream_t stream);
int et_ota_workspace_bytes(int B, int na, int nl, int NT, size_t* bytes);
int et_ota_assign(const et_loss_desc* desc , const float* strides , float img_size, int top_k,
                  void* workspace, int* match, et_stream_t stream);
int et_select_targets(const double* targets9, const uint8_t* valid, int N, const double* thr_low,
                      const double* thr_high, int nc, int with_obj, float* table, et_stream_t stream);
int et_scale_cast(const float* src, void* dst, int dtype, int64_t n, float scale,
                  const float* dev_scale , et_stream_t stream);

int et_domain_focal(const void* feat, int ldf, int dtype, int64_t P, int label, float gscale, void* grad,
                    int ldg, float* loss_sum, et_stream_t stream);
int et_scale_inplace(void* x, int dtype, int64_t n, float alpha, const float* dev_scale ,
                     et_stream_t stream);

int et_v8_decode(const void* reg, int ld_reg, const void* cls, int ld_cls, int dtype, int B, int H, int W, int reg_max, int nc,
                 float stride, float cell_offset, float* out, int64_t A_total, int64_t a_offset, et_stream_t stream);
int et_tal_loss(const float* pred_scores, const float* pred_distri, const float* anchor_points_s, const float* stride_tensor,
                const float* target_bboxes_px, const float* target_scores, const uint8_t* fg_mask, int B, int A, int nc, int reg_max,
                int iou_kind, float w_class, float w_iou, float w_dfl, float* grad_scores, float* grad_distri,
                float* acc_ws , float* out , et_stream_t stream);
int et_tal_assign_workspace_bytes(int B, int A, int G, size_t* bytes );
int et_tal_assign(const float* pd_scores, const float* pd_bboxes, const float* anc_points, const float* gt_labels,
                  const float* gt_bboxes, const float* mask_gt, int B, int A, int G, int nc, int topk, float alpha, float beta,
                  float eps, int64_t* target_labels, float* target_bboxes, float* target_scores, uint8_t* fg_mask,
                  void* workspace, size_t ws_bytes, et_stream_t stream);
int et_tal_targets_pad(const float* targets, int n, int B, int G, float img_w, float img_h, float* out, float* mask, et_stream_t stream);

int et_tal_pseudo_split(const double* targets9, const uint8_t* valid, const double* thr_low, const double* thr_high, int B, int G, int nc,
                        int with_obj, int with_bbox, int with_cls, float img_w, float img_h, float* gt_labels_r, float* gt_bboxes_r,
                        float* gt_labels_u, float* gt_bboxes_u, float* mask_reliable, float* mask_uncertain, float* u_score,
                        uint8_t* u_flags, et_stream_t stream);
int et_tal_assigned_gt(const void* workspace, int B, int A, int G, int32_t* gt_idx, et_stream_t stream);
int et_tal_merge_pseudo(const float* ts_r, const float* tb_r, const uint8_t* fg_r, const float* ts_u, const float* tb_u,
                        const uint8_t* fg_u, const int32_t* gt_idx_u, const float* u_score, const uint8_t* u_flags, int B, int A, int G,
                        int nc, float* target_scores, float* target_bboxes, uint8_t* fg_box, et_stream_t stream);


#ifdef __cplusplus
}
#endif
#endif
```

Measured before the change: 1344.

## Fuse BN backward reductions into dgrad across split-channel concat inputs

Extends the dgrad epilogue so one kernel can produce BN backward partial sums for two producer BNs whose outputs are concatenated along channels (split at a channel offset). This lets C3 stems, neck joins and ConvBias heads pass BN info into their input-gradient conv, so separate BN reduction passes over the activation gradient can be skipped. It adds per-channel segment selection and extra pointer plumbing in the epilogue, which costs some registers and branching in a hot kernel.

```diff
diff --git a/efficientteacher_amd/_lib.py b/efficientteacher_amd/_lib.py
--- a/efficientteacher_amd/_lib.py
+++ b/efficientteacher_amd/_lib.py
@@ -40,6 +40,8 @@
     "et_conv2d_fwd": (c_int, [P, P, P, c_int] + [c_int] * 11 + [P, P, c_int, P, c_int, P, c_int, P, P]),
     "et_conv2d_dgrad": (c_int, [P, P, P, c_int] + [c_int] * 11 + [c_int, P, c_int, P, P]),
     "et_conv2d_dgrad_bn": (c_int, [P, P, P, c_int] + [c_int] * 10 + [P, c_int, P, c_int, P, P, c_int, P, c_int, P, P]),
+    "et_conv2d_dgrad_bn2": (c_int, [P, P, P, c_int] + [c_int] * 10 + [P, c_int, P, c_int, P, P, c_int, P, c_int,
+                                    c_int, P, c_int, P, P, c_int, P, c_int, P, P]),
     "et_conv2d_wgrad": (c_int, [P, P, P, c_int] + [c_int] * 11 + [P, P]),
     "et_conv2d_wgrad_grouped": (c_int, [P, c_int, c_int] + [c_int] * 9 + [P, P]),
     "et_weight_transpose_all": (c_int, [P, P, c_int, P, c_int, ctypes.c_longlong, P]),
diff --git a/efficientteacher_amd/autograd.py b/efficientteacher_amd/autograd.py
--- a/efficientteacher_amd/autograd.py
+++ b/efficientteacher_amd/autograd.py
@@ -7,6 +7,7 @@
 
 FUSE_BN_BWD = True
 FUSE_BN_BWD_K = 1
+FUSE_BN_BWD_SETS = 7
 _RS_DGRAD = {}
 
 
@@ -21,7 +22,7 @@
 
 
 def _fuse_into(cs, bn, x=None):
-    if bn is None:
+    if bn is None or not FUSE_BN_BWD:
         return None
     if FUSE_BN_BWD_K & (1 if cs.k == 1 else 2):
         return bn
@@ -245,7 +246,8 @@
 class C3StemFn(Function):
 
     @staticmethod
-    def forward(ctx, x, w1, w2, cs1, bs1, cs2, bs2, act, nbt1, nbt2, buf, bn_out=None):
+    def forward(ctx, x, w1, w2, cs1, bs1, cs2, bs2, act, nbt1, nbt2, buf, bn_out=None, bn_in=None, bn_out2=None):
+        ctx.bn_in = bn_in
         ctx.w_needs_grad = w1.requires_grad or w2.requires_grad
         c = cs1.cout
         wf = cs1.w_lp.as_strided((2 * c, 1, 1, cs1.cinp), (cs1.cinp, cs1.cinp, cs1.cinp, 1), cs1.w_lp.storage_offset())
@@ -277,6 +279,10 @@
         if bn_out is not None:
             ctx.bn_mine = _bn_sums(y[..., :c], aff[0][:c], aff[1][:c], act, bs1)
             bn_out.append(ctx.bn_mine)
+        ctx.bn_mine2 = None
+        if bn_out2 is not None:
+            ctx.bn_mine2 = _bn_sums(y[..., c:], aff[0][c:], aff[1][c:], act, bs2)
+            bn_out2.append(ctx.bn_mine2)
         ctx.save_for_backward(x, y, *aff)
         return t, y2
 
@@ -294,14 +300,14 @@
                 continue
             g = _dense_or_slice(g)
             _bn_train_bwd(g, y[..., sl], bs, scale[sl], shift[sl], mean[sl], invstd[sl], act,
-                          sums=ctx.bn_mine if sl.start == 0 else None, out=dy[..., sl])
+                          sums=ctx.bn_mine if sl.start == 0 else ctx.bn_mine2, out=dy[..., sl])
         if ctx.w_needs_grad:
             _wgrad(x, dy, cs1, cs2)
         dx = None
         if ctx.x_needs_grad:
             wf = cs1.w_lp.as_strided((2 * c, 1, 1, cs1.cinp), (cs1.cinp, cs1.cinp, cs1.cinp, 1), cs1.w_lp.storage_offset())
-            dx = ops.conv2d_dgrad(dy, ops.weight_transpose(wf), (x.shape[1], x.shape[2]), 1, 0)
-        return (dx,) + (None,) * 11
+            dx = ops.conv2d_dgrad(dy, ops.weight_transpose(wf), (x.shape[1], x.shape[2]), 1, 0, bn=_fuse_into(cs1, ctx.bn_in, x))
+        return (dx,) + (None,) * 13
 
 
 class _GradDst:
@@ -362,7 +368,8 @@
 class ConvBiasFn(Function):
 
     @staticmethod
-    def forward(ctx, x, wparam, cs, act, head):
+    def forward(ctx, x, wparam, cs, act, head, bn_in=None):
+        ctx.bn_in = bn_in if cs.stride == 1 else None
         ctx.w_needs_grad = wparam.requires_grad
         y = ops.conv2d_fwd(x, cs.w_lp, cs.stride, cs.pad, bias=cs.bias, act=act)
         ctx.cs, ctx.act, ctx.head = cs, act, head
@@ -390,8 +397,8 @@
         dx = None
         if ctx.x_needs_grad:
             wT = cs.transposed()
-            dx = ops.conv2d_dgrad(dy, wT, (x.shape[1], x.shape[2]), cs.stride, cs.pad)
-        return dx, None, None, None, None
+            dx = ops.conv2d_dgrad(dy, wT, (x.shape[1], x.shape[2]), cs.stride, cs.pad, bn=_fuse_into(cs, ctx.bn_in, x))
+        return dx, None, None, None, None, None
 
 
 def head_view(y, na, no):
diff --git a/efficientteacher_amd/csrc/conv.hip b/efficientteacher_amd/csrc/conv.hip
--- a/efficientteacher_amd/csrc/conv.hip
+++ b/efficientteacher_amd/csrc/conv.hip
@@ -90,6 +90,14 @@
     const float* bn_shift;
     int bn_act;
     int stats_ld;
+    int bn_split;
+    const void* bn_y2;
+    int ld_bn2;
+    const float* bn_scale2;
+    const float* bn_shift2;
+    int bn_act2;
+    float* stats2;
+    int stats_ld2;
 };
 
 __device__ __forceinline__ void tile_of_block(const GatherGeom& g, int& bx, int& by) {
@@ -192,17 +200,22 @@
 #pragma unroll
         for (int e = 0; e < 8; ++e)
             for (int m = CVN; m < 64; m <<= 1) { st.bs1[e] += __shfl_xor(st.bs1[e], m); st.bs2[e] += __shfl_xor(st.bs2[e], m); }
+        const bool s2 = co >= ep.bn_split;
+        float* const sdst = s2 ? ep.stats2 : ep.stats;
+        const int sld = s2 ? ep.stats_ld2 : ep.stats_ld;
+        const int cs = s2 ? co - ep.bn_split : co;
+        const int cw = s2 ? g.Cout - ep.bn_split : (ep.bn_split < g.Cout ? ep.bn_split : g.Cout);
         if (ep.stats_ld) {
-            if (lane < CVN && co + 8 <= g.Cout) {
-                float* d0 = ep.stats + ((size_t)(blockIdx.x % ET_BN_SHARDS) * 2) * ep.stats_ld + co;
-#pragma unroll
-                for (int e = 0; e < 8; ++e) { unsafeAtomicAdd(d0 + e, st.bs1[e]); unsafeAtomicAdd(d0 + ep.stats_ld + e, st.bs2[e]); }
-            }
-        } else if (lane < CVN && co + 8 <= g.Cout) {
+            if (lane < CVN && co + 8 <= g.Cout && sdst) {
+                float* d0 = sdst + ((size_t)(blockIdx.x % ET_BN_SHARDS) * 2) * sld + cs;
+#pragma unroll
+                for (int e = 0; e < 8; ++e) { unsafeAtomicAdd(d0 + e, st.bs1[e]); unsafeAtomicAdd(d0 + sld + e, st.bs2[e]); }
+            }
+        } else if (lane < CVN && co + 8 <= g.Cout && sdst) {
             for (int r = 0; r <= zero_rows; ++r) {
                 if (row + r >= nrows) break;
-                float* d0 = ep.stats + ((size_t)(row + r) * 2 + 0) * g.Cout + co;
-                float* d1 = ep.stats + ((size_t)(row + r) * 2 + 1) * g.Cout + co;
+                float* d0 = sdst + ((size_t)(row + r) * 2 + 0) * cw + cs;
+                float* d1 = sdst + ((size_t)(row + r) * 2 + 1) * cw + cs;
                 if (r == 0) {
                     *(float4*)d0 = make_float4(st.bs1[0], st.bs1[1], st.bs1[2], st.bs1[3]); *(float4*)(d0 + 4) = make_float4(st.bs1[4], st.bs1[5], st.bs1[6], st.bs1[7]);
                     *(float4*)d1 = make_float4(st.bs2[0], st.bs2[1], st.bs2[2], st.bs2[3]); *(float4*)(d1 + 4) = make_float4(st.bs2[4], st.bs2[5], st.bs2[6], st.bs2[7]);
@@ -266,7 +279,10 @@
         float v = 0.f;
 #pragma unroll
         for (int w = 0; w < WM; ++w) v += red[(w * 2 + t) * BN + c];
-        if (n0 + c < g.Cout) unsafeAtomicAdd(dst + (size_t)t * ep.stats_ld + c, v);
+        if (n0 + c >= g.Cout) continue;
+        if (bnb && n0 + c >= ep.bn_split) {
+            if (ep.stats2) unsafeAtomicAdd(ep.stats2 + ((size_t)(blockIdx.x % ET_BN_SHARDS) * 2 + t) * ep.stats_ld2 + (n0 + c - ep.bn_split), v);
+        } else unsafeAtomicAdd(dst + (size_t)t * ep.stats_ld + c, v);
     }
 }
 
@@ -309,14 +325,21 @@
     const void* const ep_res = MODE == 1 ? nullptr : ep.res;
     const bool ep_accumulate = MODE == 1 ? false : (bool)ep.accumulate;
     const bool lean = ident && !bnb && ep_res == nullptr && !ep_accumulate && m0 + (wm + 1) * (BM / WM) <= g.M && n0 + BN <= g.Cout;
+    const bool seg2 = bnb && co >= ep.bn_split;
+    const int cseg = seg2 ? co - ep.bn_split : co;
+    const T* const bn_yl = !bnb ? nullptr : (seg2 ? (ep.bn_y2 ? (const T*)ep.bn_y2 + cseg : nullptr) : (const T*)ep.bn_y + cseg);
+    const int bn_ldl = seg2 ? ep.ld_bn2 : ep.ld_bn;
+    const int bn_actl = seg2 ? ep.bn_act2 : ep.bn_act;
     float bsc[8], bsh[8];
 #pragma unroll
     for (int e = 0; e < 8; ++e) { bsc[e] = 1.f; bsh[e] = 0.f; }
-    if (bnb && co + 8 <= g.Cout) {
+    if (bn_yl && co + 8 <= g.Cout) {
+        const float* const sc = seg2 ? ep.bn_scale2 : ep.bn_scale;
+        const float* const sh = seg2 ? ep.bn_shift2 : ep.bn_shift;
 #pragma unroll
         for (int e = 0; e < 8; ++e) {
             if constexpr (DEFER) { bsc[e] = st.cst[2 * st.cstride + co - n0 + e]; bsh[e] = st.cst[3 * st.cstride + co - n0 + e]; }
-            else { bsc[e] = ep.bn_scale[co + e]; bsh[e] = ep.bn_shift[co + e]; }
+            else { bsc[e] = sc[cseg + e]; bsh[e] = sh[cseg + e]; }
         }
     }
     auto bn_bwd_sums = [&](const float (&dz8)[8], const float (&y8)[8]) {
@@ -333,8 +356,8 @@
                 bs2[e] += du * y8[e];
             }
         };
-        if (ep.bn_act == ACT_SILU) body(std::integral_constant<int, ACT_SILU>{});
-        else if (ep.bn_act == ACT_RELU) body(std::integral_constant<int, ACT_RELU>{});
+        if (bn_actl == ACT_SILU) body(std::integral_constant<int, ACT_SILU>{});
+        else if (bn_actl == ACT_RELU) body(std::integral_constant<int, ACT_RELU>{});
         else body(std::integral_constant<int, ACT_NONE>{});
     };
     constexpr int NIT = SROWS / RPI;
@@ -360,7 +383,7 @@
                         const long long pix = pix_of(p);
                         if (pf_a_is_res) pf_a[it] = *(const u32x4*)((const T*)ep_res + pix * ep.ldr + co);
                         else if (ep_accumulate) pf_a[it] = *(const u32x4*)(Y + pix * g.ldy + co);
-                        if (bnb) pf_b[it] = *(const u32x4*)((const T*)ep.bn_y + pix * ep.ld_bn + co);
+                        if (bn_yl) pf_b[it] = *(const u32x4*)(bn_yl + pix * bn_ldl);
                     }
                 }
             }
@@ -431,10 +454,10 @@
                         const u32x4 packed = mk4(et_lp<T>::pack(v[0], v[1]), et_lp<T>::pack(v[2], v[3]), et_lp<T>::pack(v[4], v[5]),
                                                  et_lp<T>::pack(v[6], v[7]));
                         *(u32x4*)yp = packed;
-                        if (bnb) {
+                        if (bn_yl) {
                             u32x4 yy;
                             if constexpr (PF) yy = pf_b[it];
-                            else yy = *(const u32x4*)((const T*)ep.bn_y + pix * ep.ld_bn + co);
+                            else yy = *(const u32x4*)(bn_yl + pix * bn_ldl);
                             const unsigned pw[4] = {packed.x, packed.y, packed.z, packed.w}, yw[4] = {yy.x, yy.y, yy.z, yy.w};
                             float dz8[8], y8[8];
 #pragma unroll
@@ -456,8 +479,8 @@
                         }
                         *(float4*)yp = make_float4(v[0], v[1], v[2], v[3]);
                         *(float4*)((float*)yp + 4) = make_float4(v[4], v[5], v[6], v[7]);
-                        if (bnb) {
-                            const float* bp = (const float*)ep.bn_y + pix * ep.ld_bn + co;
+                        if (bn_yl) {
+                            const float* bp = (const float*)bn_yl + pix * bn_ldl;
                             const float4 y0 = *(const float4*)bp, y1 = *(const float4*)(bp + 4);
                             const float yv8[8] = {y0.x, y0.y, y0.z, y0.w, y1.x, y1.y, y1.z, y1.w};
                             bn_bwd_sums(v, yv8);
@@ -1387,8 +1410,10 @@
         const bool cok = c < g.Cout;
         cst[c] = (ep.scale && cok) ? ep.scale[c] : 1.0f;
         cst[BN + c] = (ep.bias && cok) ? ep.bias[c] : 0.0f;
-        cst[2 * BN + c] = (FULL && ep.bn_y && cok) ? ep.bn_scale[c] : 1.0f;
-        cst[3 * BN + c] = (FULL && ep.bn_y && cok) ? ep.bn_shift[c] : 0.0f;
+        const bool s2 = c >= ep.bn_split;
+        const bool bok = FULL && ep.bn_y && cok && (!s2 || ep.bn_y2);
+        cst[2 * BN + c] = bok ? (s2 ? ep.bn_scale2[c - ep.bn_split] : ep.bn_scale[c]) : 1.0f;
+        cst[3 * BN + c] = bok ? (s2 ? ep.bn_shift2[c - ep.bn_split] : ep.bn_shift[c]) : 0.0f;
     }
 
     int a_row[PER], a_lv[PER];
@@ -2961,14 +2986,22 @@
     dx[(((long long)n * IH + qy * stride + py) * IW + qx * stride + px) * ldx + c] = T(0);
 }
 
+struct BnSecond { int split; const void* y; int ld; const float* scale; const float* shift; int act; float* stats; int stats_ld; };
+
 static int conv2d_dgrad_impl(const void* dy, const void* wT, void* dx, int dtype, int N, int IH, int IW, int Cin,
                              int ldx, int Cout, int KH, int KW, int stride, int pad, int ldy, int accumulate,
                              const void* residual, int ldr, const void* bn_y, int ld_bn, const float* bn_scale,
-                             const float* bn_shift, int bn_act, float* bn_stats, int bn_stats_ld, const void* zero16, et_stream_t stream) {
+                             const float* bn_shift, int bn_act, float* bn_stats, int bn_stats_ld, const void* zero16, et_stream_t stream,
+                             const BnSecond* second = nullptr) {
     if (!dy || !wT || !dx) return -1;
     if (KH * KW > CONV_MAX_TAPS || stride < 1 || stride > 2 || N <= 0) return -2;
     if (residual && stride != 1) return -2;
     if (bn_y && (stride != 1 || !bn_scale || !bn_shift || !bn_stats || Cin % 8 || bn_stats_ld < 0 || (bn_stats_ld && bn_stats_ld < Cin))) return -2;
+    if (second) {
+        const BnSecond& b2 = *second;
+        if (!bn_y || b2.split <= 0 || b2.split >= Cin || b2.split % 8 || (bn_stats_ld && bn_stats_ld < b2.split)) return -2;
+        if (b2.y && (!b2.scale || !b2.shift || !b2.stats || (b2.stats_ld > 0) != (bn_stats_ld > 0) || (b2.stats_ld && b2.stats_ld < Cin - b2.split))) return -2;
+    }
     const int vec = dtype == ET_F32 ? 4 : 8;
     for (int py = 0; py < stride; ++py)
         for (int px = 0; px < stride; ++px) {
@@ -2979,6 +3012,14 @@
             const int t = g.T, QH = g.QH, QW = g.QW;
             Epilogue ep{nullptr, nullptr, ACT_NONE, residual, ldr, bn_y ? bn_stats : nullptr, accumulate,
                         bn_y, ld_bn, bn_scale, bn_shift, bn_act, bn_y ? bn_stats_ld : 0};
+            ep.bn_split = Cin;
+            if (second) {
+                ep.bn_split = second->split;
+                if (second->y) {
+                    ep.bn_y2 = second->y; ep.ld_bn2 = second->ld; ep.bn_scale2 = second->scale; ep.bn_shift2 = second->shift; ep.bn_act2 = second->act;
+                    ep.stats2 = second->stats; ep.stats_ld2 = second->stats_ld;
+                }
+            }
             if (t == 0) {
                 const long long total = (long long)N * QH * QW * Cin;
                 if (!accumulate && total > 0) {
@@ -3009,6 +3050,18 @@
     if (!bn_y) return -1;
     return conv2d_dgrad_impl(dy, wT, dx, dtype, N, IH, IW, Cin, ldx, Cout, KH, KW, 1, pad, ldy, 0, residual, ldr, bn_y, ld_bn,
                              bn_scale, bn_shift, bn_act, bn_stats_partial, bn_stats_ld, zero16, stream);
+}
+
+extern "C" int et_conv2d_dgrad_bn2(const void* dy, const void* wT, void* dx, int dtype, int N, int IH, int IW, int Cin,
+                                   int ldx, int Cout, int KH, int KW, int pad, int ldy, const void* residual, int ldr,
+                                   const void* bn_y, int ld_bn, const float* bn_scale, const float* bn_shift, int bn_act,
+                                   float* bn_stats_partial, int bn_stats_ld, int bn_split,
+                                   const void* bn_y2, int ld_bn2, const float* bn_scale2, const float* bn_shift2, int bn_act2,
+                                   float* bn_stats_partial2, int bn_stats_ld2, const void* zero16, et_stream_t stream) {
+    if (!bn_y) return -1;
+    const BnSecond b2{bn_split, bn_y2, ld_bn2, bn_scale2, bn_shift2, bn_act2, bn_stats_partial2, bn_stats_ld2};
+    return conv2d_dgrad_impl(dy, wT, dx, dtype, N, IH, IW, Cin, ldx, Cout, KH, KW, 1, pad, ldy, 0, residual, ldr, bn_y, ld_bn,
+                             bn_scale, bn_shift, bn_act, bn_stats_partial, bn_stats_ld, zero16, stream, &b2);
 }
 
 static void wgrad_geom(WgradGeom& g, int N, int IH, int IW, int Cin, int ldx, int Cout, int KH, int KW, int stride, int pad, int ldy) {
diff --git a/efficientteacher_amd/models/backbone/common.py b/efficientteacher_amd/models/backbone/common.py
--- a/efficientteacher_amd/models/backbone/common.py
+++ b/efficientteacher_amd/models/backbone/common.py
@@ -115,7 +115,7 @@
         self.cv3 = Conv(2 * c_, c2, 1, act=last_act)
         self.m = nn.Sequential(*[Bottleneck(c_, c_, shortcut, g, e=1.0, act=act) for _ in range(n)])
 
-    def forward(self, x, dst=None):
+    def forward(self, x, dst=None, bn_in=None, bn_out=None):
         N, H, W, _ = x.shape
         c_ = self.cv2.conv.out_channels
         c1s, c2s = getattr(self.cv1.conv, "_et_slot", None), getattr(self.cv2.conv, "_et_slot", None)
@@ -125,16 +125,19 @@
             buf = torch.empty((N, H, W, 3 * c_), dtype=x.dtype, device=x.device)
             bulk = self.cv1._et_flat().bulk_nbt
             fuse = _ag.FUSE_BN_BWD
+            sets = _ag.FUSE_BN_BWD_SETS if fuse else 0
             hand = [] if fuse else None
+            half2 = [] if sets & 2 else None
             t, y2 = C3StemFn.apply(x, self.cv1.conv.weight, self.cv2.conv.weight, c1s, self.cv1.bn._et_slot, c2s,
                                    self.cv2.bn._et_slot, _act_code(self.cv1.act),
                                    None if bulk else self.cv1.bn.num_batches_tracked,
-                                   None if bulk else self.cv2.bn.num_batches_tracked, buf, hand)
+                                   None if bulk else self.cv2.bn.num_batches_tracked, buf, hand, bn_in if sets & 1 else None, half2)
             for i, b in enumerate(self.m):
-                nxt = [] if (fuse and i != last) else None
+                nxt = [] if (fuse and (i != last or sets & 2)) else None
                 t = b(t, dst=(buf, c_) if i == last else None, bn_in=hand[0] if hand else None, bn_out=nxt)
                 hand = nxt
-            return self.cv3(JoinSlicesFn.apply((buf[..., c_:],), t, y2), dst=dst)
+            halves = (hand[0], half2[0], c_) if (sets & 2 and hand and half2) else None
+            return self.cv3(JoinSlicesFn.apply((buf[..., c_:],), t, y2), dst=dst, bn_in=halves, bn_out=bn_out if sets & 4 else None)
         if (c1s is not None and not self.cv1.bn.training and not self.cv2.bn.training and not torch.is_grad_enabled() and len(self.m) > 0
                 and c3_stem_fusable(c1s, self.cv1.bn._et_slot, c2s, self.cv2.bn._et_slot)
                 and _act_code(self.cv1.act) == _act_code(self.cv2.act)):
@@ -207,13 +210,13 @@
         self.cv2 = Conv(c_ * 4, c2, 1, 1, act=last_act)
         self.m = nn.MaxPool2d(kernel_size=k, stride=1, padding=k // 2)
 
-    def forward(self, x):
+    def forward(self, x, bn_in=None, bn_out=None):
         cs = getattr(self.cv1.conv, "_et_slot", None)
         if cs is None or cs.coutp != self.cv1.conv.out_channels:
-            return self.cv2(SppfPoolFn.apply(self.cv1(x)))
+            return self.cv2(SppfPoolFn.apply(self.cv1(x, bn_in=bn_in)), bn_out=bn_out)
         N, H, W, _ = x.shape
         cat = torch.empty((N, H, W, 4 * cs.coutp), dtype=x.dtype, device=x.device)
-        return self.cv2(SppfPoolFn.apply(self.cv1(x, dst=(cat, 0)), (cat,)))
+        return self.cv2(SppfPoolFn.apply(self.cv1(x, dst=(cat, 0), bn_in=bn_in), (cat,)), bn_out=bn_out)
 
 
 class Concat(nn.Module):
diff --git a/efficientteacher_amd/models/backbone/yolov5_backbone.py b/efficientteacher_amd/models/backbone/yolov5_backbone.py
--- a/efficientteacher_amd/models/backbone/yolov5_backbone.py
+++ b/efficientteacher_amd/models/backbone/yolov5_backbone.py
@@ -1,5 +1,6 @@
 import torch.nn as nn
 
+from ... import autograd as _ag
 from ...autograd import GradFork
 
 from ...utils.general import make_divisible
@@ -49,20 +50,28 @@
         self.out_shape = {'C3_size': c['stage3_2'], 'C4_size': c['stage4_2'], 'C5_size': c['conv1']}
 
     def forward(self, x, dst_c3=None, dst_c4=None):
+        train = self.training and _ag.FUSE_BN_BWD
+        sets = _ag.FUSE_BN_BWD_SETS if train else 0
+        h2, h3, h4, h5 = ([] if sets & 1 else None for _ in range(4))
+        h52, hs = ([] if sets & 4 else None for _ in range(2))
+        one = lambda h: h[0] if h else None
         x1 = self.stage1(x)
         _mark_stage("p1", x1)
-        x21 = self.stage2_1(x1)
-        x22 = self.stage2_2(x21)
+        x21 = self.stage2_1(x1, bn_out=h2)
+        x22 = self.stage2_2(x21, bn_in=one(h2))
         _mark_stage("p2", x22)
-        x31 = self.stage3_1(x22)
-        c3, c3n, f3 = GradFork.split(self.stage3_2(x31, dst=dst_c3))
+        x31 = self.stage3_1(x22, bn_out=h3)
+        c3, c3n, f3 = GradFork.split(self.stage3_2(x31, dst=dst_c3, bn_in=one(h3)))
         _mark_stage("p3", c3)
-        x41 = self.stage4_1(c3, acc=f3)
-        c4, c4n, f4 = GradFork.split(self.stage4_2(x41, dst=dst_c4))
+        x41 = self.stage4_1(c3, acc=f3, bn_out=h4)
+        c4, c4n, f4 = GradFork.split(self.stage4_2(x41, dst=dst_c4, bn_in=one(h4)))
         _mark_stage("p4", c4)
-        x51 = self.stage5_1(c4, acc=f4)
-        x5 = self.stage5_2(x51)
-        return GradFork.tap(c3n, f3), GradFork.tap(c4n, f4), self.sppf(x5)
+        x51 = self.stage5_1(c4, acc=f4, bn_out=h5)
+        x5 = self.stage5_2(x51, bn_in=one(h5), bn_out=h52)
+        p5 = self.sppf(x5, bn_in=one(h52), bn_out=hs)
+        if hs:
+            p5._et_bn_sums = hs[0]
+        return GradFork.tap(c3n, f3), GradFork.tap(c4n, f4), p5
 
     def get_depth(self, n):
         return max(round(n * self.gd), 1) if n > 1 else n
diff --git a/efficientteacher_amd/models/head/yolov5_head.py b/efficientteacher_amd/models/head/yolov5_head.py
--- a/efficientteacher_amd/models/head/yolov5_head.py
+++ b/efficientteacher_amd/models/head/yolov5_head.py
@@ -3,7 +3,7 @@
 import torch
 import torch.nn as nn
 
-from ... import ops
+from ... import autograd as _ag, ops
 from ...autograd import ConvBiasFn, head_view
 
 
@@ -42,7 +42,8 @@
         if cs is None:
             raise RuntimeError("model state is not on the device arenas yet (model.to('cuda')); no CPU path")
         if self.training and torch.is_grad_enabled():
-            return ConvBiasFn.apply(xi, self.m[i].weight, cs, ops.ACT_NONE, (self.na, self.no))
+            bn_in = getattr(xi, "_et_bn_sums", None) if (_ag.FUSE_BN_BWD and _ag.FUSE_BN_BWD_SETS & 4) else None
+            return ConvBiasFn.apply(xi, self.m[i].weight, cs, ops.ACT_NONE, (self.na, self.no), bn_in)
         return head_view(ops.conv2d_fwd(xi, cs.w_lp, 1, 0, bias=cs.bias), self.na, self.no)
 
     def forward(self, x):
diff --git a/efficientteacher_amd/models/neck/yolov5_neck.py b/efficientteacher_amd/models/neck/yolov5_neck.py
--- a/efficientteacher_amd/models/neck/yolov5_neck.py
+++ b/efficientteacher_amd/models/neck/yolov5_neck.py
@@ -1,6 +1,7 @@
 import torch
 import torch.nn as nn
 
+from ... import autograd as _ag
 from ...autograd import GradFork, JoinSlicesFn, UpsampleCatFn
 from ...utils.general import make_divisible
 from ..backbone.common import C3, Concat, Conv
@@ -69,20 +70,25 @@
             return x2, x3, x4
         c4o = self.conv4.conv.out_channels
         buf4 = torch.empty((N, H5, W5, c4o + c1o), dtype=P5.dtype, device=P5.device)
-        xp_1u, xp_1, f1 = GradFork.split(self.conv1(P5, dst=(buf4, c4o)))
-        x1 = self.C1(UpsampleCatFn.apply(xp_1u, P4, f1, b4))
+        sets = _ag.FUSE_BN_BWD_SETS if (self.training and _ag.FUSE_BN_BWD and torch.is_grad_enabled()) else 0
+        h1, h3, h4 = ([] if sets & 4 else None), ([] if sets & 1 else None), ([] if sets & 1 else None)
+        h44 = [] if sets & 4 else None
+        xp_1u, xp_1, f1 = GradFork.split(self.conv1(P5, dst=(buf4, c4o), bn_in=getattr(P5, "_et_bn_sums", None) if sets & 4 else None))
+        x1 = self.C1(UpsampleCatFn.apply(xp_1u, P4, f1, b4), bn_out=h1)
         xp_1 = GradFork.tap(xp_1, f1)
         c2o, c3o = self.conv2.conv.out_channels, self.conv3.conv.out_channels
         buf3 = torch.empty((N, x1.shape[1], x1.shape[2], c3o + c2o), dtype=x1.dtype, device=x1.device)
-        xp_2u, xp_2, f2 = GradFork.split(self.conv2(x1, dst=(buf3, c3o)))
+        xp_2u, xp_2, f2 = GradFork.split(self.conv2(x1, dst=(buf3, c3o), bn_in=h1[0] if h1 else None))
         x2c, x2, g2 = GradFork.split(self.C2(UpsampleCatFn.apply(xp_2u, P3, f2, b3)))
         xp_2 = GradFork.tap(xp_2, f2)
-        t3 = self.conv3(x2c, dst=(buf3, 0), acc=g2)
+        t3 = self.conv3(x2c, dst=(buf3, 0), acc=g2, bn_out=h3)
         x2 = GradFork.tap(x2, g2)
-        x3c, x3, g3 = GradFork.split(self.C3(self._join(buf3, t3, xp_2)))
-        t4 = self.conv4(x3c, dst=(buf4, 0), acc=g3)
+        x3c, x3, g3 = GradFork.split(self.C3(self._join(buf3, t3, xp_2), bn_in=(h3[0], None, c3o) if h3 else None))
+        t4 = self.conv4(x3c, dst=(buf4, 0), acc=g3, bn_out=h4)
         x3 = GradFork.tap(x3, g3)
-        x4 = self.C4(self._join(buf4, t4, xp_1))
+        x4 = self.C4(self._join(buf4, t4, xp_1), bn_in=(h4[0], None, c4o) if h4 else None, bn_out=h44)
+        if h44:
+            x4._et_bn_sums = h44[0]
         return x2, x3, x4
 
     @staticmethod
diff --git a/efficientteacher_amd/ops.py b/efficientteacher_amd/ops.py
--- a/efficientteacher_amd/ops.py
+++ b/efficientteacher_amd/ops.py
@@ -34,7 +34,7 @@
 class FamilyTimer:
 
     FAMILY = {
-        "et_conv2d_fwd": "gather_gemm", "et_conv2d_dgrad": "gather_gemm", "et_conv2d_dgrad_bn": "gather_gemm",
+        "et_conv2d_fwd": "gather_gemm", "et_conv2d_dgrad": "gather_gemm", "et_conv2d_dgrad_bn": "gather_gemm", "et_conv2d_dgrad_bn2": "gather_gemm",
         "et_conv2d_wgrad": "wgrad", "et_conv2d_wgrad_grouped": "wgrad", "et_conv2d_stem_u8_fwd": "gather_gemm", "et_conv2d_stem_u8_wgrad": "wgrad",
         "et_bn_finalize": "bn", "et_bn_act_fwd": "bn", "et_bn_act_fwd_sharded": "bn", "et_bn_act_bwd_sharded": "bn", "et_bn_act_bwd": "bn", "et_bn_act_bwd_from_partials": "bn", "et_act_bwd": "bn",
         "et_nms": "nms_loss_pl", "et_nms_ssod": "nms_loss_pl", "et_detect_decode": "nms_loss_pl", "et_pseudo_label_transform": "nms_loss_pl",
@@ -480,6 +480,10 @@
     if out is None:
         assert not accumulate
         out = torch.empty((N, IH, IW, Cin), dtype=dy.dtype, device=dy.device)
+    if isinstance(bn, tuple):
+        if stride == 1 and not accumulate and _bn_pair_fits(bn, out):
+            return _conv2d_dgrad_bn2(dy, wT, out, pad, residual, bn)
+        bn = None
     if bn is not None and stride == 1 and not accumulate and bn.y.shape == out.shape and bn.y.dtype == out.dtype:
         lib = _lib.load()
         if bn.slot is not None and few_rows("dgrad_bn", dy.dtype, N, IH, IW, Cin, Cout, KH, stride, pad):
@@ -518,6 +522,49 @@
     return out
 
 
+def _bn_pair_fits(bn, out):
+    first, second, split = bn
+    N, IH, IW, Cin = out.shape
+    ok = (first is not None and 0 < split < Cin and split % 8 == 0 and first.y.shape == (N, IH, IW, split) and first.y.dtype == out.dtype)
+    return ok and (second is None or (second.y.shape == (N, IH, IW, Cin - split) and second.y.dtype == out.dtype))
+
+
+def _conv2d_dgrad_bn2(dy, wT, out, pad, residual, bn):
+    first, second, split = bn
+    N, OH, OW, Cout = dy.shape
+    Cin, KH, KW, _ = wT.shape
+    IH, IW = out.shape[1], out.shape[2]
+    both = [b for b in (first, second) if b is not None]
+    if all(b.slot is not None for b in both) and few_rows("dgrad_bn", dy.dtype, N, IH, IW, Cin, Cout, KH, 1, pad):
+        keeps = [b.slot.acquire_bwd() for b in both]
+        parts = [(k[0], k[1]) for k in keeps]
+    else:
+        rows = stats_rows("dgrad_bn", dy.dtype, N, IH, IW, Cin, Cout, KH, 1, pad)
+        keeps = [torch.empty((rows, 2, b.y.shape[3]), dtype=torch.float32, device=dy.device) for b in both]
+        parts = [(k, 0) for k in keeps]
+    if second is None:
+        parts.append((None, 0))
+    ev = TIMER.span(kernel_name("dgrad_full", dy.dtype, N, IH, IW, Cin, Cout, KH, 1, pad), 2.0 * N * OH * OW * Cout * Cin * KH * KW,
+                    nbytes=(dy.numel() + N * IH * IW * (Cin + sum(b.y.shape[3] for b in both)) + wT.numel()) * dy.element_size(),
+                    shape=("dgrad", N, IH, IW, Cin, Cout, KH, 1)) if TIMER else None
+    if ev:
+        ev[0].record()
+    s2 = second
+    _lib.check(_lib.load().et_conv2d_dgrad_bn2(
+        _lib.ptr(dy), _lib.ptr(wT), _lib.ptr(out), et_dtype(dy), N, IH, IW, Cin, _nhwc(out), Cout, KH, KW, pad, _nhwc(dy),
+        _lib.ptr(residual), _nhwc(residual) if residual is not None else 0,
+        _lib.ptr(first.y), _nhwc(first.y), _lib.ptr(first.scale), _lib.ptr(first.shift), first.act, _lib.ptr(parts[0][0]), parts[0][1], split,
+        _lib.ptr(s2.y) if s2 else None, _nhwc(s2.y) if s2 else 0, _lib.ptr(s2.scale) if s2 else None, _lib.ptr(s2.shift) if s2 else None,
+        s2.act if s2 else 0, _lib.ptr(parts[1][0]), parts[1][1], _lib.ptr(zero_page(dy.device)), _lib.stream(dy)), "et_conv2d_dgrad_bn2")
+    if ev:
+        ev[1].record()
+    es = out.element_size()
+    first.partial, first.dz_ptr = keeps[0], out.data_ptr()
+    if second is not None:
+        second.partial, second.dz_ptr = keeps[1], out.data_ptr() + split * es
+    return out
+
+
 def conv2d_wgrad(x, dy, dw, ksize, stride, pad):
     N, IH, IW, Cin = x.shape
     _, OH, OW, Cout = dy.shape
@@ -596,11 +643,17 @@
     return out, sc, shf, mean, invstd
 
 
+REDUCE_PASSES = 0
+
+
 def bn_act_bwd(dz, y, gamma, scale, shift, mean, invstd, act, dgamma, dbeta, out=None, partial=None, shards=None):
+    global REDUCE_PASSES
     N, H, W, C = y.shape
     lib = _lib.load()
     if out is None:
         out = torch.empty((N, H, W, C), dtype=y.dtype, device=y.device)
+    if partial is None:
+        REDUCE_PASSES += 1
     if shards is not None:
         sh, ld = shards
         _lib.check(lib.et_bn_act_bwd_sharded(_lib.ptr(dz), _nhwc(dz), _lib.ptr(y), _nhwc(y), _lib.ptr(out), _nhwc(out), et_dtype(y),
diff --git a/include/et_hip.h b/include/et_hip.h
--- a/include/et_hip.h
+++ b/include/et_hip.h
@@ -11,7 +11,7 @@
 
 enum { ET_F32 = 0, ET_BF16 = 1, ET_F16 = 2 };
 
-#define ET_ABI_VERSION 8
+#define ET_ABI_VERSION 9
 const char* et_build_arch(void);
 int et_abi_version(void);
 
@@ -76,6 +76,11 @@
                        const float* bn_scale, const float* bn_shift, int bn_act, float* bn_stats_partial,
                        int bn_stats_ld ,
                        const void* zero16, et_stream_t stream);
+int et_conv2d_dgrad_bn2(const void* dy, const void* wT, void* dx, int dtype, int N, int IH, int IW, int Cin, int ldx, int Cout,
+                        int KH, int KW, int pad, int ldy, const void* residual, int ldr, const void* bn_y, int ld_bn,
+                        const float* bn_scale, const float* bn_shift, int bn_act, float* bn_stats_partial, int bn_stats_ld,
+                        int bn_split, const void* bn_y2, int ld_bn2, const float* bn_scale2, const float* bn_shift2, int bn_act2,
+                        float* bn_stats_partial2, int bn_stats_ld2, const void* zero16, et_stream_t stream);
 int et_conv2d_wgrad(const void* x, const void* dy, float* dw, int dtype, int N, int IH, int IW, int Cin,
                     int ldx, int Cout, int KH, int KW, int stride, int pad, int ldy, const void* zero16,
                     et_stream_t stream);
```

Result: no change. 1340 (-0.3%).
